# TencentARC/ViT-Lens

Hardware: AMD Instinct MI355X
Metric: modality-pairs/sec (ViT-L, 224^2 patches) (higher is better)
Workload: dtype bf16; 1 GPU; C3: ViT-L Lens(depth)->ViT + image + text tri-modal InfoNCE TRAINING step (fwd+bwd+AdamW), batch 1024/GPU in micro-batches of 256, first 4 blocks + adapter trainable; global_batch=1024, residual_dtype=bf16, accumulate=fp32, parallelism=dp1, gemm_cfg=-1, via=step, text_tower_operands=fp16, layernorm=folded into the GEMMs (frozen blocks), frozen_towers=second HIP stream beside the trainable tower's forward, backward=two halves of the micro-batches on two HIP streams

## Files before the change

include/vitlens_hip.h:

```cpp
#ifndef VITLENS_HIP_H
#define VITLENS_HIP_H

#include <stdint.h>

#ifdef __cplusplus
extern "C" {
#endif

#ifndef __HIP_PLATFORM_AMD__
typedef struct ihipStream_t* hipStream_t;
#endif

#define VL_EPI_BF16 0
#define VL_EPI_F32 1
#define VL_EPI_RES_F32 2
#define VL_EPI_RES_BF16 3
#define VL_EPI_GEGLU 5
#define VL_EPI_DGELU 6
#define VL_EPI_DGEGLU 7
#define VL_ACT_NONE 0
#define VL_ACT_GELU 1
#define VL_ACT_RELU 2
#define VL_ACT_GELU_DSAVE 4
#define VL_ACT_QGELU 5
#define VL_ACT_QGELU_DSAVE 6

#define VL_F32 0
#define VL_BF16 1
#define VL_F16 2

#define VL_GEMM_AUTO (-1)
#define VL_GEMM_PERSIST 8
#define VL_GEMM_PINGPONG 10

const char* vl_last_error(void);
#define VL_ABI_VERSION 606
int vl_version(void);

int vl_gemm_bf16(const void* A, const void* W, const float* bias, void* out, const void* res,
                 int M, int N, int K, int lda, int ldw, int ldo, float alpha, int epi, int act,
                 int cfg, hipStream_t stream);

int vl_gemm_splitk_accum_f32(const void* A, const void* W, float* out, int M, int N, int K, int lda, int ldw, long ldo,
                             float alpha, int splits, float* ws, hipStream_t stream);
int vl_gemm_tn_splitk_accum_f32(const void* At, const void* Bt, float* out, int M, int N, int K, int lda, int ldb, long ldo,
                                float alpha, int splits, float* ws, hipStream_t stream);
int vl_gemm_bf16_ex(const void* A, const void* W, const float* bias, void* out, const void* res, void* out2,
                    int M, int N, int K, int lda, int ldw, int ldo, float alpha, int epi, int act,
                    int res_div, int cfg, hipStream_t stream);

int vl_gemm_f16(const void* A, const void* W, const float* bias, void* out, const void* res, int M, int N, int K,
                int lda, int ldw, int ldo, float alpha, int epi, int act, hipStream_t stream);
int vl_attn_fwd_f16(const void* q, const void* k, const void* v, const long* strides, void* out, float* lse,
                    int B, int H, int Lq, int Lk, int dh, float qscale, int causal, hipStream_t stream);

int vl_gemm_f32(const float* A, const float* W, const float* bias, float* out, const float* res, int M, int N, int K,
                int lda, int ldw, int ldo, float alpha, int act, hipStream_t stream);
int vl_attn_fwd_f32(const float* q, const float* k, const float* v, const long* strides, float* out, float* lse,
                    int B, int H, int Lq, int Lk, int dh, float scale, int causal, hipStream_t stream);
int vl_im2col_f32(const float* x, float* patches, int N, int C, int H, int W, int kh, int kw, int sh, int sw,
                  int Kp, int transpose_hw, hipStream_t stream);
int vl_gemm_f32_ex(const float* A, const float* W, const float* bias, float* out, const float* res, int M, int N, int K,
                   int lda, int ldw, int ldo, float alpha, int act, int res_div, int res_pre, int geglu, hipStream_t stream);
int vl_knn_group_f32(const float* xyz, const int64_t* center_idx, int* nidx, float* patches, int B, int N, int G,
                     int k, int Kp, hipStream_t stream);
int vl_group_max_f32(const float* x, long ldx, float* out, long ldo, long groups, int M, int C, hipStream_t stream);
int vl_pad3_f32(const float* c, float* out, long R, int Kp, hipStream_t stream);

int vl_device_info(int device, char* arch, int arch_len, int* cus, int* clock_khz, long* hbm_bytes);

int vl_attn_fwd_bf16(const void* q, const void* k, const void* v, const long* strides, void* out, float* lse,
                     int B, int H, int Lq, int Lk, int dh, float qscale, int causal, hipStream_t stream);

int vl_gemm_main_rows(int M, int N);
int vl_gemm_lnfold_bf16(const void* A, const void* Wg, const float* bias_f, const float* ln_c, const float* ln_mean,
                        const float* ln_rstd, void* out, void* out2, int M, int N, int K, int lda, int ldw, int ldo, int act,
                        hipStream_t stream);
int vl_gemm_res_rowstats_bf16(const void* A, const void* W, const float* bias, void* out, const void* res, float* row_part,
                              int M, int N, int K, int lda, int ldw, int ldo, hipStream_t stream);
int vl_ln_row_stats(const float* row_part, int P, const void* x_bf16, long x_row_stride, int D, int m_main, int rows, float eps,
                    float* mean, float* rstd, const float* ln_w, const float* ln_b, void* y_left, long y_row_stride, int y_row0,
                    hipStream_t stream);

int vl_layernorm_fwd(const void* x, int x_dtype, long x_row_stride, const int64_t* row_index, long row_mul,
                     const float* w, const float* b, void* y, int y_dtype, long y_row_stride,
                     float* mean, float* rstd, int rows, int D, float eps, hipStream_t stream);

int vl_assemble_ln_pre(const void* tokens, int tok_dtype, const float* cls, const float* pos, const float* pos2,
                       const float* w, const float* b, void* y, int y_dtype, float* xpre, float* mean, float* rstd,
                       int B, int T, int D, float eps, hipStream_t stream);

int vl_l2_normalize(const float* x, float* y, void* y_bf16, float* norms, int rows, int D, float eps,
                    hipStream_t stream);
int vl_l2_normalize_bwd(const float* f, const float* df, const float* norms, float* dx, int rows, int D, float eps,
                        hipStream_t stream);

int vl_im2col_bf16(const float* x, void* patches, int N, int C, int H, int W, int kh, int kw, int sh, int sw,
                   int Kp, int transpose_hw, hipStream_t stream);

int vl_text_embed(const int64_t* ids, const float* tok_emb, const float* pos, void* out, int out_dtype,
                  int B, int L, int D, int vocab, hipStream_t stream);

int vl_cast_f32_bf16(const float* x, void* y, long n, hipStream_t stream);
int vl_add_rows(const void* x, int x_dtype, const float* table, void* y, int y_dtype, long rows, int T, int D,
                hipStream_t stream);
int vl_transpose_to_bf16(const void* in, int in_dtype, long ldi, int R, int C, void* out, long ldo, hipStream_t stream);
int vl_transpose_colsum_bf16(const void* in, int in_dtype, long ldi, int R, int C, void* out, long ldo,
                             float* colsum_out, float colsum_scale, float* ws, hipStream_t stream);

int vl_split_bf16x3(const float* x, void* out, long rows, int D, int pattern, hipStream_t stream);
int vl_ce_stats(const float* logits, long ld, int R, int C, int label_off, float* row_lse, float* col_lse,
                float* diag, float* col_ws, hipStream_t stream);
int vl_ce_loss_accum(const float* row_lse, const float* col_lse, const float* diag, int R, int C, int label_off,
                     float w_row, float w_col, float* loss_inout, hipStream_t stream);
int vl_ce_grad(const float* logits, long ld, int R, int C, int label_off, const float* row_lse, const float* col_lse,
               float w_row, float w_col, void* G, long ldg, void* GT, long ldgt, float logit_scale,
               float* dscale_inout, float* ws, hipStream_t stream);
long vl_ce_grad_ws_floats(int R, int C, long ldg, long ldgt);
int vl_ce_stats_masked(const float* logits, long ld, int R, int C, int label_off, float* row_lse, float* col_lse,
                       float* diag, float* col_ws, const float* sim, long ld_sim, float thres, hipStream_t stream);
int vl_ce_grad_masked(const float* logits, long ld, int R, int C, int label_off, const float* row_lse, const float* col_lse,
                      float w_row, float w_col, void* G, long ldg, void* GT, long ldgt, float logit_scale,
                      float* dscale_inout, float* ws, const float* sim, long ld_sim, float thres, hipStream_t stream);

int vl_layernorm_bwd(const void* dy, int dy_dtype, long dy_stride, const void* x, int x_dtype, long x_stride,
                     const float* mean, const float* rstd, const float* w, const float* dres, float* dx,
                     void* dx_bf16, long dx_stride, int rows, int D, hipStream_t stream);
int vl_layernorm_bwd_g(const void* dy, int dy_dtype, long dy_stride, const void* x, int x_dtype, long x_stride,
                       const float* mean, const float* rstd, const float* w, const void* dres, void* dx, int g_dtype,
                       void* dx_bf16, long dx_stride, int rows, int D, hipStream_t stream);
long vl_colreduce_ws_floats(int rows, int cols, int planes);
int vl_layernorm_bwd_params(const void* dy, int dy_dtype, long dy_stride, const void* x, int x_dtype, long x_stride,
                            const float* mean, const float* rstd, float* dw, float* db, int rows, int D,
                            float* ws, hipStream_t stream);
int vl_colsum(const void* a, int a_dtype, long lda, float* out, int rows, int cols, float scale, float* ws, hipStream_t stream);
int vl_gelu_bf16(const void* u, void* y, long n, hipStream_t stream);
int vl_geglu_bf16(const void* h, void* y, long rows, int n_out, hipStream_t stream);
int vl_attn_bwd_bf16(const void* q, const void* k, const void* v, const void* dO, const void* o, const long* strides,
                     const float* lse, float* delta, void* dq, void* dk, void* dv, long ld_dq, long ld_dkv,
                     int B, int H, int Lq, int Lk, int dh, float qscale, int causal, float scale, hipStream_t stream);
int vl_attn_bwd_fused_supported(int Lq, int Lk, int dh, int causal);
int vl_attn_bwd_fused_bf16(const void* q, const void* k, const void* v, const void* dO, const void* o, const long* strides,
                           const float* lse, void* dq, void* dk, void* dv, long ld_dq, long ld_dkv, int B, int H, int L, int dh,
                           float qscale, float scale, hipStream_t stream);
int vl_kaldi_fbank(const float* wave, long wave_stride, int batch, long n_samples, const float* window, const float* banks,
                   float* out, int target_len, int win, int shift, int nfft, int nmel, float preemph, float mean, float std,
                   hipStream_t stream);
int vl_resample_sinc(const float* in, long in_stride, int batch, long n_in, const int* offsets, const float* taps, int o, int n,
                     int K, float* out, long out_stride, long out_first, long n_out, hipStream_t stream);
int vl_fbank_augment(const float* in, float* out, int batch, int T, int F, const void* params, float mean, float std,
                     hipStream_t stream);
int vl_fps(const float* xyz, const int64_t* start, int64_t* idx, float* centers, int B, int N, int G, hipStream_t stream);
int vl_pc_gather_normalize(const float* pts, const int64_t* idx, float* out, int B, int N, int G, int C, hipStream_t stream);
int vl_resample_h_u8(const uint8_t* src, long row_stride, int W, int C, int row0, int nrows, const int* bounds,
                     const int* kk, int ksize, int xout0, int nxout, uint8_t* dst, hipStream_t stream);
int vl_resample_v_u8_norm(const uint8_t* src, int W, int C, int row0, int nrows, const int* bounds, const int* kk,
                          int ksize, int yout0, int nyout, const float* mean, const float* stdv, float* out,
                          uint8_t* out_u8, hipStream_t stream);
int vl_resample_batch_u8_norm(const int64_t* desc, int n, int C, int crop_h, int crop_w, int max_nrows, const int* tables,
                              uint8_t* tmp, const float* mean, const float* stdv, float* out, hipStream_t stream);
int vl_resample_h_f32(const float* src, long row_stride, int W, int row0, int nrows, const int* bounds,
                      const float* weights, int ksize, int xout0, int nxout, int clamp_on, float clamp_lo,
                      float clamp_hi, float divide_by, float* dst, hipStream_t stream);
int vl_resample_v_f32_norm(const float* src, int W, int H, int row0, const int* bounds, const float* weights, int ksize,
                           int yout0, int nyout, float mean, float stdv, float* out, hipStream_t stream);
int vl_knn_group(const float* xyz, const int64_t* center_idx, int* nidx, void* patches, int B, int N, int G,
                 int k, int Kp, hipStream_t stream);
int vl_ball_group(const float* xyz, const float* feats, const int64_t* center_idx, int* idx, void* patches, int B, int N,
                  int S, int D, float radius2, int nsample, int Kp, hipStream_t stream);
int vl_group_max(const void* x, long ldx, void* out, int out_dtype, long ldo, long groups, int M, int C, hipStream_t stream);
int vl_pad3_bf16(const float* c, void* out, long R, int Kp, hipStream_t stream);
int vl_bn_stats(const void* x, long ldx, int R, int C, float* ws, int nchunk, float* mean, float* var,
                float* running_mean, float* running_var, float momentum, hipStream_t stream);
int vl_bn_stats_local(const void* x, long ldx, int R, int C, float* ws, int nchunk, float* local, hipStream_t stream);
int vl_bn_stats_merge(const float* gathered, int W, int C, float* mean, float* var, float* running_mean,
                      float* running_var, float momentum, int* total, hipStream_t stream);
int vl_bn_bwd_reduce(const void* dy, long lddy, const void* x, long ldx, const float* mean, const float* var,
                     const float* gamma, const float* beta, float eps, int relu, float* ws, int nchunk, float* dgamma,
                     float* dbeta, float* sums, int R, int C, hipStream_t stream);
int vl_bn_bwd_apply(const void* dy, long lddy, const void* x, long ldx, const float* mean, const float* var,
                    const float* gamma, const float* beta, float eps, int relu, const float* sums, const int* total,
                    void* dx, long lddx, int R, int C, hipStream_t stream);
int vl_bn_apply(const void* x, long ldx, const float* mean, const float* var, const float* gamma, const float* beta,
                float eps, int relu, void* out, long ldo, long R, int C, hipStream_t stream);
int vl_bn_bwd(const void* dy, long lddy, const void* x, long ldx, const float* mean, const float* var,
              const float* gamma, const float* beta, float eps, int relu, int train, float* ws, int nchunk,
              float* dgamma, float* dbeta, void* dx, long lddx, int R, int C, hipStream_t stream);
int vl_group_max_bwd(const void* f, long ldf, const void* dg, long lddg, const void* base, long ldb, void* out,
                     long ldo, long groups, int M, int C, hipStream_t stream);
int vl_group_sum(const void* x, long ldx, void* out, long ldo, long groups, int M, int C, hipStream_t stream);
int vl_adamw_step(float* p, const float* g, float* m, float* v, long n, float lr, float beta1, float beta2,
                  float eps, float weight_decay, int step, float grad_scale, hipStream_t stream);
long vl_sumsq_ws_floats(void);
int vl_sumsq_f32(const float* x, long n, float* out, float* ws, hipStream_t stream);
typedef struct vl_adamw_slot {
  float* p; const float* g; float* m; float* v;
  long n;
  float weight_decay;
  int reserved;
} vl_adamw_slot;
#define VL_ADAMW_MAX_SLOTS 1024
int vl_adamw_multi_step(const vl_adamw_slot* slots, int nslots, float lr, float beta1, float beta2, float eps, int step,
                        float grad_scale, float max_norm, const float* sumsq, float* norm_out, hipStream_t stream);
int vl_clamp_scalar(float* p, float lo, float hi, hipStream_t stream);
int vl_axpy_f32(float* y, const float* x, float alpha, long n, hipStream_t stream);
int vl_scale_exp_f32(const float* x, float* out, long n, const float* log_scale, float mul, hipStream_t stream);
int vl_batch_rowsum(const float* x, float* out, int B, int T, int D, long batch_stride_rows, long row_offset,
                    hipStream_t stream);

typedef struct vl_comm* vl_comm_t;
int vl_comm_unique_id(void* id128);
int vl_comm_create(vl_comm_t* comm, const void* id128, int rank, int world);
int vl_comm_destroy(vl_comm_t comm);
int vl_allgather_embed(vl_comm_t comm, const float* local, float* gathered, long count, hipStream_t stream);
int vl_reducescatter_grad(vl_comm_t comm, const float* full, float* mine, long count_per_rank, hipStream_t stream);
int vl_allreduce_grad(vl_comm_t comm, float* buf, long count, hipStream_t stream);

#ifdef __cplusplus
}
#endif
#endif
```

vit-lens_amd/csrc/vl_bwd.hip:

```cpp
#include "vl_common.h"
#include "vitlens_hip.h"

namespace {

__device__ __forceinline__ float ld1(const float* p) { return *p; }
__device__ __forceinline__ float ld1(const bf16_t* p) { return bf2f(*p); }

__device__ __forceinline__ void ld4(const float* p, float (&v)[4]) {
  const f32x4 t = *(const f32x4*)p; v[0] = t[0]; v[1] = t[1]; v[2] = t[2]; v[3] = t[3];
}
__device__ __forceinline__ void ld4(const bf16_t* p, float (&v)[4]) {
  const u32x2 t = *(const u32x2*)p;
  v[0] = bf2f((bf16_t)(t[0] & 0xffff)); v[1] = bf2f((bf16_t)(t[0] >> 16));
  v[2] = bf2f((bf16_t)(t[1] & 0xffff)); v[3] = bf2f((bf16_t)(t[1] >> 16));
}
__device__ __forceinline__ void st4(float* p, const float (&v)[4]) { f32x4 t = {v[0], v[1], v[2], v[3]}; *(f32x4*)p = t; }
__device__ __forceinline__ void st4(bf16_t* p, const float (&v)[4]) {
  u32x2 t; t[0] = pack2bf(v[0], v[1]); t[1] = pack2bf(v[2], v[3]); *(u32x2*)p = t;
}

struct LnBwdP {
  const void* dy; const void* x; const float* mean; const float* rstd; const float* w;
  const void* dres;
  void* dx; bf16_t* dxb;
  long dys, xs, dxs;
  int rows, D;
};

template <int NCH, typename TDY, typename TX, typename TG>
__global__ void __launch_bounds__(256) ln_bwd_kernel(const LnBwdP p) {
  const int lane = threadIdx.x & 63;
  const int row = blockIdx.x * 4 + (threadIdx.x >> 6);
  if (row >= p.rows) return;
  const TDY* dy = (const TDY*)p.dy + (long)row * p.dys;
  const TX* x = (const TX*)p.x + (long)row * p.xs;
  const TG* dres = p.dres ? (const TG*)p.dres + (long)row * p.dxs : nullptr;
  TG* dx = p.dx ? (TG*)p.dx + (long)row * p.dxs : nullptr;
  bf16_t* dxb = p.dxb ? p.dxb + (long)row * p.dxs : nullptr;
  const float mu = p.mean[row], rs = p.rstd[row];
  const int D = p.D;
  if constexpr (NCH > 0) {
    float g[NCH][4], xh[NCH][4];
    float s1 = 0.f, s2 = 0.f;
#pragma unroll
    for (int c = 0; c < NCH; ++c) {
      const int e = c * 256 + lane * 4;
      float ww[4];
      ld4(dy + e, g[c]); ld4(x + e, xh[c]); ld4(p.w + e, ww);
#pragma unroll
      for (int k = 0; k < 4; ++k) {
        g[c][k] *= ww[k]; xh[c][k] = (xh[c][k] - mu) * rs;
        s1 += g[c][k]; s2 = fmaf(g[c][k], xh[c][k], s2);
      }
    }
    s1 = wave_sum(s1) / (float)D; s2 = wave_sum(s2) / (float)D;
#pragma unroll
    for (int c = 0; c < NCH; ++c) {
      const int e = c * 256 + lane * 4;
      float v[4];
#pragma unroll
      for (int k = 0; k < 4; ++k) v[k] = rs * (g[c][k] - s1 - xh[c][k] * s2);
      if (dres) {
        float r[4]; ld4(dres + e, r);
#pragma unroll
        for (int k = 0; k < 4; ++k) v[k] += r[k];
      }
      if (dx) st4(dx + e, v);
      if (dxb) st4(dxb + e, v);
    }
  } else {
    float s1 = 0.f, s2 = 0.f;
    for (int e = lane; e < D; e += 64) {
      const float g = ld1(dy + e) * p.w[e];
      const float xh = (ld1(x + e) - mu) * rs;
      s1 += g; s2 = fmaf(g, xh, s2);
    }
    s1 = wave_sum(s1) / (float)D; s2 = wave_sum(s2) / (float)D;
    for (int e = lane; e < D; e += 64) {
      const float g = ld1(dy + e) * p.w[e];
      const float xh = (ld1(x + e) - mu) * rs;
      float v = rs * (g - s1 - xh * s2);
      if (dres) v += ld1(dres + e);
      if (dx) { if constexpr (sizeof(TG) == 4) dx[e] = v; else dx[e] = f2bf(v); }
      if (dxb) dxb[e] = f2bf(v);
    }
  }
}

template <typename TDY, typename TX>
__global__ void __launch_bounds__(256) ln_bwd_params_kernel(const TDY* dy, long dys, const TX* x, long xs, const float* mean,
                                                            const float* rstd, float* ws, int rows, int D, int slab) {
  const int j = blockIdx.x * 256 + threadIdx.x;
  if (j >= D) return;
  const int r0 = blockIdx.y * slab, r1 = min(rows, r0 + slab);
  float a = 0.f, b = 0.f;
  for (int r = r0; r < r1; ++r) {
    const float g = ld1(dy + (long)r * dys + j);
    a = fmaf(g, (ld1(x + (long)r * xs + j) - mean[r]) * rstd[r], a);
    b += g;
  }
  ws[((long)blockIdx.y * 2) * D + j] = a; ws[((long)blockIdx.y * 2 + 1) * D + j] = b;
}

__global__ void __launch_bounds__(256) ln_bwd_params8_bf16_kernel(const bf16_t* dy, long dys, const bf16_t* x, long xs, const float* mean,
                                                                  const float* rstd, float* ws, int rows, int D, int slab) {
  __shared__ float sh[3][64][16];
  const int cx = threadIdx.x & 63, ry = threadIdx.x >> 6;
  const int j = (blockIdx.x * 64 + cx) * 8;
  const int r0 = blockIdx.y * slab, r1 = min(rows, r0 + slab);
  float a[8], b[8];
#pragma unroll
  for (int e = 0; e < 8; ++e) { a[e] = 0.f; b[e] = 0.f; }
  if (j < D) {
    for (int r = r0 + ry; r < r1; r += 8) {
      const bool two = r + 4 < r1;
      const int r2 = two ? r + 4 : r;
      const u32x4 g0 = *(const u32x4*)(dy + (long)r * dys + j), x0 = *(const u32x4*)(x + (long)r * xs + j);
      const u32x4 g1 = *(const u32x4*)(dy + (long)r2 * dys + j), x1 = *(const u32x4*)(x + (long)r2 * xs + j);
      const float m0 = mean[r], s0 = rstd[r], m1 = mean[r2], s1 = two ? rstd[r2] : 0.f;
      const float k1 = two ? 1.f : 0.f;
#pragma unroll
      for (int e = 0; e < 4; ++e) {
        const float gl = bf2f((bf16_t)(g0[e] & 0xffff)), gh = bf2f((bf16_t)(g0[e] >> 16));
        a[2 * e] = fmaf(gl, (bf2f((bf16_t)(x0[e] & 0xffff)) - m0) * s0, a[2 * e]);
        a[2 * e + 1] = fmaf(gh, (bf2f((bf16_t)(x0[e] >> 16)) - m0) * s0, a[2 * e + 1]);
        b[2 * e] += gl; b[2 * e + 1] += gh;
        const float hl = bf2f((bf16_t)(g1[e] & 0xffff)), hh = bf2f((bf16_t)(g1[e] >> 16));
        a[2 * e] = fmaf(hl, (bf2f((bf16_t)(x1[e] & 0xffff)) - m1) * s1, a[2 * e]);
        a[2 * e + 1] = fmaf(hh, (bf2f((bf16_t)(x1[e] >> 16)) - m1) * s1, a[2 * e + 1]);
        b[2 * e] = fmaf(hl, k1, b[2 * e]); b[2 * e + 1] = fmaf(hh, k1, b[2 * e + 1]);
      }
    }
  }
  if (ry) {
#pragma unroll
    for (int e = 0; e < 8; ++e) { sh[ry - 1][cx][e] = a[e]; sh[ry - 1][cx][8 + e] = b[e]; }
  }
  __syncthreads();
  if (ry == 0 && j < D) {
#pragma unroll
    for (int e = 0; e < 8; ++e) {
      ws[((long)blockIdx.y * 2) * D + j + e] = (a[e] + sh[0][cx][e]) + (sh[1][cx][e] + sh[2][cx][e]);
      ws[((long)blockIdx.y * 2 + 1) * D + j + e] = (b[e] + sh[0][cx][8 + e]) + (sh[1][cx][8 + e] + sh[2][cx][8 + e]);
    }
  }
}

__global__ void __launch_bounds__(256) colsum4_f32_kernel(const float* a, long lda, float* ws, int rows, int cols, int slab) {
  __shared__ float sh[3][64][4];
  const int cx = threadIdx.x & 63, ry = threadIdx.x >> 6;
  const int j = (blockIdx.x * 64 + cx) * 4;
  const int r0 = blockIdx.y * slab, r1 = min(rows, r0 + slab);
  f32x4 s = {0.f, 0.f, 0.f, 0.f};
  if (j < cols) {
    const float* ptr = a + j;
    int r = r0 + ry;
    for (; r + 12 < r1; r += 16) {
      const f32x4 v0 = *(const f32x4*)(ptr + (long)r * lda), v1 = *(const f32x4*)(ptr + (long)(r + 4) * lda);
      const f32x4 v2 = *(const f32x4*)(ptr + (long)(r + 8) * lda), v3 = *(const f32x4*)(ptr + (long)(r + 12) * lda);
      s += v0; s += v1; s += v2; s += v3;
    }
    for (; r < r1; r += 4) s += *(const f32x4*)(ptr + (long)r * lda);
  }
  if (ry) {
#pragma unroll
    for (int e = 0; e < 4; ++e) sh[ry - 1][cx][e] = s[e];
  }
  __syncthreads();
  if (ry == 0 && j < cols) {
#pragma unroll
    for (int e = 0; e < 4; ++e) ws[(long)blockIdx.y * cols + j + e] = (s[e] + sh[0][cx][e]) + (sh[1][cx][e] + sh[2][cx][e]);
  }
}

__global__ void __launch_bounds__(256) ln_bwd_params4_bf16_f32_kernel(const bf16_t* dy, long dys, const float* x, long xs, const float* mean,
                                                                      const float* rstd, float* ws, int rows, int D, int slab) {
  __shared__ float sh[3][64][8];
  const int cx = threadIdx.x & 63, ry = threadIdx.x >> 6;
  const int j = (blockIdx.x * 64 + cx) * 4;
  const int r0 = blockIdx.y * slab, r1 = min(rows, r0 + slab);
  float a[4], b[4];
#pragma unroll
  for (int e = 0; e < 4; ++e) { a[e] = 0.f; b[e] = 0.f; }
  if (j < D) {
    for (int r = r0 + ry; r < r1; r += 8) {
      const bool two = r + 4 < r1;
      const int r2 = two ? r + 4 : r;
      const u32x2 g0 = *(const u32x2*)(dy + (long)r * dys + j), g1 = *(const u32x2*)(dy + (long)r2 * dys + j);
      const f32x4 x0 = *(const f32x4*)(x + (long)r * xs + j), x1 = *(const f32x4*)(x + (long)r2 * xs + j);
      const float m0 = mean[r], s0 = rstd[r], m1 = mean[r2], s1 = two ? rstd[r2] : 0.f;
      const float k1 = two ? 1.f : 0.f;
#pragma unroll
      for (int e = 0; e < 4; ++e) {
        const float gl = bf2f((bf16_t)((e & 1) ? (g0[e >> 1] >> 16) : (g0[e >> 1] & 0xffff)));
        const float hl = bf2f((bf16_t)((e & 1) ? (g1[e >> 1] >> 16) : (g1[e >> 1] & 0xffff)));
        a[e] = fmaf(gl, (x0[e] - m0) * s0, a[e]);
        b[e] += gl;
        a[e] = fmaf(hl, (x1[e] - m1) * s1, a[e]);
        b[e] = fmaf(hl, k1, b[e]);
      }
    }
  }
  if (ry) {
#pragma unroll
    for (int e = 0; e < 4; ++e) { sh[ry - 1][cx][e] = a[e]; sh[ry - 1][cx][4 + e] = b[e]; }
  }
  __syncthreads();
  if (ry == 0 && j < D) {
#pragma unroll
    for (int e = 0; e < 4; ++e) {
      ws[((long)blockIdx.y * 2) * D + j + e] = (a[e] + sh[0][cx][e]) + (sh[1][cx][e] + sh[2][cx][e]);
      ws[((long)blockIdx.y * 2 + 1) * D + j + e] = (b[e] + sh[0][cx][4 + e]) + (sh[1][cx][4 + e] + sh[2][cx][4 + e]);
    }
  }
}

__global__ void __launch_bounds__(1024) slab_finalize_kernel(const float* ws, int nslab, int K, int D, float scale, float* out0, float* out1) {
  __shared__ float sh[16][64];
  const int jl = threadIdx.x & 63, g = threadIdx.x >> 6;
  const int j = blockIdx.x * 64 + jl, k = blockIdx.y;
  float s = 0.f;
  if (j < D)
    for (int t = g; t < nslab; t += 16) s += ws[((long)t * K + k) * D + j];
  sh[g][jl] = s;
  __syncthreads();
  if (g == 0 && j < D) {
    float a[16];
#pragma unroll
    for (int i = 0; i < 16; ++i) a[i] = sh[i][jl];
#pragma unroll
    for (int w = 8; w > 0; w >>= 1)
#pragma unroll
      for (int i = 0; i < w; ++i) a[i] += a[i + w];
    float* o = k == 0 ? out0 : out1;
    o[j] += a[0] * scale;
  }
}

template <typename T>
__global__ void __launch_bounds__(256) colsum_kernel(const T* a, long lda, float* ws, int rows, int cols, int slab) {
  const int j = blockIdx.x * 256 + threadIdx.x;
  if (j >= cols) return;
  const int r0 = blockIdx.y * slab, r1 = min(rows, r0 + slab);
  float s = 0.f;
  for (int r = r0; r < r1; ++r) s += ld1(a + (long)r * lda + j);
  ws[(long)blockIdx.y * cols + j] = s;
}

__global__ void __launch_bounds__(256) colsum8_bf16_kernel(const bf16_t* a, long lda, float* ws, int rows, int cols, int slab) {
  __shared__ float sh[3][64][8];
  const int cx = threadIdx.x & 63, ry = threadIdx.x >> 6;
  const int j = (blockIdx.x * 64 + cx) * 8;
  const int r0 = blockIdx.y * slab, r1 = min(rows, r0 + slab);
  float s[8];
#pragma unroll
  for (int e = 0; e < 8; ++e) s[e] = 0.f;
  auto add = [&](const u32x4 v) {
#pragma unroll
    for (int e = 0; e < 4; ++e) { s[2 * e] += bf2f((bf16_t)(v[e] & 0xffff)); s[2 * e + 1] += bf2f((bf16_t)(v[e] >> 16)); }
  };
  if (j < cols) {
    const bf16_t* ptr = a + j;
    int r = r0 + ry;
    for (; r + 12 < r1; r += 16) {
      const u32x4 v0 = *(const u32x4*)(ptr + (long)r * lda), v1 = *(const u32x4*)(ptr + (long)(r + 4) * lda);
      const u32x4 v2 = *(const u32x4*)(ptr + (long)(r + 8) * lda), v3 = *(const u32x4*)(ptr + (long)(r + 12) * lda);
      add(v0); add(v1); add(v2); add(v3);
    }
    for (; r < r1; r += 4) add(*(const u32x4*)(ptr + (long)r * lda));
  }
  if (ry) {
#pragma unroll
    for (int e = 0; e < 8; ++e) sh[ry - 1][cx][e] = s[e];
  }
  __syncthreads();
  if (ry == 0 && j < cols) {
#pragma unroll
    for (int e = 0; e < 8; ++e) ws[(long)blockIdx.y * cols + j + e] = (s[e] + sh[0][cx][e]) + (sh[1][cx][e] + sh[2][cx][e]);
  }
}

__global__ void __launch_bounds__(256) gelu_kernel(const bf16_t* u, bf16_t* y, long n) {
  for (long i = ((long)blockIdx.x * 256 + threadIdx.x) * 8; i < n; i += (long)gridDim.x * 256 * 8) {
    const u32x4 v = *(const u32x4*)(u + i);
    u32x4 o;
#pragma unroll
    for (int e = 0; e < 4; ++e)
      o[e] = pack2bf(gelu_erf(bf2f((bf16_t)(v[e] & 0xffff))), gelu_erf(bf2f((bf16_t)(v[e] >> 16))));
    *(u32x4*)(y + i) = o;
  }
}

__global__ void __launch_bounds__(256) geglu_kernel(const bf16_t* h, bf16_t* y, long n) {
  for (long i = ((long)blockIdx.x * 256 + threadIdx.x) * 4; i < n; i += (long)gridDim.x * 256 * 4) {
    const u32x4 v = *(const u32x4*)(h + 2 * i);
    u32x2 o;
    o[0] = pack2bf(bf2f((bf16_t)(v[0] & 0xffff)) * gelu_erf(bf2f((bf16_t)(v[0] >> 16))),
                   bf2f((bf16_t)(v[1] & 0xffff)) * gelu_erf(bf2f((bf16_t)(v[1] >> 16))));
    o[1] = pack2bf(bf2f((bf16_t)(v[2] & 0xffff)) * gelu_erf(bf2f((bf16_t)(v[2] >> 16))),
                   bf2f((bf16_t)(v[3] & 0xffff)) * gelu_erf(bf2f((bf16_t)(v[3] >> 16))));
    *(u32x2*)(y + i) = o;
  }
}

struct AdamwC { float lr, b1, b2, eps, bc1, bc2_sqrt; };
__device__ __forceinline__ void adamw_update(float& pi, const float gi, float& mi, float& vi, const AdamwC c, const float wd) {
#pragma clang fp contract(off)
  const float decay = fmaf(-c.lr, wd, 1.0f);
  mi = fmaf(1.0f - c.b1, gi, c.b1 * mi);
  vi = c.b2 * vi + ((1.0f - c.b2) * gi) * gi;
  pi = pi * decay - ((c.lr / c.bc1) * mi) / (sqrtf(vi) / c.bc2_sqrt + c.eps);
}

__global__ void __launch_bounds__(256) adamw_kernel(float* p, const float* g, float* m, float* v, long n, float lr, float b1,
                                                    float b2, float eps, float wd, float bc1, float bc2_sqrt, float gscale) {
  const AdamwC c{lr, b1, b2, eps, bc1, bc2_sqrt};
  for (long i = (long)blockIdx.x * 256 + threadIdx.x; i < n; i += (long)gridDim.x * 256) {
    float pi = p[i], mi = m[i], vi = v[i];
    adamw_update(pi, g[i] * gscale, mi, vi, c, wd);
    m[i] = mi; v[i] = vi;
    p[i] = pi;
  }
}

constexpr int kSumsqMaxBlocks = 2048;
constexpr int kSumsqPerBlock = 256 * 16;

__device__ __forceinline__ double wave_sum_f64(double v) {
#pragma unroll
  for (int o = 32; o > 0; o >>= 1) v += __shfl_xor(v, o, 64);
  return v;
}
__device__ __forceinline__ double block_sum_f64(double v) {
  __shared__ double sh[4];
  v = wave_sum_f64(v);
  if ((threadIdx.x & 63) == 0) sh[threadIdx.x >> 6] = v;
  __syncthreads();
  return (sh[0] + sh[1]) + (sh[2] + sh[3]);
}

__global__ void __launch_bounds__(256) sumsq_partial_kernel(const float* x, long n, double* part) {
  const long head = min(n, (long)((4 - (((uintptr_t)x >> 2) & 3)) & 3));
  const f32x4* x4 = (const f32x4*)(x + head);
  const long n4 = (n - head) >> 2;
  double a0 = 0.0, a1 = 0.0, a2 = 0.0, a3 = 0.0;
  const long stride = (long)gridDim.x * 1024;
  for (long base = (long)blockIdx.x * 1024; base < n4; base += stride) {
    const long i = base + threadIdx.x;
    const f32x4 z = {0.f, 0.f, 0.f, 0.f};
    f32x4 t0, t1, t2, t3;
    if (base + 1024 <= n4) {
      t0 = x4[i]; t1 = x4[i + 256]; t2 = x4[i + 512]; t3 = x4[i + 768];
    } else {
      t0 = i < n4 ? x4[i] : z; t1 = i + 256 < n4 ? x4[i + 256] : z;
      t2 = i + 512 < n4 ? x4[i + 512] : z; t3 = i + 768 < n4 ? x4[i + 768] : z;
    }
#pragma unroll
    for (int e = 0; e < 4; ++e) {
      a0 = fma((double)t0[e], (double)t0[e], a0); a1 = fma((double)t1[e], (double)t1[e], a1);
      a2 = fma((double)t2[e], (double)t2[e], a2); a3 = fma((double)t3[e], (double)t3[e], a3);
    }
  }
  if (blockIdx.x == 0 && threadIdx.x < 8) {
    const long t = threadIdx.x < 4 ? threadIdx.x : head + n4 * 4 + (threadIdx.x - 4);
    const bool live = threadIdx.x < 4 ? t < head : t < n;
    if (live) a1 = fma((double)x[t], (double)x[t], a1);
  }
  const double s = block_sum_f64((a0 + a1) + (a2 + a3));
  if (threadIdx.x == 0) part[blockIdx.x] = s;
}

__global__ void __launch_bounds__(256) sumsq_final_kernel(const double* part, int nparts, float* out) {
  double a = 0.0;
  for (int i = threadIdx.x; i < nparts; i += 256) a += part[i];
  const double s = block_sum_f64(a);
  if (threadIdx.x == 0) out[0] = (float)s;
}

constexpr int kAdamTile = 2048;

__device__ __forceinline__ float clip_coef(const float norm, const float max_norm) {
  const float c = max_norm / (norm + 1e-6f);
  return c > 1.0f ? 1.0f : c;
}

__global__ void __launch_bounds__(256) adamw_multi_kernel(const vl_adamw_slot* slots, int nslots, AdamwC c, float gscale,
                                                          float max_norm, const float* sumsq, float* norm_out) {
  __shared__ int first[VL_ADAMW_MAX_SLOTS + 1];
  if (threadIdx.x < 64) {
    const int lane = threadIdx.x;
    int cnt[16], sum = 0;
#pragma unroll
    for (int k = 0; k < 16; ++k) {
      const int s = lane * 16 + k;
      cnt[k] = s < nslots ? (int)((slots[s].n + kAdamTile - 1) / kAdamTile) : 0;
      sum += cnt[k];
    }
    int incl = sum;
#pragma unroll
    for (int o = 1; o < 64; o <<= 1) {
      const int t = __shfl_up(incl, o, 64);
      if (lane >= o) incl += t;
    }
    int run = incl - sum;
#pragma unroll
    for (int k = 0; k < 16; ++k) {
      const int s = lane * 16 + k;
      if (s < nslots) first[s] = run;
      run += cnt[k];
    }
    if (lane == 63) first[nslots] = incl;
  }
  __syncthreads();
  const int ntiles = first[nslots];
  const float norm = gscale * sqrtf(sumsq[0]);
  const float gmul = clip_coef(norm, max_norm);
  if (norm_out && blockIdx.x == 0 && threadIdx.x == 0) norm_out[0] = norm;
  for (int tile = blockIdx.x; tile < ntiles; tile += gridDim.x) {
    int lo = 0, hi = nslots - 1;
    while (lo < hi) {
      const int mid = (lo + hi + 1) >> 1;
      if (first[mid] <= tile) lo = mid; else hi = mid - 1;
    }
    const vl_adamw_slot S = slots[lo];
    const long base = (long)(tile - first[lo]) * kAdamTile;
    const int cntE = (int)min((long)kAdamTile, S.n - base);
    float* p = S.p + base; const float* g = S.g + base; float* m = S.m + base; float* v = S.v + base;
    const float wd = S.weight_decay;
    const bool vec = ((((uintptr_t)p | (uintptr_t)g | (uintptr_t)m | (uintptr_t)v) & 15) == 0);
    const int nvec = vec ? (cntE >> 2) : 0;
    for (int i = threadIdx.x; i < nvec; i += 256) {
      f32x4 pp = ((f32x4*)p)[i], mm = ((f32x4*)m)[i], vv = ((f32x4*)v)[i];
      const f32x4 gg = ((const f32x4*)g)[i];
#pragma unroll
      for (int e = 0; e < 4; ++e) {
        float pe = pp[e], me = mm[e], ve = vv[e];
        adamw_update(pe, gg[e] * gscale * gmul, me, ve, c, wd);
        pp[e] = pe; mm[e] = me; vv[e] = ve;
      }
      ((f32x4*)m)[i] = mm; ((f32x4*)v)[i] = vv; ((f32x4*)p)[i] = pp;
    }
    for (int i = nvec * 4 + threadIdx.x; i < cntE; i += 256) {
      float pe = p[i], me = m[i], ve = v[i];
      adamw_update(pe, g[i] * gscale * gmul, me, ve, c, wd);
      m[i] = me; v[i] = ve; p[i] = pe;
    }
  }
}

__global__ void clamp_scalar_kernel(float* p, float lo, float hi) { *p = fminf(fmaxf(*p, lo), hi); }

__global__ void __launch_bounds__(256) axpy_kernel(float* y, const float* x, float alpha, long n) {
  for (long i = (long)blockIdx.x * 256 + threadIdx.x; i < n; i += (long)gridDim.x * 256) y[i] = fmaf(alpha, x[i], y[i]);
}

__global__ void __launch_bounds__(256) scale_exp_kernel(const float* x, float* out, long n, const float* log_scale, float mul) {
  const float s = __expf(log_scale[0]) * mul;
  for (long i = (long)blockIdx.x * 256 + threadIdx.x; i < n; i += (long)gridDim.x * 256) out[i] = x[i] * s;
}

__global__ void __launch_bounds__(256) batch_rowsum_kernel(const float* x, float* out, int B, int T, int D, long bstride, long toff) {
  const long n = (long)T * D;
  for (long i = (long)blockIdx.x * 256 + threadIdx.x; i < n; i += (long)gridDim.x * 256) {
    const long t = i / D; const int d = (int)(i - t * D);
    float s = 0.f;
    for (int b = 0; b < B; ++b) s += x[((long)b * bstride + toff + t) * D + d];
    out[i] += s;
  }
}

}

extern "C" int vl_set_error(const char* msg);
#define VL_HIP_OK(e) do { hipError_t _e = (e); if (_e != hipSuccess) return vl_set_error(hipGetErrorString(_e)); } while (0)
static int grid_for(long n) { long g = (n + 255) / 256; return (int)(g > 4096 ? 4096 : (g < 1 ? 1 : g)); }

template <typename TDY, typename TX, typename TG>
static void ln_bwd_launch(const LnBwdP& p, hipStream_t stream) {
  const dim3 g((p.rows + 3) / 4), b(256);
  const bool vec = (p.D % 256 == 0) && (p.dys % 4 == 0) && (p.xs % 4 == 0) && (p.dxs % 4 == 0);
  if (vec && p.D == 1024) hipLaunchKernelGGL((ln_bwd_kernel<4, TDY, TX, TG>), g, b, 0, stream, p);
  else if (vec && p.D == 768) hipLaunchKernelGGL((ln_bwd_kernel<3, TDY, TX, TG>), g, b, 0, stream, p);
  else if (vec && p.D == 512) hipLaunchKernelGGL((ln_bwd_kernel<2, TDY, TX, TG>), g, b, 0, stream, p);
  else if (vec && p.D == 256) hipLaunchKernelGGL((ln_bwd_kernel<1, TDY, TX, TG>), g, b, 0, stream, p);
  else hipLaunchKernelGGL((ln_bwd_kernel<0, TDY, TX, TG>), g, b, 0, stream, p);
}

extern "C" int vl_layernorm_bwd_g(const void* dy, int dy_dtype, long dy_stride, const void* x, int x_dtype, long x_stride,
                                  const float* mean, const float* rstd, const float* w, const void* dres, void* dx, int g_dtype,
                                  void* dx_bf16, long dx_stride, int rows, int D, hipStream_t stream) {
  if (rows <= 0 || D <= 0) return vl_set_error("vl_layernorm_bwd: empty problem");
  LnBwdP p{dy, x, mean, rstd, w, dres, dx, (bf16_t*)dx_bf16, dy_stride, x_stride, dx_stride, rows, D};
  const int key = (dy_dtype == VL_BF16 ? 4 : 0) | (x_dtype == VL_BF16 ? 2 : 0) | (g_dtype == VL_BF16 ? 1 : 0);
  switch (key) {
    case 0: ln_bwd_launch<float, float, float>(p, stream); break;
    case 1: ln_bwd_launch<float, float, bf16_t>(p, stream); break;
    case 2: ln_bwd_launch<float, bf16_t, float>(p, stream); break;
    case 3: ln_bwd_launch<float, bf16_t, bf16_t>(p, stream); break;
    case 4: ln_bwd_launch<bf16_t, float, float>(p, stream); break;
    case 5: ln_bwd_launch<bf16_t, float, bf16_t>(p, stream); break;
    case 6: ln_bwd_launch<bf16_t, bf16_t, float>(p, stream); break;
    default: ln_bwd_launch<bf16_t, bf16_t, bf16_t>(p, stream); break;
  }
  VL_HIP_OK(hipGetLastError());
  return 0;
}

extern "C" int vl_layernorm_bwd(const void* dy, int dy_dtype, long dy_stride, const void* x, int x_dtype, long x_stride,
                                const float* mean, const float* rstd, const float* w, const float* dres, float* dx,
                                void* dx_bf16, long dx_stride, int rows, int D, hipStream_t stream) {
  return vl_layernorm_bwd_g(dy, dy_dtype, dy_stride, x, x_dtype, x_stride, mean, rstd, w, dres, dx, VL_F32, dx_bf16, dx_stride, rows, D, stream);
}

static const int kSlabRows = 256;
extern "C" long vl_colreduce_ws_floats(int rows, int cols, int planes) {
  return (long)((rows + kSlabRows - 1) / kSlabRows) * planes * cols;
}

extern "C" int vl_layernorm_bwd_params(const void* dy, int dy_dtype, long dy_stride, const void* x, int x_dtype, long x_stride,
                                       const float* mean, const float* rstd, float* dw, float* db, int rows, int D,
                                       float* ws, hipStream_t stream) {
  if (rows <= 0 || D <= 0) return vl_set_error("vl_layernorm_bwd_params: empty problem");
  if (!ws) return vl_set_error("vl_layernorm_bwd_params: workspace of vl_colreduce_ws_floats(rows, D, 2) floats required");
  const int slab = kSlabRows, nslab = (rows + slab - 1) / slab;
  const dim3 g((D + 255) / 256, nslab), b(256);
  if (dy_dtype == VL_BF16 && x_dtype == VL_F32 && (D & 3) == 0 && (dy_stride & 3) == 0 && (x_stride & 3) == 0 &&
      ((uintptr_t)dy & 7) == 0 && ((uintptr_t)x & 15) == 0)
    hipLaunchKernelGGL(ln_bwd_params4_bf16_f32_kernel, dim3((D + 255) / 256, nslab), b, 0, stream, (const bf16_t*)dy, dy_stride, (const float*)x, x_stride, mean, rstd, ws, rows, D, slab);
  else if (dy_dtype == VL_BF16 && x_dtype == VL_F32)
    hipLaunchKernelGGL((ln_bwd_params_kernel<bf16_t, float>), g, b, 0, stream, (const bf16_t*)dy, dy_stride, (const float*)x, x_stride, mean, rstd, ws, rows, D, slab);
  else if (dy_dtype == VL_BF16 && (D & 7) == 0 && (dy_stride & 7) == 0 && (x_stride & 7) == 0 && (((uintptr_t)dy | (uintptr_t)x) & 15) == 0)
    hipLaunchKernelGGL(ln_bwd_params8_bf16_kernel, dim3((D + 511) / 512, nslab), b, 0, stream, (const bf16_t*)dy, dy_stride, (const bf16_t*)x, x_stride, mean, rstd, ws, rows, D, slab);
  else if (dy_dtype == VL_BF16)
    hipLaunchKernelGGL((ln_bwd_params_kernel<bf16_t, bf16_t>), g, b, 0, stream, (const bf16_t*)dy, dy_stride, (const bf16_t*)x, x_stride, mean, rstd, ws, rows, D, slab);
  else if (x_dtype == VL_F32)
    hipLaunchKernelGGL((ln_bwd_params_kernel<float, float>), g, b, 0, stream, (const float*)dy, dy_stride, (const float*)x, x_stride, mean, rstd, ws, rows, D, slab);
  else
    hipLaunchKernelGGL((ln_bwd_params_kernel<float, bf16_t>), g, b, 0, stream, (const float*)dy, dy_stride, (const bf16_t*)x, x_stride, mean, rstd, ws, rows, D, slab);
  hipLaunchKernelGGL(slab_finalize_kernel, dim3((D + 63) / 64, 2), dim3(1024), 0, stream, ws, nslab, 2, D, 1.0f, dw, db);
  VL_HIP_OK(hipGetLastError());
  return 0;
}

extern "C" int vl_colsum(const void* a, int a_dtype, long lda, float* out, int rows, int cols, float scale, float* ws, hipStream_t stream) {
  if (rows <= 0 || cols <= 0) return vl_set_error("vl_colsum: empty problem");
  if (!ws) return vl_set_error("vl_colsum: workspace of vl_colreduce_ws_floats(rows, cols, 1) floats required");
  const int slab = kSlabRows, nslab = (rows + slab - 1) / slab;
  const dim3 g((cols + 255) / 256, nslab), b(256);
  if (a_dtype == VL_BF16 && (cols & 7) == 0 && (lda & 7) == 0 && ((uintptr_t)a & 15) == 0)
    hipLaunchKernelGGL(colsum8_bf16_kernel, dim3((cols + 511) / 512, nslab), b, 0, stream, (const bf16_t*)a, lda, ws, rows, cols, slab);
  else if (a_dtype == VL_BF16) hipLaunchKernelGGL(colsum_kernel<bf16_t>, g, b, 0, stream, (const bf16_t*)a, lda, ws, rows, cols, slab);
  else if (a_dtype == VL_F32 && (cols & 3) == 0 && (lda & 3) == 0 && ((uintptr_t)a & 15) == 0)
    hipLaunchKernelGGL(colsum4_f32_kernel, g, b, 0, stream, (const float*)a, lda, ws, rows, cols, slab);
  else hipLaunchKernelGGL(colsum_kernel<float>, g, b, 0, stream, (const float*)a, lda, ws, rows, cols, slab);
  hipLaunchKernelGGL(slab_finalize_kernel, dim3((cols + 63) / 64, 1), dim3(1024), 0, stream, ws, nslab, 1, cols, scale, out, out);
  VL_HIP_OK(hipGetLastError());
  return 0;
}

extern "C" int vl_gelu_bf16(const void* u, void* y, long n, hipStream_t stream) {
  if (n <= 0) return 0;
  if (n & 7) return vl_set_error("vl_gelu_bf16: n must be a multiple of 8");
  hipLaunchKernelGGL(gelu_kernel, dim3(grid_for(n / 8)), dim3(256), 0, stream, (const bf16_t*)u, (bf16_t*)y, n);
  VL_HIP_OK(hipGetLastError());
  return 0;
}

extern "C" int vl_geglu_bf16(const void* h, void* y, long rows, int n_out, hipStream_t stream) {
  const long n = rows * n_out;
  if (n <= 0) return 0;
  if (n_out & 3) return vl_set_error("vl_geglu_bf16: n_out must be a multiple of 4");
  hipLaunchKernelGGL(geglu_kernel, dim3(grid_for(n / 4)), dim3(256), 0, stream, (const bf16_t*)h, (bf16_t*)y, n);
  VL_HIP_OK(hipGetLastError());
  return 0;
}

extern "C" int vl_adamw_step(float* p, const float* g, float* m, float* v, long n, float lr, float beta1, float beta2,
                             float eps, float weight_decay, int step, float grad_scale, hipStream_t stream) {
  if (n <= 0) return 0;
  if (step < 1) return vl_set_error("vl_adamw_step: step counts from 1");
  const float bc1 = 1.0f - powf(beta1, (float)step);
  const float bc2s = sqrtf(1.0f - powf(beta2, (float)step));
  hipLaunchKernelGGL(adamw_kernel, dim3(grid_for(n)), dim3(256), 0, stream, p, g, m, v, n, lr, beta1, beta2, eps, weight_decay,
                     bc1, bc2s, grad_scale);
  VL_HIP_OK(hipGetLastError());
  return 0;
}

extern "C" long vl_sumsq_ws_floats(void) { return 2L * kSumsqMaxBlocks; }

extern "C" int vl_sumsq_f32(const float* x, long n, float* out, float* ws, hipStream_t stream) {
  if (n < 0) return vl_set_error("vl_sumsq_f32: negative n");
  if (!out || !ws || (n > 0 && !x)) return vl_set_error("vl_sumsq_f32: null argument");
  if (((uintptr_t)x & 3) || ((uintptr_t)out & 3)) return vl_set_error("vl_sumsq_f32: x and out must be 4-byte aligned");
  if ((uintptr_t)ws & 7) return vl_set_error("vl_sumsq_f32: workspace of vl_sumsq_ws_floats() floats, 8-byte aligned, required");
  const long want = (n / 4 + 1023) / 1024;
  const int nb = (int)(want > kSumsqMaxBlocks ? kSumsqMaxBlocks : (want < 1 ? 1 : want));
  hipLaunchKernelGGL(sumsq_partial_kernel, dim3(nb), dim3(256), 0, stream, x, n, (double*)ws);
  hipLaunchKernelGGL(sumsq_final_kernel, dim3(1), dim3(256), 0, stream, (const double*)ws, nb, out);
  VL_HIP_OK(hipGetLastError());
  return 0;
}

extern "C" int vl_adamw_multi_step(const vl_adamw_slot* slots, int nslots, float lr, float beta1, float beta2, float eps, int step,
                                   float grad_scale, float max_norm, const float* sumsq, float* norm_out, hipStream_t stream) {
  if (nslots < 0 || nslots > VL_ADAMW_MAX_SLOTS) return vl_set_error("vl_adamw_multi_step: 0 <= nslots <= VL_ADAMW_MAX_SLOTS");
  if (step < 1) return vl_set_error("vl_adamw_multi_step: step counts from 1");
  if (!(max_norm > 0.0f)) return vl_set_error("vl_adamw_multi_step: max_norm must be positive");
  if (!sumsq || (nslots > 0 && !slots)) return vl_set_error("vl_adamw_multi_step: null argument");
  if (nslots == 0) return 0;
  const AdamwC c{lr, beta1, beta2, eps, 1.0f - powf(beta1, (float)step), sqrtf(1.0f - powf(beta2, (float)step))};
  hipLaunchKernelGGL(adamw_multi_kernel, dim3(2048), dim3(256), 0, stream, slots, nslots, c, grad_scale, max_norm, sumsq, norm_out);
  VL_HIP_OK(hipGetLastError());
  return 0;
}

extern "C" int vl_clamp_scalar(float* p, float lo, float hi, hipStream_t stream) {
  hipLaunchKernelGGL(clamp_scalar_kernel, dim3(1), dim3(1), 0, stream, p, lo, hi);
  VL_HIP_OK(hipGetLastError());
  return 0;
}

extern "C" int vl_axpy_f32(float* y, const float* x, float alpha, long n, hipStream_t stream) {
  if (n <= 0) return 0;
  hipLaunchKernelGGL(axpy_kernel, dim3(grid_for(n)), dim3(256), 0, stream, y, x, alpha, n);
  VL_HIP_OK(hipGetLastError());
  return 0;
}

extern "C" int vl_scale_exp_f32(const float* x, float* out, long n, const float* log_scale, float mul, hipStream_t stream) {
  if (n <= 0) return 0;
  if (!x || !out || !log_scale) return vl_set_error("vl_scale_exp_f32: null argument");
  hipLaunchKernelGGL(scale_exp_kernel, dim3(grid_for(n)), dim3(256), 0, stream, x, out, n, log_scale, mul);
  VL_HIP_OK(hipGetLastError());
  return 0;
}

extern "C" int vl_batch_rowsum(const float* x, float* out, int B, int T, int D, long batch_stride_rows, long row_offset,
                               hipStream_t stream) {
  if (B <= 0 || T <= 0 || D <= 0) return vl_set_error("vl_batch_rowsum: empty problem");
  hipLaunchKernelGGL(batch_rowsum_kernel, dim3(grid_for((long)T * D)), dim3(256), 0, stream, x, out, B, T, D, batch_stride_rows, row_offset);
  VL_HIP_OK(hipGetLastError());
  return 0;
}
```

vit-lens_amd/vitlens_hip/_lib.py:

```python
import ctypes as C
import os

_HERE = os.path.dirname(os.path.abspath(__file__))
_LIB = None


class LibraryNotBuilt(ImportError):
    pass


def lib_path() -> str:
    return os.path.join(_HERE, "libvitlens_hip.so")


P, I, L, F = C.c_void_p, C.c_int, C.c_long, C.c_float

ABI_VERSION = 606

SIGNATURES = {
    "vl_version": [],
    "vl_device_info": [I, C.c_char_p, I, C.POINTER(I), C.POINTER(I), C.POINTER(L)],
    "vl_gemm_bf16": [P, P, P, P, P, I, I, I, I, I, I, F, I, I, I, P],
    "vl_gemm_splitk_accum_f32": [P, P, P, I, I, I, I, I, L, F, I, P, P],
    "vl_gemm_tn_splitk_accum_f32": [P, P, P, I, I, I, I, I, L, F, I, P, P],
    "vl_attn_fwd_bf16": [P, P, P, P, P, P, I, I, I, I, I, F, I, P],
    "vl_gemm_f16": [P, P, P, P, P, I, I, I, I, I, I, F, I, I, P],
    "vl_gemm_f32": [P, P, P, P, P, I, I, I, I, I, I, F, I, P],
    "vl_attn_fwd_f32": [P, P, P, P, P, P, I, I, I, I, I, F, I, P],
    "vl_im2col_f32": [P, P, I, I, I, I, I, I, I, I, I, I, P],
    "vl_gemm_f32_ex": [P, P, P, P, P, I, I, I, I, I, I, F, I, I, I, I, P],
    "vl_knn_group_f32": [P, P, P, P, I, I, I, I, I, P],
    "vl_group_max_f32": [P, L, P, L, L, I, I, P],
    "vl_pad3_f32": [P, P, L, I, P],
    "vl_attn_fwd_f16": [P, P, P, P, P, P, I, I, I, I, I, F, I, P],
    "vl_layernorm_fwd": [P, I, L, P, L, P, P, P, I, L, P, P, I, I, F, P],
    "vl_gemm_main_rows": [I, I],
    "vl_gemm_lnfold_bf16": [P, P, P, P, P, P, P, P, I, I, I, I, I, I, I, P],
    "vl_gemm_res_rowstats_bf16": [P, P, P, P, P, P, I, I, I, I, I, I, P],
    "vl_ln_row_stats": [P, I, P, L, I, I, I, F, P, P, P, P, P, L, I, P],
    "vl_assemble_ln_pre": [P, I, P, P, P, P, P, P, I, P, P, P, I, I, I, F, P],
    "vl_l2_normalize": [P, P, P, P, I, I, F, P],
    "vl_l2_normalize_bwd": [P, P, P, P, I, I, F, P],
    "vl_im2col_bf16": [P, P, I, I, I, I, I, I, I, I, I, I, P],
    "vl_text_embed": [P, P, P, P, I, I, I, I, I, P],
    "vl_cast_f32_bf16": [P, P, L, P],
    "vl_add_rows": [P, I, P, P, I, L, I, I, P],
    "vl_transpose_to_bf16": [P, I, L, I, I, P, L, P],
    "vl_transpose_colsum_bf16": [P, I, L, I, I, P, L, P, F, P, P],
    "vl_split_bf16x3": [P, P, L, I, I, P],
    "vl_ce_stats": [P, L, I, I, I, P, P, P, P, P],
    "vl_ce_loss_accum": [P, P, P, I, I, I, F, F, P, P],
    "vl_ce_grad": [P, L, I, I, I, P, P, F, F, P, L, P, L, F, P, P, P],
    "vl_ce_grad_ws_floats": [I, I, L, L],
    "vl_ce_stats_masked": [P, L, I, I, I, P, P, P, P, P, L, F, P],
    "vl_ce_grad_masked": [P, L, I, I, I, P, P, F, F, P, L, P, L, F, P, P, P, L, F, P],
    "vl_gemm_bf16_ex": [P, P, P, P, P, P, I, I, I, I, I, I, F, I, I, I, I, P],
    "vl_kaldi_fbank": [P, L, I, L, P, P, P, I, I, I, I, I, F, F, F, P],
    "vl_resample_sinc": [P, L, I, L, P, P, I, I, I, P, L, L, L, P],
    "vl_fbank_augment": [P, P, I, I, I, P, F, F, P],
    "vl_fps": [P, P, P, P, I, I, I, P],
    "vl_pc_gather_normalize": [P, P, P, I, I, I, I, P],
    "vl_resample_h_u8": [P, L, I, I, I, I, P, P, I, I, I, P, P],
    "vl_resample_v_u8_norm": [P, I, I, I, I, P, P, I, I, I, P, P, P, P, P],
    "vl_resample_batch_u8_norm": [P, I, I, I, I, I, P, P, P, P, P, P],
    "vl_resample_h_f32": [P, L, I, I, I, P, P, I, I, I, I, F, F, F, P, P],
    "vl_resample_v_f32_norm": [P, I, I, I, P, P, I, I, I, F, F, P, P],
    "vl_knn_group": [P, P, P, P, I, I, I, I, I, P],
    "vl_ball_group": [P, P, P, P, P, I, I, I, I, F, I, I, P],
    "vl_group_max": [P, L, P, I, L, L, I, I, P],
    "vl_pad3_bf16": [P, P, L, I, P],
    "vl_bn_stats": [P, L, I, I, P, I, P, P, P, P, F, P],
    "vl_bn_stats_local": [P, L, I, I, P, I, P, P],
    "vl_bn_stats_merge": [P, I, I, P, P, P, P, F, P, P],
    "vl_bn_bwd_reduce": [P, L, P, L, P, P, P, P, F, I, P, I, P, P, P, I, I, P],
    "vl_bn_bwd_apply": [P, L, P, L, P, P, P, P, F, I, P, P, P, L, I, I, P],
    "vl_bn_apply": [P, L, P, P, P, P, F, I, P, L, L, I, P],
    "vl_bn_bwd": [P, L, P, L, P, P, P, P, F, I, I, P, I, P, P, P, L, I, I, P],
    "vl_group_max_bwd": [P, L, P, L, P, L, P, L, L, I, I, P],
    "vl_group_sum": [P, L, P, L, L, I, I, P],
    "vl_layernorm_bwd": [P, I, L, P, I, L, P, P, P, P, P, P, L, I, I, P],
    "vl_layernorm_bwd_g": [P, I, L, P, I, L, P, P, P, P, P, I, P, L, I, I, P],
    "vl_colreduce_ws_floats": [I, I, I],
    "vl_layernorm_bwd_params": [P, I, L, P, I, L, P, P, P, P, I, I, P, P],
    "vl_colsum": [P, I, L, P, I, I, F, P, P],
    "vl_gelu_bf16": [P, P, L, P],
    "vl_geglu_bf16": [P, P, L, I, P],
    "vl_attn_bwd_bf16": [P, P, P, P, P, P, P, P, P, P, P, L, L, I, I, I, I, I, F, I, F, P],
    "vl_attn_bwd_fused_supported": [I, I, I, I],
    "vl_attn_bwd_fused_bf16": [P, P, P, P, P, P, P, P, P, P, L, L, I, I, I, I, F, F, P],
    "vl_adamw_step": [P, P, P, P, L, F, F, F, F, F, I, F, P],
    "vl_sumsq_ws_floats": [],
    "vl_sumsq_f32": [P, L, P, P, P],
    "vl_adamw_multi_step": [P, I, F, F, F, F, I, F, F, P, P, P],
    "vl_clamp_scalar": [P, F, F, P],
    "vl_axpy_f32": [P, P, F, L, P],
    "vl_scale_exp_f32": [P, P, L, P, F, P],
    "vl_batch_rowsum": [P, P, I, I, I, L, L, P],
    "vl_comm_unique_id": [P],
    "vl_comm_create": [C.POINTER(P), P, I, I],
    "vl_comm_destroy": [P],
    "vl_allgather_embed": [P, P, P, L, P],
    "vl_reducescatter_grad": [P, P, P, L, P],
    "vl_allreduce_grad": [P, P, L, P],
}


_RET = {"vl_colreduce_ws_floats": L, "vl_ce_grad_ws_floats": L, "vl_sumsq_ws_floats": L}


def load_library():
    global _LIB
    if _LIB is not None:
        return _LIB
    path = lib_path()
    if not os.path.exists(path):
        raise LibraryNotBuilt(
            f"{path} is missing: build it with `python -c 'import __graft_entry__ as g; g.build()'` "
            "or `make -C vit-lens_amd/csrc` (hipcc --offload-arch=gfx950). No CPU/eager fallback exists.")
    lib = C.CDLL(path)
    lib.vl_last_error.restype = C.c_char_p
    lib.vl_last_error.argtypes = []
    for name, args in SIGNATURES.items():
        fn = getattr(lib, name)
        fn.argtypes = args
        fn.restype = _RET.get(name, I)
    got = int(lib.vl_version())
    if got != ABI_VERSION:
        raise RuntimeError(f"{path} reports ABI version {got}, this binding was written for {ABI_VERSION} "
                           "(include/vitlens_hip.h: VL_ABI_VERSION): rebuild the library (`make -C vit-lens_amd/csrc`)")
    _LIB = lib
    return lib


def check(status: int):
    if status != 0:
        raise RuntimeError("libvitlens_hip: " + load_library().vl_last_error().decode())
```

vit-lens_amd/vitlens_hip/engine.py:

```python
from dataclasses import dataclass
from typing import Dict, Optional

import os

import torch

from . import ops


@dataclass
class TowerCfg:
    width: int = 1024
    layers: int = 24
    heads: int = 16
    mlp_ratio: float = 4.0
    patch: int = 14
    image_size: int = 224
    embed_dim: int = 768
    in_chans: int = 3
    quick_gelu: bool = False


@dataclass
class TextCfg:
    context_length: int = 77
    vocab_size: int = 49408
    width: int = 768
    heads: int = 12
    layers: int = 12
    embed_dim: int = 768
    quick_gelu: bool = False


def _pad64(n):
    return (n + 63) // 64 * 64


def _dev(t, device, dtype=torch.float32):
    out = t.detach().to(device=device, dtype=dtype).contiguous()
    return out.clone() if out.data_ptr() == t.data_ptr() else out


def prep_block(sd: Dict[str, torch.Tensor], p: str, device) -> Dict[str, torch.Tensor]:
    bf = torch.bfloat16
    dv = lambda k: sd[p + k].detach().to(device)
    blk = _prep_block_plain(sd, p, device)
    if LN_FOLD:
        blk["in_f"] = ops.fold_ln_linear(dv("attn.in_proj_weight"), dv("attn.in_proj_bias"), dv("ln_1.weight"), dv("ln_1.bias"))
        blk["fc_f"] = ops.fold_ln_linear(dv("mlp.c_fc.weight"), dv("mlp.c_fc.bias"), dv("ln_2.weight"), dv("ln_2.bias"))
    return blk


def _prep_block_plain(sd: Dict[str, torch.Tensor], p: str, device) -> Dict[str, torch.Tensor]:
    bf = torch.bfloat16
    return {
        "ln1_w": _dev(sd[p + "ln_1.weight"], device), "ln1_b": _dev(sd[p + "ln_1.bias"], device),
        "in_w": _dev(sd[p + "attn.in_proj_weight"], device, bf), "in_b": _dev(sd[p + "attn.in_proj_bias"], device),
        "out_w": _dev(sd[p + "attn.out_proj.weight"], device, bf), "out_b": _dev(sd[p + "attn.out_proj.bias"], device),
        "ln2_w": _dev(sd[p + "ln_2.weight"], device), "ln2_b": _dev(sd[p + "ln_2.bias"], device),
        "fc_w": _dev(sd[p + "mlp.c_fc.weight"], device, bf), "fc_b": _dev(sd[p + "mlp.c_fc.bias"], device),
        "proj_w": _dev(sd[p + "mlp.c_proj.weight"], device, bf), "proj_b": _dev(sd[p + "mlp.c_proj.bias"], device),
    }


def conv_weight_as_gemm(w: torch.Tensor, device, dtype=torch.bfloat16) -> torch.Tensor:
    O = w.shape[0]
    K = w[0].numel()
    out = torch.zeros(O, _pad64(K), dtype=torch.float32, device=w.device)
    out[:, :K] = w.detach().reshape(O, K).float()
    return out.to(device=device, dtype=dtype).contiguous()


def copy_tree(dst, src):
    if torch.is_tensor(dst):
        dst.copy_(src)
    elif isinstance(dst, dict):
        for k in dst:
            copy_tree(dst[k], src[k])
    else:
        for d, s_ in zip(dst, src):
            copy_tree(d, s_)


class _Workspace:
    def __init__(self, B, L, D, H, hidden, device, res_dtype):
        dh = D // H
        bf = torch.bfloat16
        self.Lp = (L + 7) // 8 * 8
        self.x = torch.empty(B * L, D, device=device, dtype=res_dtype)
        self.h = torch.empty(B * L, D, device=device, dtype=bf)
        self.qkv = torch.empty(B * L, 3 * D, device=device, dtype=bf)
        hv = lambda i: ops.heads_view(self.qkv, B, L, H, dh, i * D)
        self.q, self.k, self.v = hv(0), hv(1), hv(2)
        self.a = torch.empty(B * L, D, device=device, dtype=bf)
        self.hid = torch.empty(B * L, hidden, device=device, dtype=bf)
        self.mean = torch.empty(B * L, device=device, dtype=torch.float32)
        self.rstd = torch.empty(B * L, device=device, dtype=torch.float32)
        self.part = torch.empty(B * L * (D // 64) * 2, device=device, dtype=torch.float32) if D % 64 == 0 else None


LN_FOLD = True


def run_blocks(blocks, ws: _Workspace, B, L, D, H, causal=False, cfg=-1, fold=None, quick_gelu=False):
    dh = D // H
    act = ops.mlp_act(quick_gelu)
    res_epi = ops.EPI_RES_F32 if ws.x.dtype == torch.float32 else ops.EPI_RES_BF16
    if fold is None:
        fold = LN_FOLD
    can_fold = bool(fold) and ws.x.dtype == torch.bfloat16 and ws.part is not None
    folded = [can_fold and "in_f" in w for w in blocks]
    mm = 0
    r_in = r_fc = 0
    if any(folded):
        r_in, r_fc = ops.fold_rows(ws.x, ws.qkv, 3 * D), ops.fold_rows(ws.x, ws.hid, ws.hid.shape[1])
    for i, w in enumerate(blocks):
        nxt = i + 1 < len(blocks) and folded[i + 1]
        if folded[i]:
            k_in = dict(ln_w=w["ln1_w"], ln_b=w["ln1_b"], h_left=ws.h, h_row0=r_in) if mm <= r_in else {}
            ops.ln_row_stats(ws.part, ws.x, mm, ws.mean, ws.rstd, **k_in)
            ops.gemm_lnfold(ws.x, w["in_f"], ws.mean, ws.rstd, ws.qkv, w["in_w"], w["in_b"], w["ln1_w"], w["ln1_b"], ws.h, cfg=cfg,
                            h_ready=bool(k_in))
            ops.attn_fwd(ws.q, ws.k, ws.v, ws.a, causal=causal, qscale=dh ** -0.5 * ops.LOG2E)
            mm = ops.gemm_res_rowstats(ws.a, w["out_w"], w["out_b"], ws.x, ws.x, ws.part, cfg=cfg)
            k_fc = dict(ln_w=w["ln2_w"], ln_b=w["ln2_b"], h_left=ws.h, h_row0=r_fc) if mm <= r_fc else {}
            ops.ln_row_stats(ws.part, ws.x, mm, ws.mean, ws.rstd, **k_fc)
            ops.gemm_lnfold(ws.x, w["fc_f"], ws.mean, ws.rstd, ws.hid, w["fc_w"], w["fc_b"], w["ln2_w"], w["ln2_b"], ws.h,
                            act=act, cfg=cfg, h_ready=bool(k_fc))
        else:
            ops.layernorm(ws.x, w["ln1_w"], w["ln1_b"], ws.h, B * L, D)
            ops.gemm(ws.h, w["in_w"], w["in_b"], out=ws.qkv, epi=ops.EPI_BF16, cfg=cfg)
            ops.attn_fwd(ws.q, ws.k, ws.v, ws.a, causal=causal, qscale=dh ** -0.5 * ops.LOG2E)
            ops.gemm(ws.a, w["out_w"], w["out_b"], out=ws.x, res=ws.x, epi=res_epi, cfg=cfg)
            ops.layernorm(ws.x, w["ln2_w"], w["ln2_b"], ws.h, B * L, D)
            ops.gemm(ws.h, w["fc_w"], w["fc_b"], out=ws.hid, epi=ops.EPI_BF16, act=act, cfg=cfg)
        if nxt:
            mm = ops.gemm_res_rowstats(ws.hid, w["proj_w"], w["proj_b"], ws.x, ws.x, ws.part, cfg=cfg)
        else:
            ops.gemm(ws.hid, w["proj_w"], w["proj_b"], out=ws.x, res=ws.x, epi=res_epi, cfg=cfg)
            mm = 0


def _hi_lo(w: torch.Tensor, device):
    w = w.detach().float().to(device)
    hi = w.bfloat16()
    lo = (w - hi.float()).bfloat16()
    return hi.contiguous(), lo.contiguous()


def prep_block_wsplit(sd: Dict[str, torch.Tensor], p: str, device) -> Dict[str, torch.Tensor]:
    blk = prep_block(sd, p, device)
    for key, name in (("in_w", "attn.in_proj_weight"), ("fc_w", "mlp.c_fc.weight")):
        hi, lo = _hi_lo(sd[p + name], device)
        blk[key + "2"] = torch.cat([hi, lo], dim=1).contiguous()
    for key, name in (("out_w", "attn.out_proj.weight"), ("proj_w", "mlp.c_proj.weight")):
        blk[key], blk[key + "_lo"] = _hi_lo(sd[p + name], device)
    return blk


def run_blocks_wsplit(blocks, ws: "_Workspace", B, L, D, H, causal=False, cfg=-1, quick_gelu=False):
    dh = D // H
    act = ops.mlp_act(quick_gelu)
    h2 = ws.h2
    for w in blocks:
        ops.layernorm(ws.x, w["ln1_w"], w["ln1_b"], h2[:, :D], B * L, D)
        ops.layernorm(ws.x, w["ln1_w"], w["ln1_b"], h2[:, D:], B * L, D)
        ops.gemm(h2, w["in_w2"], w["in_b"], out=ws.qkv, epi=ops.EPI_BF16, cfg=cfg)
        ops.attn_fwd(ws.q, ws.k, ws.v, ws.a, causal=causal, qscale=dh ** -0.5 * ops.LOG2E)
        ops.gemm(ws.a, w["out_w"], w["out_b"], out=ws.x, res=ws.x, epi=ops.EPI_RES_F32, cfg=cfg)
        ops.gemm(ws.a, w["out_w_lo"], None, out=ws.x, res=ws.x, epi=ops.EPI_RES_F32, cfg=cfg)
        ops.layernorm(ws.x, w["ln2_w"], w["ln2_b"], h2[:, :D], B * L, D)
        ops.layernorm(ws.x, w["ln2_w"], w["ln2_b"], h2[:, D:], B * L, D)
        ops.gemm(h2, w["fc_w2"], w["fc_b"], out=ws.hid, epi=ops.EPI_BF16, act=act, cfg=cfg)
        ops.gemm(ws.hid, w["proj_w"], w["proj_b"], out=ws.x, res=ws.x, epi=ops.EPI_RES_F32, cfg=cfg)
        ops.gemm(ws.hid, w["proj_w_lo"], None, out=ws.x, res=ws.x, epi=ops.EPI_RES_F32, cfg=cfg)


class VitEngine:

    def __init__(self, sd, prefix: str, cfg: TowerCfg, device, res_dtype=torch.float32, gemm_cfg: int = -1,
                 n_tokens: Optional[int] = None):
        self.cfg, self.device, self.res_dtype, self.gemm_cfg = cfg, torch.device(device), res_dtype, gemm_cfg
        self.prefix = prefix
        D = cfg.width
        self.cls = _dev(sd[prefix + "class_embedding"], device)
        self.pos = _dev(sd[prefix + "positional_embedding"], device)
        self.T = self.pos.shape[0] - 1
        self.ln_pre = (_dev(sd[prefix + "ln_pre.weight"], device), _dev(sd[prefix + "ln_pre.bias"], device))
        self.ln_post = (_dev(sd[prefix + "ln_post.weight"], device), _dev(sd[prefix + "ln_post.bias"], device))
        self.projT = _dev(sd[prefix + "proj"].t(), device, torch.bfloat16) if prefix + "proj" in sd else None
        self.blocks = [prep_block(sd, f"{prefix}transformer.resblocks.{i}.", device) for i in range(cfg.layers)]
        self.conv_w = None
        if prefix + "conv1.weight" in sd:
            self.conv_w = conv_weight_as_gemm(sd[prefix + "conv1.weight"], device)
        self._ws = {}

    def update_params(self, sd, names):
        p, dev = self.prefix, self.device
        top = {n for n in names if not n.startswith("transformer.resblocks.")}
        if "class_embedding" in top:
            self.cls.copy_(sd[p + "class_embedding"])
        if "positional_embedding" in top:
            self.pos.copy_(sd[p + "positional_embedding"])
        for nm, pair in (("ln_pre", self.ln_pre), ("ln_post", self.ln_post)):
            if nm + ".weight" in top or nm + ".bias" in top:
                pair[0].copy_(sd[p + nm + ".weight"]); pair[1].copy_(sd[p + nm + ".bias"])
        if "proj" in top and self.projT is not None:
            self.projT.copy_(sd[p + "proj"].t())
        if "conv1.weight" in top and self.conv_w is not None:
            self.conv_w.copy_(conv_weight_as_gemm(sd[p + "conv1.weight"], dev))
        for l in sorted({int(n.split(".")[2]) for n in names if n.startswith("transformer.resblocks.")}):
            copy_tree(self.blocks[l], prep_block(sd, f"{p}transformer.resblocks.{l}.", dev))

    def workspace(self, B, L):
        key = (B, L)
        if key not in self._ws:
            self._ws[key] = _Workspace(B, L, self.cfg.width, self.cfg.heads, int(self.cfg.width * self.cfg.mlp_ratio),
                                       self.device, self.res_dtype)
        return self._ws[key]

    def patch_tokens(self, image: torch.Tensor) -> torch.Tensor:
        p = self.cfg.patch
        cols, gh, gw = ops.im2col(image.contiguous().float(), p, p, p, p, self.conv_w.shape[1])
        return ops.gemm(cols, self.conv_w, None, epi=ops.EPI_BF16, cfg=self.gemm_cfg)

    def trunk(self, tokens: torch.Tensor, B: int, pos2: Optional[torch.Tensor] = None, use_orig_pos=True):
        cfg = self.cfg
        D, T = cfg.width, tokens.shape[0] // B
        L = T + 1
        ws = self.workspace(B, L)
        pos = self.pos if use_orig_pos else torch.zeros_like(self.pos)
        ops.assemble_ln_pre(tokens, self.cls, pos, pos2, self.ln_pre[0], self.ln_pre[1], ws.x, B, T, D)
        run_blocks(self.blocks, ws, B, L, D, cfg.heads, causal=False, cfg=self.gemm_cfg, quick_gelu=cfg.quick_gelu)
        pooled = torch.empty(B, D, device=self.device, dtype=torch.bfloat16)
        if self.projT is None:
            pooled = torch.empty(B, D, device=self.device, dtype=torch.float32)
        ops.layernorm(ws.x, self.ln_post[0], self.ln_post[1], pooled, B, D, x_row_stride=L * D)
        if self.projT is None:
            return pooled
        return ops.gemm(pooled, self.projT, None, epi=ops.EPI_F32, cfg=self.gemm_cfg)

    def encode_image(self, image: torch.Tensor, normalize: bool = False) -> torch.Tensor:
        B = image.shape[0]
        f = self.trunk(self.patch_tokens(image), B)
        return ops.l2_normalize(f) if normalize else f


def prep_block_f16(sd: Dict[str, torch.Tensor], p: str, device) -> Dict[str, torch.Tensor]:
    hf = torch.float16
    return {
        "ln1_w": _dev(sd[p + "ln_1.weight"], device), "ln1_b": _dev(sd[p + "ln_1.bias"], device),
        "in_w": _dev(sd[p + "attn.in_proj_weight"], device, hf), "in_b": _dev(sd[p + "attn.in_proj_bias"], device),
        "out_w": _dev(sd[p + "attn.out_proj.weight"], device, hf), "out_b": _dev(sd[p + "attn.out_proj.bias"], device),
        "ln2_w": _dev(sd[p + "ln_2.weight"], device), "ln2_b": _dev(sd[p + "ln_2.bias"], device),
        "fc_w": _dev(sd[p + "mlp.c_fc.weight"], device, hf), "fc_b": _dev(sd[p + "mlp.c_fc.bias"], device),
        "proj_w": _dev(sd[p + "mlp.c_proj.weight"], device, hf), "proj_b": _dev(sd[p + "mlp.c_proj.bias"], device),
    }


class _WorkspaceF16:

    def __init__(self, B, L, D, H, device):
        hf = torch.float16
        self.rows = B * L
        self.Mp = (self.rows + 255) // 256 * 256
        self.Bp = (B + 255) // 256 * 256
        z = lambda *shape, dt=hf: torch.zeros(*shape, device=device, dtype=dt)
        self.x = z(self.Mp, D, dt=torch.float32)
        self.h, self.qkv, self.a, self.hid = z(self.Mp, D), z(self.Mp, 3 * D), z(self.Mp, D), z(self.Mp, 4 * D)
        dh = D // H
        hv = lambda i: ops.heads_view(self.qkv, B, L, H, dh, i * D)
        self.q, self.k, self.v = hv(0), hv(1), hv(2)
        self.pooled = z(self.Bp, D)


class TextEngine:

    def __init__(self, sd, cfg: TextCfg, device, res_dtype=torch.float32, gemm_cfg: int = -1, wsplit: Optional[bool] = None,
                 arith: str = "f16"):
        self.cfg, self.device, self.gemm_cfg = cfg, torch.device(device), gemm_cfg
        if wsplit is not None:
            arith = "bf16x2" if wsplit else "bf16"
        if arith not in ("f16", "bf16x2", "bf16"):
            raise ValueError(f"TextEngine: arith must be 'f16', 'bf16x2' or 'bf16', got {arith!r}")
        if arith == "f16" and (cfg.width % 256 or cfg.width < 512 or cfg.width // cfg.heads != 64 or cfg.embed_dim % 256
                               or cfg.context_length > 288):
            arith = "bf16x2"
        self.arith = arith
        self.wsplit = arith == "bf16x2"
        self.res_dtype = res_dtype if arith == "bf16" else torch.float32
        self.tok = _dev(sd["token_embedding.weight"], device)
        self.pos = _dev(sd["positional_embedding"], device)
        self.ln_final = (_dev(sd["ln_final.weight"], device), _dev(sd["ln_final.bias"], device))
        if arith == "f16":
            self.projT = _dev(sd["text_projection"].t(), device, torch.float16)
            self.blocks = [prep_block_f16(sd, f"transformer.resblocks.{i}.", device) for i in range(cfg.layers)]
        elif self.wsplit:
            hi, lo = _hi_lo(sd["text_projection"].t(), device)
            self.projT = torch.cat([hi, lo], dim=1).contiguous()
            self.blocks = [prep_block_wsplit(sd, f"transformer.resblocks.{i}.", device) for i in range(cfg.layers)]
        else:
            self.projT = _dev(sd["text_projection"].t(), device, torch.bfloat16)
            self.blocks = [_prep_block_plain(sd, f"transformer.resblocks.{i}.", device) for i in range(cfg.layers)]
        self._ws = {}

    def _encode_f16(self, text: torch.Tensor) -> torch.Tensor:
        cfg = self.cfg
        B, L = text.shape
        D, H = cfg.width, cfg.heads
        key = ("f16", B, L)
        if key not in self._ws:
            self._ws[key] = _WorkspaceF16(B, L, D, H, self.device)
        ws = self._ws[key]
        rows = ws.rows
        ops.text_embed(text, self.tok, self.pos, ws.x[:rows])
        eot = text.argmax(dim=-1).contiguous()
        qs = (D // H) ** -0.5 * ops.LOG2E
        act = ops.mlp_act(cfg.quick_gelu)
        for w in self.blocks:
            ops.layernorm(ws.x, w["ln1_w"], w["ln1_b"], ws.h, rows, D)
            ops.gemm_f16(ws.h, w["in_w"], w["in_b"], out=ws.qkv)
            ops.attn_fwd(ws.q, ws.k, ws.v, ws.a, causal=True, qscale=qs)
            ops.gemm_f16(ws.a, w["out_w"], w["out_b"], out=ws.x, res=ws.x, epi=ops.EPI_RES_F32)
            ops.layernorm(ws.x, w["ln2_w"], w["ln2_b"], ws.h, rows, D)
            ops.gemm_f16(ws.h, w["fc_w"], w["fc_b"], out=ws.hid, act=act)
            ops.gemm_f16(ws.hid, w["proj_w"], w["proj_b"], out=ws.x, res=ws.x, epi=ops.EPI_RES_F32)
        ops.layernorm(ws.x, self.ln_final[0], self.ln_final[1], ws.pooled, B, D, x_row_stride=D, row_index=eot, row_mul=L)
        f = torch.zeros(ws.Bp, self.projT.shape[0], device=self.device, dtype=torch.float32)
        ops.gemm_f16(ws.pooled, self.projT, None, out=f, res=f, epi=ops.EPI_RES_F32)
        return f[:B]

    def encode_text(self, text: torch.Tensor, normalize: bool = False) -> torch.Tensor:
        cfg = self.cfg
        B, L = text.shape
        D = cfg.width
        text = text.to(self.device).contiguous()
        if self.arith == "f16":
            f = self._encode_f16(text)
            return ops.l2_normalize(f) if normalize else f.contiguous()
        key = (B, L)
        if key not in self._ws:
            self._ws[key] = _Workspace(B, L, D, cfg.heads, 4 * D, self.device, self.res_dtype)
        ws = self._ws[key]
        ops.text_embed(text, self.tok, self.pos, ws.x)
        eot = text.argmax(dim=-1).contiguous()
        if self.wsplit:
            if not hasattr(ws, "h2"):
                ws.h2 = torch.empty(B * L, 2 * D, device=self.device, dtype=torch.bfloat16)
            run_blocks_wsplit(self.blocks, ws, B, L, D, cfg.heads, causal=True, cfg=self.gemm_cfg, quick_gelu=cfg.quick_gelu)
            pooled = torch.empty(B, 2 * D, device=self.device, dtype=torch.bfloat16)
            for half in (pooled[:, :D], pooled[:, D:]):
                ops.layernorm(ws.x, self.ln_final[0], self.ln_final[1], half, B, D, x_row_stride=D, row_index=eot, row_mul=L)
        else:
            run_blocks(self.blocks, ws, B, L, D, cfg.heads, causal=True, cfg=self.gemm_cfg, fold=False, quick_gelu=cfg.quick_gelu)
            pooled = torch.empty(B, D, device=self.device, dtype=torch.bfloat16)
            ops.layernorm(ws.x, self.ln_final[0], self.ln_final[1], pooled, B, D, x_row_stride=D, row_index=eot, row_mul=L)
        f = ops.gemm(pooled, self.projT, None, epi=ops.EPI_F32, cfg=self.gemm_cfg)
        return ops.l2_normalize(f) if normalize else f


@dataclass
class LensCfg:
    modality: str = "depth"
    perceiver_identity: bool = True
    depth: int = 2
    self_per_cross: int = 3
    num_latents: int = 256
    latent_dim: int = 1024
    input_chan: int = 1024
    cross_heads: int = 1
    cross_dim_head: int = 64
    latent_heads: int = 16
    latent_dim_head: int = 64
    audio_fstride: int = 10
    audio_tstride: int = 10
    audio_mel_bins: int = 128
    audio_target_length: int = 512
    pc_num_group: int = 512
    pc_group_size: int = 32
    pc_encoder_dims: int = 256
    pc_trans_dim: int = 384
    pc_tokenizer: str = "pointbert"
    pc_radius: float = 0.2
    pc_in_dim: int = 3
    use_orig_pos: bool = True
    disable_adapter_pos: bool = False
    eeg_chans: int = 128
    eeg_time_len: int = 512
    eeg_window_size: int = 1
    eeg_stride: int = 1
    weight_tie_layers: bool = False


def _interleave_geglu(w: torch.Tensor, b: torch.Tensor):
    half = w.shape[0] // 2
    wi = torch.stack([w[:half], w[half:]], dim=1).reshape(w.shape[0], w.shape[1])
    bi = torch.stack([b[:half], b[half:]], dim=1).reshape(-1)
    return wi, bi


def prep_lens_attn(sd, p, device, packed_self: bool):
    bf = torch.bfloat16
    d = {"to_out_w": _dev(sd[p + "to_out.weight"], device, bf), "to_out_b": _dev(sd[p + "to_out.bias"], device)}
    if packed_self:
        d["qkv_w"] = _dev(torch.cat([sd[p + "to_q.weight"], sd[p + "to_kv.weight"]], 0), device, bf)
    else:
        d["q_w"] = _dev(sd[p + "to_q.weight"], device, bf)
        d["kv_w"] = _dev(sd[p + "to_kv.weight"], device, bf)
    return d


def prep_lens_ff(sd, p, device):
    w0, b0 = _interleave_geglu(sd[p + "net.0.weight"].detach().float(), sd[p + "net.0.bias"].detach().float())
    return {"w0": _dev(w0, device, torch.bfloat16), "b0": _dev(b0, device),
            "w2": _dev(sd[p + "net.2.weight"], device, torch.bfloat16), "b2": _dev(sd[p + "net.2.bias"], device)}


class PerceiverEngine:

    def __init__(self, sd, prefix: str, cfg: LensCfg, device, gemm_cfg=-1):
        self.cfg, self.device, self.gemm_cfg = cfg, torch.device(device), gemm_cfg
        self.latents = _dev(sd[prefix + "latents"], device)
        ln = lambda q: (_dev(sd[q + ".weight"], device), _dev(sd[q + ".bias"], device))
        self.layers = []
        for i in range(cfg.depth):
            if cfg.weight_tie_layers and i >= 2:
                self.layers.append(self.layers[1])
                continue
            q = f"{prefix}layers.{i}."
            lay = {"x_norm": ln(q + "0.norm"), "x_norm_ctx": ln(q + "0.norm_context"),
                   "x_attn": prep_lens_attn(sd, q + "0.fn.", device, False),
                   "x_ff_norm": ln(q + "1.norm"), "x_ff": prep_lens_ff(sd, q + "1.fn.", device), "selfs": []}
            for j in range(cfg.self_per_cross):
                r = f"{q}2.{j}."
                lay["selfs"].append({"norm": ln(r + "0.norm"), "attn": prep_lens_attn(sd, r + "0.fn.", device, True),
                                     "ff_norm": ln(r + "1.norm"), "ff": prep_lens_ff(sd, r + "1.fn.", device)})
            self.layers.append(lay)
        self._ws = {}

    def update_params(self, sd, prefix: str):
        fresh = PerceiverEngine(sd, prefix, self.cfg, self.device, self.gemm_cfg)
        self.latents.copy_(fresh.latents)
        copy_tree(self.layers, fresh.layers)

    def _workspace(self, B, Tc):
        key = (B, Tc)
        if key in self._ws:
            return self._ws[key]
        c, dev, bf = self.cfg, self.device, torch.bfloat16
        n, D = c.num_latents, c.latent_dim
        f = lambda *s, dt=bf: torch.empty(*s, device=dev, dtype=dt)
        ws = {
            "x": f(B * n, D, dt=torch.float32), "h": f(B * n, D), "ctx": f(B * Tc, c.input_chan),
            "xq2": f(B * n, c.cross_heads * c.cross_dim_head), "xkv2": f(B * Tc, 2 * c.cross_heads * c.cross_dim_head),
            "xa": f(B * n, c.cross_heads * c.cross_dim_head),
            "sqkv2": f(B * n, 3 * c.latent_heads * c.latent_dim_head),
            "sa": f(B * n, c.latent_heads * c.latent_dim_head), "hid": f(B * n, 4 * D),
        }
        xi, si = c.cross_heads * c.cross_dim_head, c.latent_heads * c.latent_dim_head
        ws["xq"] = ops.heads_view(ws["xq2"], B, n, c.cross_heads, c.cross_dim_head)
        ws["xk"] = ops.heads_view(ws["xkv2"], B, Tc, c.cross_heads, c.cross_dim_head)
        ws["xv"] = ops.heads_view(ws["xkv2"], B, Tc, c.cross_heads, c.cross_dim_head, xi)
        for i, nm in enumerate(("sq", "sk", "sv")):
            ws[nm] = ops.heads_view(ws["sqkv2"], B, n, c.latent_heads, c.latent_dim_head, i * si)
        self._ws[key] = ws
        return ws

    def _ff(self, ws, norm, ff, rows, D):
        ops.layernorm(ws["x"], norm[0], norm[1], ws["h"], rows, D)
        ops.gemm(ws["h"], ff["w0"], ff["b0"], out=ws["hid"], epi=ops.EPI_GEGLU, cfg=self.gemm_cfg)
        ops.gemm(ws["hid"], ff["w2"], ff["b2"], out=ws["x"], res=ws["x"], epi=ops.EPI_RES_F32, cfg=self.gemm_cfg)

    def forward(self, data: torch.Tensor, B: int) -> torch.Tensor:
        c = self.cfg
        Tc, n, D = data.shape[0] // B, c.num_latents, c.latent_dim
        ws = self._workspace(B, Tc)
        ws["x"].view(B, n, D).copy_(self.latents)
        rows = B * n
        for lay in self.layers:
            a = lay["x_attn"]
            ops.layernorm(ws["x"], lay["x_norm"][0], lay["x_norm"][1], ws["h"], rows, D)
            ops.layernorm(data, lay["x_norm_ctx"][0], lay["x_norm_ctx"][1], ws["ctx"], B * Tc, c.input_chan)
            ops.gemm(ws["h"], a["q_w"], None, out=ws["xq2"], epi=ops.EPI_BF16, cfg=self.gemm_cfg)
            ops.gemm(ws["ctx"], a["kv_w"], None, out=ws["xkv2"], epi=ops.EPI_BF16, cfg=self.gemm_cfg)
            ops.attn_fwd(ws["xq"], ws["xk"], ws["xv"], ws["xa"], qscale=c.cross_dim_head ** -0.5 * ops.LOG2E)
            ops.gemm(ws["xa"], a["to_out_w"], a["to_out_b"], out=ws["x"], res=ws["x"], epi=ops.EPI_RES_F32, cfg=self.gemm_cfg)
            self._ff(ws, lay["x_ff_norm"], lay["x_ff"], rows, D)
            for sl in lay["selfs"]:
                a = sl["attn"]
                ops.layernorm(ws["x"], sl["norm"][0], sl["norm"][1], ws["h"], rows, D)
                ops.gemm(ws["h"], a["qkv_w"], None, out=ws["sqkv2"], epi=ops.EPI_BF16, cfg=self.gemm_cfg)
                ops.attn_fwd(ws["sq"], ws["sk"], ws["sv"], ws["sa"], qscale=c.latent_dim_head ** -0.5 * ops.LOG2E)
                ops.gemm(ws["sa"], a["to_out_w"], a["to_out_b"], out=ws["x"], res=ws["x"], epi=ops.EPI_RES_F32, cfg=self.gemm_cfg)
                self._ff(ws, sl["ff_norm"], sl["ff"], rows, D)
        return ws["x"]


class LensEngine:

    def __init__(self, sd, prefix: str, tower: TowerCfg, lens: LensCfg, device, res_dtype=torch.float32, gemm_cfg=-1):
        self.tower, self.lens, self.device, self.gemm_cfg = tower, lens, torch.device(device), gemm_cfg
        self.vit = VitEngine(sd, prefix, tower, device, res_dtype=res_dtype, gemm_cfg=gemm_cfg)
        a = prefix + "visual_adapter."
        self.prefix_adapter = a
        self.adapter_pos = None
        if lens.modality in ("depth", "audio"):
            self.conv_w = conv_weight_as_gemm(sd[a + "conv1.weight"], device)
            pos = sd[a + "pos_emb"].detach().float()
            self.adapter_pos = _dev(pos * (0.0 if lens.disable_adapter_pos else 1.0), device)
        elif lens.modality == "eeg":
            self.conv_w = conv_weight_as_gemm(sd[a + "proj.weight"].unsqueeze(2), device)
            self.conv_b = _dev(sd[a + "proj.bias"], device)
            self.adapter_pos = _dev(sd[a + "pos_emb"].detach().float() * (0.0 if lens.disable_adapter_pos else 1.0), device)
        elif lens.modality == "pc":
            if lens.pc_tokenizer == "pnsa":
                from .points import PNSATokenizerTrainer
                self.points = PNSATokenizerTrainer(sd, a, lens, device, gemm_cfg=gemm_cfg, bn_training=False)
            else:
                from .points import PointTokenizerEngine
                self.points = PointTokenizerEngine(sd, a, lens, device, gemm_cfg=gemm_cfg)
        else:
            raise NotImplementedError(lens.modality)
        self.perceiver = None if lens.perceiver_identity else PerceiverEngine(sd, prefix + "perceiver.", lens, device, gemm_cfg)

    def update_params(self, sd, prefix: str, names):
        L, a = self.lens, prefix + "visual_adapter."
        self.vit.update_params(sd, [n for n in names if not n.startswith(("visual_adapter.", "perceiver."))])
        if any(n.startswith("visual_adapter.") for n in names):
            scale = 0.0 if L.disable_adapter_pos else 1.0
            if L.modality in ("depth", "audio"):
                self.conv_w.copy_(conv_weight_as_gemm(sd[a + "conv1.weight"], self.device))
                self.adapter_pos.copy_(sd[a + "pos_emb"].detach().float() * scale)
            elif L.modality == "eeg":
                self.conv_w.copy_(conv_weight_as_gemm(sd[a + "proj.weight"].unsqueeze(2), self.device))
                self.conv_b.copy_(sd[a + "proj.bias"])
                self.adapter_pos.copy_(sd[a + "pos_emb"].detach().float() * scale)
# ... 51 lines not shown
```

vit-lens_amd/vitlens_hip/ops.py:

```python
import ctypes as C
import threading

import torch

from ._lib import load_library, check

F32, BF16, F16 = 0, 1, 2
EPI_BF16, EPI_F32, EPI_RES_F32, EPI_RES_BF16, EPI_GEGLU, EPI_DGELU, EPI_DGEGLU = 0, 1, 2, 3, 5, 6, 7
ACT_NONE, ACT_GELU, ACT_RELU = 0, 1, 2
ACT_GELU_DSAVE = 4
ACT_QGELU = 5
ACT_QGELU_DSAVE = 6


def mlp_act(quick_gelu: bool, dsave: bool = False) -> int:
    if quick_gelu:
        return ACT_QGELU_DSAVE if dsave else ACT_QGELU
    return ACT_GELU_DSAVE if dsave else ACT_GELU
LOG2E = 1.4426950408889634

_lib = load_library()


def _stream():
# ... 48 lines not shown
            raise ValueError("gemm: residual must share out's row stride and dtype")
        if res_div > 1 and res.shape[0] * res_div < M:
            raise ValueError("gemm: broadcast residual has too few rows")
    if bias is not None and (bias.dtype != torch.float32 or bias.numel() != N):
        raise ValueError("gemm: bias must be f32 [N]")
    if out2 is not None and (out2.stride(0) != out.stride(0) * (2 if epi == EPI_GEGLU else 1) or out2.dtype != torch.bfloat16):
        raise ValueError("gemm: out2 must be bf16 with out's row stride (twice that for GEGLU)")
    check(_lib.vl_gemm_bf16_ex(_p(a), _p(w), _p(bias), _p(out), _p(res), _p(out2), M, N, K, a.stride(0), w.stride(0),
                               out.stride(0), float(alpha), epi, act, res_div, cfg, _stream()))
    return out


def gemm_f16(a, w, bias=None, out=None, res=None, epi=EPI_BF16, act=ACT_NONE, alpha=1.0):
    _chk2d(a, "a", torch.float16); _chk2d(w, "w", torch.float16)
    M, K = a.shape
    N = w.shape[0]
    if w.shape[1] != K:
        raise ValueError(f"gemm_f16: K mismatch {a.shape} vs {w.shape}")
    if out is None:
        out = torch.empty(M, N, device=a.device, dtype=torch.float32 if epi == EPI_RES_F32 else torch.float16)
    _chk2d(out, "out", torch.float32 if epi == EPI_RES_F32 else torch.float16)
    if res is not None:
        _chk2d(res, "res", torch.float32)
        if res.stride(0) != out.stride(0):
            raise ValueError("gemm_f16: residual must share out's row stride")
    if bias is not None and (bias.dtype != torch.float32 or bias.numel() != N):
        raise ValueError("gemm_f16: bias must be f32 [N]")
    check(_lib.vl_gemm_f16(_p(a), _p(w), _p(bias), _p(out), _p(res), M, N, K, a.stride(0), w.stride(0), out.stride(0),
                           float(alpha), epi, act, _stream()))
    return out


def gemm_f32(a, w, bias=None, out=None, res=None, act=ACT_NONE, alpha=1.0):
    _chk2d(a, "a", torch.float32); _chk2d(w, "w", torch.float32)
    M, K = a.shape
    N = w.shape[0]
    if w.shape[1] != K:
        raise ValueError(f"gemm_f32: K mismatch {a.shape} vs {w.shape}")
    if out is None:
        out = torch.empty(M, N, device=a.device, dtype=torch.float32)
    _chk2d(out, "out", torch.float32)
    if res is not None:
        _chk2d(res, "res", torch.float32)
        if res.stride(0) != out.stride(0):
            raise ValueError("gemm_f32: residual must share out's row stride")
    if bias is not None and (bias.dtype != torch.float32 or bias.numel() != N):
        raise ValueError("gemm_f32: bias must be f32 [N]")
    check(_lib.vl_gemm_f32(_p(a), _p(w), _p(bias), _p(out), _p(res), M, N, K, a.stride(0), w.stride(0), out.stride(0),
                           float(alpha), act, _stream()))
    return out


def attn_fwd_f32(q, k, v, out, lse=None, causal=False, scale=1.0):
    import ctypes
    B, H, Lq, dh = q.shape
    Lk = k.shape[2]
    vals = []
    for t in (q, k, v):
        if t.dim() != 4 or t.stride(3) != 1 or t.dtype != torch.float32:
            raise ValueError("attn_fwd_f32: operands must be f32 [B,H,L,dh] views with unit last stride")
        vals += [t.stride(0), t.stride(1), t.stride(2)]
    if out.dtype != torch.float32:
        raise TypeError("attn_fwd_f32: out must be f32")
    check(_lib.vl_attn_fwd_f32(_p(q), _p(k), _p(v), (ctypes.c_long * 9)(*vals), _p(out), _p(lse), B, H, Lq, Lk, dh, float(scale),
                               1 if causal else 0, _stream()))
    return out


def gemm_f32_ex(a, w, bias=None, out=None, res=None, act=ACT_NONE, alpha=1.0, res_div=1, res_pre=False, geglu=False):
    _chk2d(a, "a", torch.float32); _chk2d(w, "w", torch.float32)
    M, K = a.shape
    N = w.shape[0]
    if w.shape[1] != K:
        raise ValueError(f"gemm_f32_ex: K mismatch {a.shape} vs {w.shape}")
    if out is None:
        out = torch.empty(M, N // 2 if geglu else N, device=a.device, dtype=torch.float32)
    _chk2d(out, "out", torch.float32)
    if res is not None:
        _chk2d(res, "res", torch.float32)
        if res.stride(0) != out.stride(0):
            raise ValueError("gemm_f32_ex: residual must share out's row stride")
        if res.shape[0] * res_div < M:
            raise ValueError("gemm_f32_ex: residual has too few rows")
    if bias is not None and (bias.dtype != torch.float32 or bias.numel() != N):
        raise ValueError("gemm_f32_ex: bias must be f32 [N]")
    check(_lib.vl_gemm_f32_ex(_p(a), _p(w), _p(bias), _p(out), _p(res), M, N, K, a.stride(0), w.stride(0), out.stride(0),
                              float(alpha), act, int(res_div), 1 if res_pre else 0, 1 if geglu else 0, _stream()))
    return out


def im2col_f32(x, kh, kw, sh, sw, Kp, transpose_hw=False):
    if x.dtype != torch.float32 or not x.is_contiguous():
        raise ValueError("im2col_f32: need contiguous f32 input")
    N, Cc = x.shape[0], x.shape[1]
    H, W = (x.shape[3], x.shape[2]) if transpose_hw else (x.shape[2], x.shape[3])
    gh, gw = (H - kh) // sh + 1, (W - kw) // sw + 1
    out = torch.empty(N * gh * gw, Kp, device=x.device, dtype=torch.float32)
    check(_lib.vl_im2col_f32(_p(x), _p(out), N, Cc, H, W, kh, kw, sh, sw, Kp, 1 if transpose_hw else 0, _stream()))
    return out, gh, gw


def fold_ln_linear(w, b, gamma, beta):
    w = w.detach().float()
    wg = (w * gamma.detach().float()[None, :]).to(torch.bfloat16).contiguous()
    c = wg.float().sum(1).contiguous()
    d = (b.detach().float() + (w * beta.detach().float()[None, :]).sum(1)).contiguous()
    return wg, d, c


def _fold_rows(x, out, N, K):
    M = x.shape[0]
    if x.dtype != torch.bfloat16 or out.dtype != torch.bfloat16 or K < 512 or K % 64 or N % 256 or x.stride(0) % 8 or out.stride(0) % 8:
        return 0
    if x.data_ptr() % 16 or out.data_ptr() % 16:
        return 0
    return int(_lib.vl_gemm_main_rows(M, N))


def _leftover_cfg(rows, N, cfg):
    if cfg >= 0 or rows > 512:
        return cfg
    return 11 if ((rows + 63) // 64) * ((N + 63) // 64) >= 192 else 9


def gemm_lnfold(x, fold, mean, rstd, out, w, b, ln_w, ln_b, h_ws, act=ACT_NONE, out2=None, eps=1e-5, cfg=-1, h_ready=False):
    wg, d, c = fold
    M, K = x.shape
    N = wg.shape[0]
    mm = _fold_rows(x, out, N, K)
    if mm:
        check(_lib.vl_gemm_lnfold_bf16(_p(x), _p(wg), _p(d), _p(c), _p(mean), _p(rstd), _p(out), _p(out2), mm, N, K,
                                       x.stride(0), wg.stride(0), out.stride(0), act, _stream()))
    if mm < M:
        r = M - mm
        h = h_ws[:r]
        if not h_ready:
            layernorm(x[mm:], ln_w, ln_b, h, r, K, x_row_stride=x.stride(0), mean=mean[mm:], rstd=rstd[mm:], eps=eps)
        gemm(h, w, b, out=out[mm:], epi=EPI_BF16, act=act, cfg=_leftover_cfg(r, N, cfg) if mm else cfg,
             out2=None if out2 is None else out2[mm:])
    return out


def gemm_res_rowstats(a, w, b, out, res, part, cfg=-1):
    M, K = a.shape
    N = w.shape[0]
    mm = _fold_rows(a, out, N, K) if (res.dtype == torch.bfloat16 and res.stride(0) == out.stride(0) and res.data_ptr() % 16 == 0
                                      and part.numel() >= M * (N // 64) * 2) else 0
    if mm:
        check(_lib.vl_gemm_res_rowstats_bf16(_p(a), _p(w), _p(b), _p(out), _p(res), _p(part), mm, N, K, a.stride(0), w.stride(0),
                                             out.stride(0), _stream()))
    if mm < M:
        gemm(a[mm:], w, b, out=out[mm:], res=res[mm:], epi=EPI_RES_BF16, cfg=_leftover_cfg(M - mm, N, cfg) if mm else cfg)
    return mm


def fold_rows(x, out, N):
    return _fold_rows(x, out, N, x.shape[1])


def ln_row_stats(part, x, m_main, mean, rstd, eps=1e-5, ln_w=None, ln_b=None, h_left=None, h_row0=None):
    rows, D = x.shape
    if h_left is not None:
        if h_row0 is None or h_row0 < m_main or h_left.dtype != torch.bfloat16 or h_left.shape[0] < rows - h_row0:
            raise ValueError("ln_row_stats: h_left needs h_row0 >= m_main and a bf16 buffer of at least rows - h_row0 rows")
    check(_lib.vl_ln_row_stats(_p(part) if m_main else None, D // 64, _p(x), x.stride(0), D, m_main, rows, float(eps), _p(mean),
                               _p(rstd), _p(ln_w), _p(ln_b), _p(h_left), h_left.stride(0) if h_left is not None else 0,
                               int(h_row0 or 0), _stream()))


def logits_gemm(xb, yb, scale):
    Cn = yb.shape[0]
    Cp = (Cn + 3) // 4 * 4
    if Cp != Cn:
        yb = torch.cat([yb, torch.zeros(Cp - Cn, yb.shape[1], device=yb.device, dtype=yb.dtype)], 0)
    out = gemm(xb, yb, None, epi=EPI_F32, alpha=scale)
    return out if Cp == Cn else out[:, :Cn]


def gemm_dw(dyt, xt, g, cfg=-1, alpha=1.0):
    _chk2d(dyt, "dyt", torch.bfloat16); _chk2d(xt, "xt", torch.bfloat16); _chk2d(g, "g", torch.float32)
    M, K = dyt.shape
    N = xt.shape[0]
    nk = K // 64
    if K % 64 == 0 and M % 256 == 0 and N % 256 == 0 and nk >= 64:
        t256 = (M // 256) * (N // 256)
        for splits in (1, 2, 4, 8, 16):
            if nk % splits == 0 and t256 * splits >= 192 and nk // splits >= 16:
                ws = torch.empty(splits * M * N, device=g.device, dtype=torch.float32)
                check(_lib.vl_gemm_splitk_accum_f32(_p(dyt), _p(xt), _p(g), M, N, K, dyt.stride(0), xt.stride(0), g.stride(0),
                                                    float(alpha), splits, _p(ws), _stream()))
                return g
    tiles = ((M + 127) // 128) * ((N + 127) // 128)
    if K % 64 == 0 and tiles * 2 <= 256 and nk >= 32:
        splits = max(1, min(512 // tiles, nk // 16))
        if splits > 1:
            ws = torch.empty(splits * M * N, device=g.device, dtype=torch.float32)
            check(_lib.vl_gemm_splitk_accum_f32(_p(dyt), _p(xt), _p(g), M, N, K, dyt.stride(0), xt.stride(0), g.stride(0),
                                                float(alpha), splits, _p(ws), _stream()))
            return g
    return gemm(dyt, xt, None, out=g, res=g, epi=EPI_RES_F32, cfg=cfg, alpha=alpha)


def gemm_dw_tn(dy, x, g, alpha=1.0):
    if dy.dtype != torch.bfloat16 or x.dtype != torch.bfloat16 or g.dtype != torch.float32 or dy.dim() != 2 or x.dim() != 2:
        return False
    R, M = dy.shape
    N = x.shape[1]
    if x.shape[0] != R or R % 64 or M % 256 or N % 256 or dy.stride(1) != 1 or x.stride(1) != 1 or g.stride(1) != 1:
        return False
    if dy.stride(0) % 8 or x.stride(0) % 8 or g.stride(0) % 4 or dy.data_ptr() % 16 or x.data_ptr() % 16 or tuple(g.shape) != (M, N):
        return False
    splits = tn_splits(R // 64, (M // 256) * (N // 256))
    if not splits:
        return False
    ws = torch.empty(splits * M * N, device=g.device, dtype=torch.float32)
    check(_lib.vl_gemm_tn_splitk_accum_f32(_p(dy), _p(x), _p(g), M, N, R, dy.stride(0), x.stride(0), g.stride(0),
                                           float(alpha), splits, _p(ws), _stream()))
    return True


def tn_splits(nk: int, tiles: int, few_tiles_ok: bool = False) -> int:
    valid = lambda splits: (nk // splits >= 16 and nk - (-(-nk // (-(-nk // splits))) - 1) * (-(-nk // splits)) >= 4)
    cands = (1, 2, 4, 8, 16, 32, 64) if few_tiles_ok else (1, 2, 4, 8, 16)
    best = 0
    for splits in cands:
        if not valid(splits):
            continue
        if tiles * splits >= 192:
            return splits
        best = splits
    return best if few_tiles_ok else 0


_pad_cache = {}


def _zero_padded(t, cols, tag):
    key = (tag, t.device, torch.cuda.current_stream(t.device).cuda_stream, threading.get_ident(), t.shape[0], t.shape[1], cols)
    buf = _pad_cache.get(key)
    if buf is None:
        buf = torch.zeros(t.shape[0], cols, device=t.device, dtype=torch.bfloat16)
        _pad_cache[key] = buf
    buf[:, :t.shape[1]].copy_(t)
    return buf


def gemm_dw_tn_any(dy, x, g, alpha=1.0):
    if dy.dtype != torch.bfloat16 or x.dtype != torch.bfloat16 or g.dtype != torch.float32 or dy.dim() != 2 or x.dim() != 2:
        return False
    R, M = dy.shape
    N = x.shape[1]
    if x.shape[0] != R or R % 64 or tuple(g.shape) != (M, N) or dy.stride(1) != 1 or x.stride(1) != 1:
        return False
    Mp, Np = (M + 255) // 256 * 256, (N + 255) // 256 * 256
    if Mp == M and Np == N and gemm_dw_tn(dy, x, g, alpha):
        return True
    if dy.stride(0) % 8 or x.stride(0) % 8 or dy.data_ptr() % 16 or x.data_ptr() % 16:
        return False
    splits = tn_splits(R // 64, (Mp // 256) * (Np // 256), few_tiles_ok=True)
    if not splits:
        return False
    dyp = dy if Mp == M else _zero_padded(dy, Mp, "dy")
    xp = x if Np == N else _zero_padded(x, Np, "x")
    direct = Mp == M and Np == N and g.stride(1) == 1 and g.stride(0) % 4 == 0
    gp = g if direct else torch.zeros(Mp, Np, device=g.device, dtype=torch.float32)
    ws = torch.empty(splits * Mp * Np, device=g.device, dtype=torch.float32)
    check(_lib.vl_gemm_tn_splitk_accum_f32(_p(dyp), _p(xp), _p(gp), Mp, Np, R, dyp.stride(0), xp.stride(0), gp.stride(0),
                                           float(alpha), splits, _p(ws), _stream()))
    if not direct:
        g += gp[:M, :N]
    return True


def _bhld_strides(*views):
    import ctypes
    vals = []
    for t in views:
        if t.dim() != 4 or t.stride(3) != 1 or t.dtype != views[0].dtype or t.dtype not in (torch.bfloat16, torch.float16):
            raise ValueError("attention operands must be bf16 (or, forward only, fp16) [B,H,L,dh] views of one dtype with unit last stride")
        vals += [t.stride(0), t.stride(1), t.stride(2)]
    return (ctypes.c_long * len(vals))(*vals)


def heads_view(x2d, B, L, H, dh, col0=0):
    W = x2d.stride(0)
    return x2d.as_strided((B, H, L, dh), (L * W, dh, W, 1), x2d.storage_offset() + col0)


def attn_fwd(q, k, v, out, lse=None, causal=False, qscale=1.0):
    B, H, Lq, dh = q.shape
    Lk = k.shape[2]
    st = _bhld_strides(q, k, v)
    if q.dtype == torch.float16:
        if k.dtype != q.dtype or v.dtype != q.dtype or out.dtype != q.dtype:
            raise TypeError("attn_fwd: fp16 q needs fp16 k, v and out")
        check(_lib.vl_attn_fwd_f16(_p(q), _p(k), _p(v), st, _p(out), _p(lse), B, H, Lq, Lk, dh, float(qscale),
                                   1 if causal else 0, _stream()))
        return out
    check(_lib.vl_attn_fwd_bf16(_p(q), _p(k), _p(v), st, _p(out), _p(lse), B, H, Lq, Lk, dh, float(qscale),
                                1 if causal else 0, _stream()))
    return out


def layernorm(x, w, b, out, rows, D, x_row_stride=None, row_index=None, row_mul=0, mean=None, rstd=None,
              eps=1e-5):
    xs = D if x_row_stride is None else x_row_stride
    check(_lib.vl_layernorm_fwd(_p(x), _dt(x), xs, _p(row_index), row_mul, _p(w), _p(b), _p(out), _dt(out),
                                out.stride(-2) if out.dim() >= 2 else D, _p(mean), _p(rstd), rows, D,
                                float(eps), _stream()))
    return out


def assemble_ln_pre(tokens, cls, pos, pos2, w, b, out, B, T, D, eps=1e-5, xpre=None, mean=None, rstd=None):
    check(_lib.vl_assemble_ln_pre(_p(tokens), _dt(tokens), _p(cls), _p(pos), _p(pos2), _p(w), _p(b), _p(out),
                                  _dt(out), _p(xpre), _p(mean), _p(rstd), B, T, D, float(eps), _stream()))
    return out


def l2_normalize(x, out=None, out_bf16=None, norms=None, eps=1e-12):
    _chk2d(x, "x", torch.float32)
    if out is None:
        out = torch.empty_like(x)
    check(_lib.vl_l2_normalize(_p(x), _p(out), _p(out_bf16), _p(norms), x.shape[0], x.shape[1], float(eps),
                               _stream()))
    return out


def l2_normalize_bwd(f, df, norms, eps=1e-12):
    dx = torch.empty_like(f)
    check(_lib.vl_l2_normalize_bwd(_p(f), _p(df), _p(norms), _p(dx), f.shape[0], f.shape[1], float(eps),
                                   _stream()))
    return dx


def im2col(x, kh, kw, sh, sw, Kp, transpose_hw=False, out=None):
    if x.dtype != torch.float32 or not x.is_contiguous():
        raise ValueError("im2col: need contiguous f32 input")
    N, Cc = x.shape[0], x.shape[1]
    H, W = (x.shape[3], x.shape[2]) if transpose_hw else (x.shape[2], x.shape[3])
    gh, gw = (H - kh) // sh + 1, (W - kw) // sw + 1
    if out is None:
        out = torch.empty(N * gh * gw, Kp, device=x.device, dtype=torch.bfloat16)
    check(_lib.vl_im2col_bf16(_p(x), _p(out), N, Cc, H, W, kh, kw, sh, sw, Kp, 1 if transpose_hw else 0,
                              _stream()))
    return out, gh, gw


def text_embed(ids, tok_emb, pos, out):
    B, L = ids.shape
    check(_lib.vl_text_embed(_p(ids), _p(tok_emb), _p(pos), _p(out), _dt(out), B, L, tok_emb.shape[1],
                             tok_emb.shape[0], _stream()))
    return out


def cast_bf16(x, out=None):
    if out is None:
        out = torch.empty(x.shape, device=x.device, dtype=torch.bfloat16)
    check(_lib.vl_cast_f32_bf16(_p(x), _p(out), x.numel(), _stream()))
    return out


def add_rows(x, table, out, rows, T, D):
    check(_lib.vl_add_rows(_p(x), _dt(x), _p(table), _p(out), _dt(out), rows, T, D, _stream()))
    return out


def transpose_to_bf16(x, ldo=None, out=None):
    _chk2d(x, "x")
    R, Cc = x.shape
    ldo = R if ldo is None else ldo
    if out is None:
        out = torch.empty(Cc, ldo, device=x.device, dtype=torch.bfloat16)
    check(_lib.vl_transpose_to_bf16(_p(x), _dt(x), x.stride(0), R, Cc, _p(out), ldo, _stream()))
    return out


def transpose_colsum(x, ldo, colsum_out=None, scale=1.0, out=None):
    _chk2d(x, "x")
    R, Cc = x.shape
    ok = Cc % 64 == 0 and ldo % 8 == 0 and x.stride(0) % 8 == 0 and R >= 256 and x.data_ptr() % 16 == 0
    if not ok:
        out = transpose_to_bf16(x, ldo=ldo, out=out)
        if colsum_out is not None:
            colsum(x, colsum_out, scale)
        return out
    if out is None:
        out = torch.empty(Cc, ldo, device=x.device, dtype=torch.bfloat16)
    ws = _ws_for(x.device, ldo, Cc, 1) if colsum_out is not None else None
    check(_lib.vl_transpose_colsum_bf16(_p(x), _dt(x), x.stride(0), R, Cc, _p(out), ldo, _p(colsum_out), float(scale), _p(ws),
                                        _stream()))
    return out


def split_bf16x3(x, pattern):
    _chk2d(x, "x", torch.float32)
    out = torch.empty(x.shape[0], 3 * x.shape[1], device=x.device, dtype=torch.bfloat16)
    check(_lib.vl_split_bf16x3(_p(x.contiguous()), _p(out), x.shape[0], x.shape[1], pattern, _stream()))
    return out


def _chk_sim(logits, sim, thres, who):
    if thres is None:
        raise ValueError(f"{who}: sim needs thres")
    if not torch.is_tensor(sim) or sim.dtype != torch.float32 or sim.dim() != 2 or tuple(sim.shape) != tuple(logits.shape):
        raise ValueError(f"{who}: sim must be an f32 tensor of the logits' shape {tuple(logits.shape)}")
    if sim.device != logits.device or sim.stride(1) != 1:
        raise ValueError(f"{who}: sim must live on the logits' device with contiguous rows")


def ce_stats(logits, label_off=0, want_cols=True, sim=None, thres=None):
    _chk2d(logits, "logits", torch.float32)
    if sim is None and thres is not None:
        raise ValueError("ce_stats: thres needs sim")
    if sim is not None:
        _chk_sim(logits, sim, thres, "ce_stats")
    R, Cc = logits.shape
    dev = logits.device
    row_lse = torch.empty(R, device=dev, dtype=torch.float32)
    diag = torch.empty(R, device=dev, dtype=torch.float32)
    col_lse = torch.empty(Cc, device=dev, dtype=torch.float32) if want_cols else None
    ws = torch.empty(2 * ((R + 63) // 64) * Cc, device=dev, dtype=torch.float32) if want_cols else None
    if sim is None:
        check(_lib.vl_ce_stats(_p(logits), logits.stride(0), R, Cc, label_off, _p(row_lse), _p(col_lse), _p(diag),
                               _p(ws), _stream()))
    else:
        check(_lib.vl_ce_stats_masked(_p(logits), logits.stride(0), R, Cc, label_off, _p(row_lse), _p(col_lse), _p(diag),
                                      _p(ws), _p(sim), sim.stride(0), float(thres), _stream()))
    return row_lse, col_lse, diag


def ce_loss_accum(loss, row_lse, col_lse, diag, R, Cc, label_off, w_row, w_col):
    check(_lib.vl_ce_loss_accum(_p(row_lse), _p(col_lse), _p(diag), R, Cc, label_off, float(w_row), float(w_col),
                                _p(loss), _stream()))


def ce_grad(logits, row_lse, col_lse, label_off, w_row, w_col, logit_scale, dscale, need_g=True, need_gt=True, sim=None,
            thres=None):
    if sim is None and thres is not None:
        raise ValueError("ce_grad: thres needs sim")
    if sim is not None:
        _chk2d(logits, "logits", torch.float32)
        _chk_sim(logits, sim, thres, "ce_grad")
    R, Cc = logits.shape
    dev = logits.device
    ldg = (Cc + 63) // 64 * 64
    ldgt = (R + 63) // 64 * 64
    G = torch.empty(R, ldg, device=dev, dtype=torch.bfloat16) if need_g else None
    GT = torch.empty(Cc, ldgt, device=dev, dtype=torch.bfloat16) if need_gt else None
    ws = None
    if dscale is not None:
        ws = torch.empty(int(_lib.vl_ce_grad_ws_floats(R, Cc, ldg if need_g else 0, ldgt if need_gt else 0)), device=dev,
                         dtype=torch.float32)
    if sim is None:
        check(_lib.vl_ce_grad(_p(logits), logits.stride(0), R, Cc, label_off, _p(row_lse), _p(col_lse), float(w_row),
                              float(w_col), _p(G), ldg, _p(GT), ldgt, float(logit_scale), _p(dscale), _p(ws), _stream()))
    else:
        check(_lib.vl_ce_grad_masked(_p(logits), logits.stride(0), R, Cc, label_off, _p(row_lse), _p(col_lse), float(w_row),
                                     float(w_col), _p(G), ldg, _p(GT), ldgt, float(logit_scale), _p(dscale), _p(ws), _p(sim),
                                     sim.stride(0), float(thres), _stream()))
    return G, GT


def device_info(device=0):
    arch = C.create_string_buffer(64)
    cus, clk, mem = C.c_int(), C.c_int(), C.c_long()
    check(_lib.vl_device_info(device, arch, 64, C.byref(cus), C.byref(clk), C.byref(mem)))
    return {"arch": arch.value.decode(), "cus": cus.value, "clock_khz": clk.value, "hbm_bytes": mem.value}


def layernorm_bwd(dy, x, mean, rstd, w, rows, D, dres=None, dx=None, dx_bf16=None, x_row_stride=None,
                  dy_row_stride=None, dx_row_stride=None):
    g = dx if dx is not None else dres
    gdt = F32 if g is None else _dt(g)
    if dres is not None and dx is not None and dres.dtype != dx.dtype:
        raise TypeError("layernorm_bwd: dres and dx must share a dtype")
    check(_lib.vl_layernorm_bwd_g(_p(dy), _dt(dy), D if dy_row_stride is None else dy_row_stride, _p(x), _dt(x),
                                  D if x_row_stride is None else x_row_stride, _p(mean), _p(rstd), _p(w), _p(dres),
                                  _p(dx), gdt, _p(dx_bf16), D if dx_row_stride is None else dx_row_stride, rows, D, _stream()))


_colreduce_ws = {}


def _ws_for(device, rows, cols, planes):
    need = int(_lib.vl_colreduce_ws_floats(rows, cols, planes))
    key = (device, torch.cuda.current_stream(device).cuda_stream, threading.get_ident())
    t = _colreduce_ws.get(key)
    if t is None or t.numel() < need:
        t = torch.empty(need, device=device, dtype=torch.float32)
        _colreduce_ws[key] = t
    return t


def layernorm_bwd_params(dy, x, mean, rstd, dw, db, rows, D, x_row_stride=None, dy_row_stride=None):
    ws = _ws_for(dy.device, rows, D, 2)
    check(_lib.vl_layernorm_bwd_params(_p(dy), _dt(dy), D if dy_row_stride is None else dy_row_stride, _p(x), _dt(x),
                                       D if x_row_stride is None else x_row_stride, _p(mean), _p(rstd), _p(dw), _p(db),
                                       rows, D, _p(ws), _stream()))


def colsum(a, out, scale=1.0):
    _chk2d(a, "a")
    ws = _ws_for(a.device, a.shape[0], a.shape[1], 1)
    check(_lib.vl_colsum(_p(a), _dt(a), a.stride(0), _p(out), a.shape[0], a.shape[1], float(scale), _p(ws), _stream()))


def geglu_bf16(h, out):
    check(_lib.vl_geglu_bf16(_p(h), _p(out), h.shape[0], h.shape[1] // 2, _stream()))
    return out


def gelu_bf16(u, out):
    check(_lib.vl_gelu_bf16(_p(u), _p(out), u.numel(), _stream()))
    return out


def attn_bwd(q, k, v, dO, o, lse, delta, dq, dk, dv, ld_dq, ld_dkv, causal=False, softmax_scale=None, qscale=None, fused=None):
    B, H, Lq, dh = q.shape
    Lk = k.shape[2]
    scale = dh ** -0.5 if softmax_scale is None else softmax_scale
    qs = scale * LOG2E if qscale is None else qscale
    st = _bhld_strides(q, k, v, dO, o)
    if fused is None:
        fused = bool(_lib.vl_attn_bwd_fused_supported(Lq, Lk, dh, 1 if causal else 0))
    if fused:
        if Lq != Lk or causal:
            raise ValueError("attn_bwd(fused=True): self-attention without a causal mask only")
        check(_lib.vl_attn_bwd_fused_bf16(_p(q), _p(k), _p(v), _p(dO), _p(o), st, _p(lse), _p(dq), _p(dk), _p(dv),
                                          ld_dq, ld_dkv, B, H, Lq, dh, float(qs), float(scale), _stream()))
        return
    check(_lib.vl_attn_bwd_bf16(_p(q), _p(k), _p(v), _p(dO), _p(o), st, _p(lse), _p(delta), _p(dq), _p(dk), _p(dv),
                                ld_dq, ld_dkv, B, H, Lq, Lk, dh, float(qs), 1 if causal else 0, float(scale), _stream()))


def adamw_step(p, g, m, v, lr, beta1, beta2, eps, weight_decay, step, grad_scale=1.0):
    for t in (p, g, m, v):
        if t.dtype != torch.float32 or not t.is_contiguous():
            raise ValueError("adamw_step: contiguous f32 tensors required")
    check(_lib.vl_adamw_step(_p(p), _p(g), _p(m), _p(v), p.numel(), float(lr), float(beta1), float(beta2), float(eps),
                             float(weight_decay), int(step), float(grad_scale), _stream()))


ADAMW_MAX_SLOTS = 1024
_sumsq_ws = {}


def grad_sumsq(flat, out=None):
    if flat.dtype != torch.float32 or not flat.is_contiguous():
        raise ValueError("grad_sumsq: contiguous f32 tensor required")
    if not flat.is_cuda:
        raise RuntimeError("vitlens_hip ops need GPU tensors (no CPU fallback)")
    if out is None:
        out = torch.empty(1, device=flat.device, dtype=torch.float32)
    elif out.dtype != torch.float32 or out.numel() != 1 or out.device != flat.device:
        raise ValueError("grad_sumsq: out must be one f32 element on the input's device")
    key = (flat.device, torch.cuda.current_stream(flat.device).cuda_stream)
    ws = _sumsq_ws.get(key)
    if ws is None:
        ws = _sumsq_ws[key] = torch.empty(int(_lib.vl_sumsq_ws_floats()) // 2, device=flat.device, dtype=torch.float64)
    check(_lib.vl_sumsq_f32(_p(flat) if flat.numel() else None, flat.numel(), _p(out), _p(ws), _stream()))
    return out


def adamw_multi(slots, nslots, lr, beta1, beta2, eps, step, grad_scale, max_norm, sumsq, norm_out=None):
    if slots.dtype != torch.int64 or slots.dim() != 2 or slots.shape[1] != 6 or not slots.is_contiguous():
        raise ValueError("adamw_multi: slots must be a contiguous int64 [nslots, 6] table")
    if not 0 <= int(nslots) <= min(slots.shape[0], ADAMW_MAX_SLOTS):
        raise ValueError(f"adamw_multi: nslots {nslots} outside the table of {slots.shape[0]} rows (at most {ADAMW_MAX_SLOTS} per launch)")
    if sumsq.dtype != torch.float32 or sumsq.numel() != 1:
        raise ValueError("adamw_multi: sumsq must be one f32 element")
    if norm_out is not None and (norm_out.dtype != torch.float32 or norm_out.numel() != 1):
        raise ValueError("adamw_multi: norm_out must be one f32 element")
    if not float(max_norm) > 0.0:
        raise ValueError(f"adamw_multi: max_norm must be positive, got {max_norm}")
    if int(step) < 1:
        raise ValueError("adamw_multi: step counts from 1")
    check(_lib.vl_adamw_multi_step(_p(slots), int(nslots), float(lr), float(beta1), float(beta2), float(eps), int(step),
                                   float(grad_scale), float(max_norm), _p(sumsq), _p(norm_out), _stream()))


def clamp_scalar(p, lo, hi):
    check(_lib.vl_clamp_scalar(_p(p), float(lo), float(hi), _stream()))


def axpy(y, x, alpha=1.0):
    check(_lib.vl_axpy_f32(_p(y), _p(x), float(alpha), y.numel(), _stream()))


def scale_exp(x, log_scale, out=None, mul=1.0):
    if x.dtype != torch.float32 or not x.is_contiguous() or log_scale.dtype != torch.float32:
        raise ValueError("scale_exp: contiguous f32 tensors required")
    out = torch.empty_like(x) if out is None else out
    check(_lib.vl_scale_exp_f32(_p(x), _p(out), x.numel(), _p(log_scale), float(mul), _stream()))
    return out


def batch_rowsum(x, out, B, T, D, batch_stride_rows, row_offset):
    check(_lib.vl_batch_rowsum(_p(x), _p(out), B, T, D, batch_stride_rows, row_offset, _stream()))


def fps(xyz, start, G, want_centers=True):
    B, N, _ = xyz.shape
    idx = torch.empty(B, G, device=xyz.device, dtype=torch.int64)
    centers = torch.empty(B, G, 3, device=xyz.device, dtype=torch.float32) if want_centers else None
    check(_lib.vl_fps(_p(xyz.contiguous()), _p(start.contiguous()), _p(idx), _p(centers), B, N, G, _stream()))
    return idx, centers


def pc_gather_normalize(pts, idx=None):
    B, N, Cc = pts.shape
    G = N if idx is None else idx.shape[1]
    out = torch.empty(B, G, Cc, device=pts.device, dtype=torch.float32)
    check(_lib.vl_pc_gather_normalize(_p(pts.contiguous()), _p(idx.contiguous() if idx is not None else None), _p(out), B, N, G, Cc,
                                      _stream()))
    return out


def knn_group(xyz, center_idx, k, Kp=64, want_idx=False):
    B, N, _ = xyz.shape
    G = center_idx.shape[1]
    nidx = torch.empty(B, G, k, device=xyz.device, dtype=torch.int32) if want_idx else None
    patches = torch.empty(B * G * k, Kp, device=xyz.device, dtype=torch.bfloat16)
    check(_lib.vl_knn_group(_p(xyz.contiguous()), _p(center_idx.contiguous()), _p(nidx), _p(patches), B, N, G, k, Kp, _stream()))
    return patches, nidx


def ball_group(xyz, feats, center_idx, radius, nsample, Kp=64, want_idx=False):
    import numpy as np
    B, N, _ = xyz.shape
    S = center_idx.shape[1]
    D = 0 if feats is None else feats.shape[2]
    idx = torch.empty(B, S, nsample, device=xyz.device, dtype=torch.int32) if want_idx else None
    patches = torch.empty(B * S * nsample, Kp, device=xyz.device, dtype=torch.bfloat16)
    check(_lib.vl_ball_group(_p(xyz.contiguous()), _p(feats.contiguous() if feats is not None else None), _p(center_idx.contiguous()),
                             _p(idx), _p(patches), B, N, S, D, float(np.float32(float(radius) ** 2)), nsample, Kp, _stream()))
    return patches, idx


def group_max(x, M, out_dtype=torch.bfloat16):
    _chk2d(x, "x", torch.bfloat16)
    groups = x.shape[0] // M
    out = torch.empty(groups, x.shape[1], device=x.device, dtype=out_dtype)
    check(_lib.vl_group_max(_p(x), x.stride(0), _p(out), _dt(out), out.stride(0), groups, M, x.shape[1], _stream()))
    return out


def pad3(c, Kp=64):
    c = c.reshape(-1, 3).contiguous()
    out = torch.empty(c.shape[0], Kp, device=c.device, dtype=torch.bfloat16)
    check(_lib.vl_pad3_bf16(_p(c), _p(out), c.shape[0], Kp, _stream()))
    return out


def knn_group_f32(xyz, center_idx, k, Kp=4, want_idx=False, out=None):
    B, N, _ = xyz.shape
    G = center_idx.shape[1]
    nidx = torch.empty(B, G, k, device=xyz.device, dtype=torch.int32) if want_idx else None
    patches = torch.empty(B * G * k, Kp, device=xyz.device, dtype=torch.float32) if out is None else out
    if patches.dtype != torch.float32 or not patches.is_contiguous() or tuple(patches.shape) != (B * G * k, Kp):
        raise ValueError(f"knn_group_f32: out must be contiguous f32 [{B * G * k}, {Kp}]")
    check(_lib.vl_knn_group_f32(_p(xyz.contiguous()), _p(center_idx.contiguous()), _p(nidx), _p(patches), B, N, G, k, Kp,
                                _stream()))
    return patches, nidx


def group_max_f32(x, M, out=None):
    _chk2d(x, "x", torch.float32)
    groups = x.shape[0] // M
    if out is None:
        out = torch.empty(groups, x.shape[1], device=x.device, dtype=torch.float32)
    _chk2d(out, "out", torch.float32)
    check(_lib.vl_group_max_f32(_p(x), x.stride(0), _p(out), out.stride(0), groups, M, x.shape[1], _stream()))
    return out


def pad3_f32(c, Kp=4):
    c = c.reshape(-1, 3).contiguous()
    out = torch.empty(c.shape[0], Kp, device=c.device, dtype=torch.float32)
    check(_lib.vl_pad3_f32(_p(c), _p(out), c.shape[0], Kp, _stream()))
    return out


def _bn_chunks(R):
    return max(1, min(1024, R // 64))


def bn_stats(x, running_mean=None, running_var=None, momentum=0.1):
    _chk2d(x, "x", torch.bfloat16)
    R, C = x.shape
    n = _bn_chunks(R)
    ws = torch.empty((n + 1) * 2 * C, device=x.device, dtype=torch.float32)
    mean = torch.empty(C, device=x.device, dtype=torch.float32); var = torch.empty_like(mean)
    check(_lib.vl_bn_stats(_p(x), x.stride(0), R, C, _p(ws), n, _p(mean), _p(var), _p(running_mean), _p(running_var),
                           momentum, _stream()))
    return mean, var


def bn_apply(x, mean, var, gamma, beta, eps=1e-5, relu=False, out=None):
    _chk2d(x, "x", torch.bfloat16)
    out = torch.empty_like(x) if out is None else out
    check(_lib.vl_bn_apply(_p(x), x.stride(0), _p(mean), _p(var), _p(gamma), _p(beta), eps, int(relu), _p(out), out.stride(0),
                           x.shape[0], x.shape[1], _stream()))
    return out


def bn_bwd(dy, x, mean, var, gamma, beta, dgamma, dbeta, eps=1e-5, relu=False, train=True, need_dx=True):
    _chk2d(dy, "dy", torch.bfloat16); _chk2d(x, "x", torch.bfloat16)
    R, C = x.shape
    n = _bn_chunks(R)
    ws = torch.empty((n + 1) * 2 * C, device=x.device, dtype=torch.float32)
    dx = torch.empty_like(x) if need_dx else None
    check(_lib.vl_bn_bwd(_p(dy), dy.stride(0), _p(x), x.stride(0), _p(mean), _p(var), _p(gamma), _p(beta), eps, int(relu),
                         int(train), _p(ws), n, _p(dgamma), _p(dbeta), _p(dx), dx.stride(0) if need_dx else 0, R, C, _stream()))
    return dx


def bn_stats_local(x):
    _chk2d(x, "x", torch.bfloat16)
    R, C = x.shape
    n = _bn_chunks(R)
    ws = torch.empty((n + 1) * 2 * C, device=x.device, dtype=torch.float32)
    local = torch.empty(2 * C + 1, device=x.device, dtype=torch.float32)
    check(_lib.vl_bn_stats_local(_p(x), x.stride(0), R, C, _p(ws), n, _p(local), _stream()))
    return local


def bn_stats_merge(gathered, running_mean=None, running_var=None, momentum=0.1):
    W, n = gathered.shape
    Cc = (n - 1) // 2
    mean = torch.empty(Cc, device=gathered.device, dtype=torch.float32); var = torch.empty_like(mean)
    total = torch.empty(1, device=gathered.device, dtype=torch.int32)
    check(_lib.vl_bn_stats_merge(_p(gathered.contiguous()), W, Cc, _p(mean), _p(var), _p(running_mean), _p(running_var), momentum,
                                 _p(total), _stream()))
    return mean, var, total


def bn_bwd_reduce(dy, x, mean, var, gamma, beta, dgamma, dbeta, eps=1e-5, relu=False):
    _chk2d(dy, "dy", torch.bfloat16); _chk2d(x, "x", torch.bfloat16)
    R, C = x.shape
    n = _bn_chunks(R)
    ws = torch.empty((n + 1) * 2 * C, device=x.device, dtype=torch.float32)
    sums = torch.empty(2 * C, device=x.device, dtype=torch.float32)
    check(_lib.vl_bn_bwd_reduce(_p(dy), dy.stride(0), _p(x), x.stride(0), _p(mean), _p(var), _p(gamma), _p(beta), eps, int(relu),
                                _p(ws), n, _p(dgamma), _p(dbeta), _p(sums), R, C, _stream()))
    return sums


def bn_bwd_apply(dy, x, mean, var, gamma, beta, sums, total, eps=1e-5, relu=False):
    _chk2d(dy, "dy", torch.bfloat16); _chk2d(x, "x", torch.bfloat16)
    R, C = x.shape
    dx = torch.empty_like(x)
    check(_lib.vl_bn_bwd_apply(_p(dy), dy.stride(0), _p(x), x.stride(0), _p(mean), _p(var), _p(gamma), _p(beta), eps, int(relu),
                               _p(sums), _p(total), _p(dx), dx.stride(0), R, C, _stream()))
    return dx


def group_max_bwd(f, dg, M, base=None):
    _chk2d(f, "f", torch.bfloat16); _chk2d(dg, "dg", torch.bfloat16)
    out = torch.empty_like(f)
    check(_lib.vl_group_max_bwd(_p(f), f.stride(0), _p(dg), dg.stride(0), _p(base), base.stride(0) if base is not None else 0,
                                _p(out), out.stride(0), f.shape[0] // M, M, f.shape[1], _stream()))
    return out


def group_sum(x, M):
    _chk2d(x, "x", torch.bfloat16)
    out = torch.empty(x.shape[0] // M, x.shape[1], device=x.device, dtype=torch.bfloat16)
    check(_lib.vl_group_sum(_p(x), x.stride(0), _p(out), out.stride(0), x.shape[0] // M, M, x.shape[1], _stream()))
    return out
```

vit-lens_amd/vitlens_hip/train.py:

```python
from typing import Dict, Iterable, Optional

import torch

from . import ops
from . import engine as _engine
from .engine import VitEngine

BF = torch.bfloat16


class _Saved:

    def __init__(self, B, L, D, H, hidden, layers, device, res_dtype=torch.float32, keep_blocks=(), checkpoint=False):
        dh = D // H
        T = B * L
        Lp = (L + 7) // 8 * 8
        f32 = lambda *s: torch.empty(*s, device=device, dtype=torch.float32)
        bf = lambda *s: torch.empty(*s, device=device, dtype=BF)
        self.Lp = Lp
        xres = f32 if res_dtype == torch.float32 else bf

        def per_layer(make):
            if not checkpoint:
                return [make() for _ in range(layers)]
            one = make()
            return [one] * layers
        mids = per_layer(lambda: xres(T, D))
        self.X = [None] * (2 * layers + 1)
        for l in range(layers):
            self.X[2 * l] = xres(T, D); self.X[2 * l + 1] = mids[l]
        self.X[2 * layers] = xres(T, D)
        self.stats = per_layer(lambda: [f32(T) for _ in range(4)])
        self.qkv = per_layer(lambda: bf(T, 3 * D))
        hv = lambda m, i=0: ops.heads_view(m, B, L, H, dh, i * D)
        self.q = [hv(m, 0) for m in self.qkv]; self.k = [hv(m, 1) for m in self.qkv]; self.v = [hv(m, 2) for m in self.qkv]
        self.a = per_layer(lambda: bf(T, D))
        self.av = [hv(m) for m in self.a]
        self.lse = per_layer(lambda: f32(B, H, L))
        self.u = per_layer(lambda: bf(T, hidden))
        self.h = bf(T, D); self.hid = bf(T, hidden)
        if checkpoint and keep_blocks:
            k1, k2, k3 = bf(T, D), bf(T, D), bf(T, hidden)
            self.h1 = {l: k1 for l in keep_blocks}; self.h2 = {l: k2 for l in keep_blocks}; self.hidk = {l: k3 for l in keep_blocks}
        else:
            self.h1 = {l: bf(T, D) for l in keep_blocks}; self.h2 = {l: bf(T, D) for l in keep_blocks}
            self.hidk = {l: bf(T, hidden) for l in keep_blocks}
        self.part = f32(T * (D // 64) * 2) if (D % 64 == 0 and res_dtype == BF) else None
        self.part_of, self.part_rows = None, 0
        self.xpre = f32(T, D); self.pre_stats = [f32(T), f32(T)]
        self.post_stats = [f32(B), f32(B)]
        self.pooled = bf(B, D)
        self.dx = xres(T, D); self.dxb = bf(T, D) if res_dtype == torch.float32 else self.dx
        self.du = bf(T, hidden); self.dh = bf(T, D)
        self.dOm = bf(T, D); self.dO = hv(self.dOm)
        self.delta = f32(B, H, L); self.dqkv = bf(T, 3 * D)


class TowerTrainer:
    def __init__(self, eng: VitEngine, train_blocks: Iterable[int] = (), train_cls=False, train_pos=False,
                 param_prefix: str = "visual.", train_ln_pre=False, train_ln_post=False, train_proj=False, checkpoint=False):
        self.eng, self.prefix = eng, param_prefix
        self.causal = False
        self.checkpoint = bool(checkpoint)
        self.train_blocks = sorted(set(train_blocks))
        self.train_cls, self.train_pos = train_cls, train_pos
        self.train_ln_pre, self.train_ln_post, self.train_proj = train_ln_pre, train_ln_post, train_proj
        c = eng.cfg
        self.D, self.H, self.hidden, self.layers = c.width, c.heads, int(c.width * c.mlp_ratio), c.layers
        self.act_dsave = ops.mlp_act(bool(getattr(c, "quick_gelu", False)), dsave=True)
        dev = eng.device
        self.wT = [{k: w[k].t().contiguous() for k in ("in_w", "out_w", "fc_w", "proj_w")} for w in eng.blocks]
        self.proj = eng.projT.t().contiguous() if eng.projT is not None else None
        self._saved = {}
        self.grads: Dict[str, torch.Tensor] = {}
        self.ctx = None

    def refresh_derived(self, blocks=(), proj=False):
        for l in blocks:
            for k in ("in_w", "out_w", "fc_w", "proj_w"):
                self.wT[l][k].copy_(self.eng.blocks[l][k].t())
        if proj and self.proj is not None:
            self.proj.copy_(self.eng.projT.t())

    def saved(self, B, L):
        key = (B, L)
        if key not in self._saved:
            self._saved[key] = _Saved(B, L, self.D, self.H, self.hidden, self.layers, self.eng.device, self.eng.res_dtype,
                                      keep_blocks=tuple(self.train_blocks), checkpoint=self.checkpoint)
        return self._saved[key]

    def grad_buffer(self, name, like):
        g = self.grads.get(name)
        if g is None:
            g = torch.zeros(like.shape, device=self.eng.device, dtype=torch.float32)
            self.grads[name] = g
        return g

    def zero_grads(self):
        for g in self.grads.values():
            g.zero_()

    def forward(self, tokens: torch.Tensor, B: int, pos2: Optional[torch.Tensor] = None) -> torch.Tensor:
        e, D, H = self.eng, self.D, self.H
        T = tokens.shape[0] // B
        L = T + 1
        dh = D // H
        S = self.saved(B, L)
        cfg = e.gemm_cfg
        res_epi = ops.EPI_RES_F32 if e.res_dtype == torch.float32 else ops.EPI_RES_BF16
        ops.assemble_ln_pre(tokens, e.cls, e.pos, pos2, e.ln_pre[0], e.ln_pre[1], S.X[0], B, T, D,
                            xpre=S.xpre, mean=S.pre_stats[0], rstd=S.pre_stats[1])
        for l in range(self.layers):
            self._block_forward(S, l, B, L)
        xl = S.X[2 * self.layers]
        ops.layernorm(xl, e.ln_post[0], e.ln_post[1], S.pooled, B, D, x_row_stride=L * D,
                      mean=S.post_stats[0], rstd=S.post_stats[1])
        if e.projT is None:
            feat = S.pooled.float()
        else:
            feat = ops.gemm(S.pooled, e.projT, None, epi=ops.EPI_F32, cfg=cfg)
        self.ctx = (B, L, tokens, pos2 is not None)
        return feat

    def _block_forward(self, S, l, B, L, write_out=True):
        e, D, H = self.eng, self.D, self.H
        dh = D // H
        cfg = e.gemm_cfg
        res_epi = ops.EPI_RES_F32 if e.res_dtype == torch.float32 else ops.EPI_RES_BF16
        w = e.blocks[l]
        m1, r1, m2, r2 = S.stats[l]
        h1, h2, hid = S.h1.get(l, S.h), S.h2.get(l, S.h), S.hidk.get(l, S.hid)
        fold_ok = _engine.LN_FOLD and S.part is not None
        folded = fold_ok and "in_f" in w and l not in self.train_blocks
        next_folded = (fold_ok and l + 1 < self.layers and "in_f" in e.blocks[l + 1] and (l + 1) not in self.train_blocks)
        if folded:
            x0, x1 = S.X[2 * l], S.X[2 * l + 1]
            mm0 = S.part_rows if S.part_of is x0 else 0
            S.part_of = None
            r_in, r_fc = ops.fold_rows(x0, S.qkv[l], 3 * D), ops.fold_rows(x1, hid, hid.shape[1])
            k_in = dict(ln_w=w["ln1_w"], ln_b=w["ln1_b"], h_left=S.h, h_row0=r_in) if mm0 <= r_in else {}
            ops.ln_row_stats(S.part, x0, mm0, m1, r1, **k_in)
            ops.gemm_lnfold(x0, w["in_f"], m1, r1, S.qkv[l], w["in_w"], w["in_b"], w["ln1_w"], w["ln1_b"], S.h, cfg=cfg,
                            h_ready=bool(k_in))
            ops.attn_fwd(S.q[l], S.k[l], S.v[l], S.a[l], lse=S.lse[l], causal=self.causal, qscale=dh ** -0.5 * ops.LOG2E)
            mm = ops.gemm_res_rowstats(S.a[l], w["out_w"], w["out_b"], x1, x0, S.part, cfg=cfg)
            k_fc = dict(ln_w=w["ln2_w"], ln_b=w["ln2_b"], h_left=S.h, h_row0=r_fc) if mm <= r_fc else {}
            ops.ln_row_stats(S.part, x1, mm, m2, r2, **k_fc)
            ops.gemm_lnfold(x1, w["fc_f"], m2, r2, hid, w["fc_w"], w["fc_b"], w["ln2_w"], w["ln2_b"], S.h,
                            act=self.act_dsave, out2=S.u[l], cfg=cfg, h_ready=bool(k_fc))
        else:
            ops.layernorm(S.X[2 * l], w["ln1_w"], w["ln1_b"], h1, B * L, D, mean=m1, rstd=r1)
            ops.gemm(h1, w["in_w"], w["in_b"], out=S.qkv[l], epi=ops.EPI_BF16, cfg=cfg)
            ops.attn_fwd(S.q[l], S.k[l], S.v[l], S.a[l], lse=S.lse[l], causal=self.causal, qscale=dh ** -0.5 * ops.LOG2E)
            ops.gemm(S.a[l], w["out_w"], w["out_b"], out=S.X[2 * l + 1], res=S.X[2 * l], epi=res_epi, cfg=cfg)
            ops.layernorm(S.X[2 * l + 1], w["ln2_w"], w["ln2_b"], h2, B * L, D, mean=m2, rstd=r2)
            ops.gemm(h2, w["fc_w"], w["fc_b"], out=hid, epi=ops.EPI_BF16, act=self.act_dsave, cfg=cfg, out2=S.u[l])
        if write_out:
            S.part_of, S.part_rows = None, 0
            if next_folded:
                S.part_rows = ops.gemm_res_rowstats(hid, w["proj_w"], w["proj_b"], S.X[2 * l + 2], S.X[2 * l + 1], S.part, cfg=cfg)
                S.part_of = S.X[2 * l + 2]
            else:
                ops.gemm(hid, w["proj_w"], w["proj_b"], out=S.X[2 * l + 2], res=S.X[2 * l + 1], epi=res_epi, cfg=cfg)

    def _dw(self, name, dy, x, rows, bias_name=None):
        g = self.grad_buffer(name, torch.empty(dy.shape[1], x.shape[1]))
        rp = (rows + 63) // 64 * 64
        gb = self.grad_buffer(bias_name, torch.empty(dy.shape[1])) if bias_name else None
        if rows == dy.shape[0] == x.shape[0] and ops.gemm_dw_tn(dy, x, g):
            if gb is not None:
                ops.colsum(dy, gb)
            return
        dyt = ops.transpose_colsum(dy, rp, colsum_out=gb)
        xt = ops.transpose_colsum(x, rp)
        ops.gemm_dw(dyt, xt, g, cfg=self.eng.gemm_cfg)

    def backward(self, dfeat: torch.Tensor, on_block_done=None) -> torch.Tensor:
        e, D, H = self.eng, self.D, self.H
        B, L, tokens, has_pos2 = self.ctx
        dh = D // H
        T = L - 1
        S = self.saved(B, L)
        rows = B * L
        cfg = e.gemm_cfg
        P = self.prefix
        dfb = ops.cast_bf16(dfeat.contiguous())
        dpooled = dfb if self.proj is None else ops.gemm(dfb, self.proj, None, epi=ops.EPI_BF16, cfg=cfg)
        if self.train_proj and self.proj is not None:
            bp = (B + 63) // 64 * 64
            ops.gemm_dw(ops.transpose_to_bf16(S.pooled, ldo=bp), ops.transpose_to_bf16(dfb, ldo=bp),
                        self.grad_buffer(P + "proj", torch.empty(D, dfeat.shape[1])), cfg=cfg)
        if self.train_ln_post:
            ops.layernorm_bwd_params(dpooled, S.X[2 * self.layers], S.post_stats[0], S.post_stats[1],
                                     self.grad_buffer(P + "ln_post.weight", e.ln_post[0]),
                                     self.grad_buffer(P + "ln_post.bias", e.ln_post[1]), B, D, x_row_stride=L * D)
        S.dx.zero_()
        ops.layernorm_bwd(dpooled, S.X[2 * self.layers], S.post_stats[0], S.post_stats[1], e.ln_post[0], B, D,
                          dx=S.dx, x_row_stride=L * D, dx_row_stride=L * D)
        self._blocks_backward(S, B, L, on_block_done)
        dxpre = torch.empty(S.dx.shape, device=S.dx.device, dtype=torch.float32)
        if self.train_ln_pre:
            ops.layernorm_bwd_params(S.dx, S.xpre, S.pre_stats[0], S.pre_stats[1], self.grad_buffer(P + "ln_pre.weight", e.ln_pre[0]),
                                     self.grad_buffer(P + "ln_pre.bias", e.ln_pre[1]), rows, D)
        ops.layernorm_bwd(S.dx, S.xpre, S.pre_stats[0], S.pre_stats[1], e.ln_pre[0], rows, D, dx=dxpre)
        if self.train_cls:
            ops.batch_rowsum(dxpre, self.grad_buffer(P + "class_embedding", e.cls).view(1, D), B, 1, D, L, 0)
        if self.train_pos:
            ops.batch_rowsum(dxpre, self.grad_buffer(P + "positional_embedding", e.pos), B, L, D, L, 0)
        self.dxpre = dxpre
        return dxpre.view(B, L, D)[:, 1:, :].reshape(B * T, D)

    def _blocks_backward(self, S, B, L, on_block_done=None):
        e, D, H = self.eng, self.D, self.H
        rows = B * L
        cfg = e.gemm_cfg
        P = self.prefix
        f32_stream = S.dx.dtype == torch.float32
        dxb_out = S.dxb if f32_stream else None
        if f32_stream:
            ops.cast_bf16(S.dx, out=S.dxb)
        for l in reversed(range(self.layers)):
            if self.checkpoint:
                self._block_forward(S, l, B, L, write_out=False)
            w, wT = e.blocks[l], self.wT[l]
            m1, r1, m2, r2 = S.stats[l]
            trainable = l in self.train_blocks
            bp = f"{P}transformer.resblocks.{l}."
            ops.gemm(S.dxb, wT["proj_w"], None, out=S.du, res=S.u[l], epi=ops.EPI_DGELU, act=self.act_dsave, cfg=cfg)
            if trainable:
                self._dw(bp + "mlp.c_proj.weight", S.dx, S.hidk[l], rows, bp + "mlp.c_proj.bias")
                self._dw(bp + "mlp.c_fc.weight", S.du, S.h2[l], rows, bp + "mlp.c_fc.bias")
            ops.gemm(S.du, wT["fc_w"], None, out=S.dh, epi=ops.EPI_BF16, cfg=cfg)
            if trainable:
                ops.layernorm_bwd_params(S.dh, S.X[2 * l + 1], m2, r2, self.grad_buffer(bp + "ln_2.weight", w["ln2_w"]),
                                         self.grad_buffer(bp + "ln_2.bias", w["ln2_b"]), rows, D)
            ops.layernorm_bwd(S.dh, S.X[2 * l + 1], m2, r2, w["ln2_w"], rows, D, dres=S.dx, dx=S.dx, dx_bf16=dxb_out)
            if trainable:
                self._dw(bp + "attn.out_proj.weight", S.dx, S.a[l], rows, bp + "attn.out_proj.bias")
            ops.gemm(S.dxb, wT["out_w"], None, out=S.dOm, epi=ops.EPI_BF16, cfg=cfg)
            ops.attn_bwd(S.q[l], S.k[l], S.v[l], S.dO, S.av[l], S.lse[l], S.delta,
                         S.dqkv, S.dqkv[:, D:], S.dqkv[:, 2 * D:], 3 * D, 3 * D, causal=self.causal)
            if trainable:
                self._dw(bp + "attn.in_proj_weight", S.dqkv, S.h1[l], rows, bp + "attn.in_proj_bias")
            ops.gemm(S.dqkv, wT["in_w"], None, out=S.dh, epi=ops.EPI_BF16, cfg=cfg)
            if trainable:
                ops.layernorm_bwd_params(S.dh, S.X[2 * l], m1, r1, self.grad_buffer(bp + "ln_1.weight", w["ln1_w"]),
                                         self.grad_buffer(bp + "ln_1.bias", w["ln1_b"]), rows, D)
            ops.layernorm_bwd(S.dh, S.X[2 * l], m1, r1, w["ln1_w"], rows, D, dres=S.dx, dx=S.dx, dx_bf16=dxb_out)
            if trainable and on_block_done is not None:
                on_block_done(l)


def conv_weight_grad(dtok: torch.Tensor, cols: torch.Tensor, g: torch.Tensor, gemm_cfg: int = -1):
    if ops.gemm_dw_tn_any(ops.cast_bf16(dtok.contiguous()), cols, g):
        return
    rp = (dtok.shape[0] + 63) // 64 * 64
    ops.gemm_dw(ops.transpose_to_bf16(dtok, ldo=rp), ops.transpose_to_bf16(cols, ldo=rp), g, cfg=gemm_cfg)


class DepthLensTrainer:

    def __init__(self, lens_engine, unlock_first_n: int = 4, tower_kw=None):
        self.le = lens_engine
        kw = dict(train_blocks=range(unlock_first_n)) if tower_kw is None else dict(tower_kw)
        self.tower = TowerTrainer(lens_engine.vit, param_prefix="visual.", **kw)
        self.ctx = None

    @property
    def grads(self):
        return self.tower.grads

    def forward(self, x: torch.Tensor) -> torch.Tensor:
        le = self.le
        p = le.tower.patch
        cols, gh, gw = ops.im2col(x.contiguous().float(), p, p, p, p, le.conv_w.shape[1])
        tok = ops.gemm(cols, le.conv_w, None, epi=ops.EPI_BF16, cfg=le.gemm_cfg)
        self.ctx = (cols, x.shape[0])
        return self.tower.forward(tok, x.shape[0], pos2=le.adapter_pos)

    def backward(self, dfeat: torch.Tensor, on_block_done=None):
        cols, B = self.ctx
        dtok = self.tower.backward(dfeat, on_block_done)
        T, D = dtok.shape[0] // B, dtok.shape[1]
        t = self.tower
        g = t.grad_buffer("visual.visual_adapter.conv1.weight_gemm", torch.empty(D, cols.shape[1]))
        conv_weight_grad(dtok, cols, g, self.le.gemm_cfg)
        ops.batch_rowsum(t.dxpre, t.grad_buffer("visual.visual_adapter.pos_emb", self.le.adapter_pos), B, T, D, T + 1, 1)


class ImageTowerTrainer:

    def __init__(self, vit_engine, tower_kw=None, train_conv: bool = False):
        self.eng = vit_engine
        self.tower = TowerTrainer(vit_engine, param_prefix="visual.", **(tower_kw or {}))
        self.train_conv = train_conv
        self.ctx = None

    @property
    def grads(self):
        return self.tower.grads

    def forward(self, x: torch.Tensor) -> torch.Tensor:
        e = self.eng
        p = e.cfg.patch
        cols, gh, gw = ops.im2col(x.contiguous().float(), p, p, p, p, e.conv_w.shape[1])
        tok = ops.gemm(cols, e.conv_w, None, epi=ops.EPI_BF16, cfg=e.gemm_cfg)
        self.ctx = cols
        return self.tower.forward(tok, x.shape[0])

    def backward(self, dfeat: torch.Tensor):
        dtok = self.tower.backward(dfeat)
        if self.train_conv:
            cols = self.ctx
            g = self.tower.grad_buffer("visual.conv1.weight_gemm", torch.empty(dtok.shape[1], cols.shape[1]))
            conv_weight_grad(dtok, cols, g, self.eng.gemm_cfg)


class _TextAsTower:

    def __init__(self, te):
        from types import SimpleNamespace
        c = te.cfg
        self.cfg = SimpleNamespace(width=c.width, heads=c.heads, mlp_ratio=4.0, layers=c.layers, quick_gelu=c.quick_gelu)
        self.device, self.res_dtype, self.gemm_cfg = te.device, torch.float32, te.gemm_cfg
        self.blocks, self.projT, self.ln_post = te.blocks, te.projT, te.ln_final
        self.tok, self.pos = te.tok, te.pos


class TextTowerTrainer(TowerTrainer):

    def __init__(self, text_engine):
        if getattr(text_engine, "arith", "bf16") != "bf16":
            raise ValueError("TextTowerTrainer needs a TextEngine(arith='bf16')")
        eng = _TextAsTower(text_engine)
        super().__init__(eng, train_blocks=range(eng.cfg.layers), param_prefix="", train_ln_post=True, train_proj=True)
        self.causal = True

    def forward(self, text: torch.Tensor) -> torch.Tensor:
        e, D = self.eng, self.D
        B, L = text.shape
        S = self.saved(B, L)
        text = text.to(e.device).contiguous()
        ops.text_embed(text, e.tok, e.pos, S.X[0])
        for l in range(self.layers):
            self._block_forward(S, l, B, L)
        eot = text.argmax(dim=-1).contiguous()
        ops.layernorm(S.X[2 * self.layers], e.ln_post[0], e.ln_post[1], S.pooled, B, D, x_row_stride=D, row_index=eot, row_mul=L,
                      mean=S.post_stats[0], rstd=S.post_stats[1])
        feat = ops.gemm(S.pooled, e.projT, None, epi=ops.EPI_F32, cfg=e.gemm_cfg)
        self.ctx = (B, L, text, eot)
        return feat

    def backward(self, dfeat: torch.Tensor):
        e, D = self.eng, self.D
        B, L, text, eot = self.ctx
        S = self.saved(B, L)
        cfg = e.gemm_cfg
        dfb = ops.cast_bf16(dfeat.contiguous())
        dpooled = ops.gemm(dfb, self.proj, None, epi=ops.EPI_BF16, cfg=cfg)
        bp = (B + 63) // 64 * 64
        ops.gemm_dw(ops.transpose_to_bf16(S.pooled, ldo=bp), ops.transpose_to_bf16(dfb, ldo=bp),
                    self.grad_buffer("text_projection", torch.empty(D, dfeat.shape[1])), cfg=cfg)
        rows = torch.arange(B, device=e.device) * L + eot
        x_eot = S.X[2 * self.layers].index_select(0, rows).contiguous()
        ops.layernorm_bwd_params(dpooled, x_eot, S.post_stats[0], S.post_stats[1], self.grad_buffer("ln_final.weight", e.ln_post[0]),
                                 self.grad_buffer("ln_final.bias", e.ln_post[1]), B, D)
        dx_eot = torch.empty(B, D, device=e.device, dtype=torch.float32)
        ops.layernorm_bwd(dpooled, x_eot, S.post_stats[0], S.post_stats[1], e.ln_post[0], B, D, dx=dx_eot)
        S.dx.zero_()
        S.dx.index_copy_(0, rows, dx_eot)
        self._blocks_backward(S, B, L)
        ops.batch_rowsum(S.dx, self.grad_buffer("positional_embedding", e.pos), B, L, D, L, 0)
        self.grad_buffer("token_embedding.weight", e.tok).index_add_(0, text.reshape(-1), S.dx)


def clip_coef(sumsq: torch.Tensor, max_norm: float, grad_scale: float = 1.0) -> torch.Tensor:
    norm = torch.sqrt(sumsq.float()) * float(grad_scale)
    return torch.clamp(max_norm / (norm + 1e-6), max=1.0)


def clip_grad_norm_(flat_or_tensors, max_norm: float) -> torch.Tensor:
    if not float(max_norm) > 0.0:
        raise ValueError(f"clip_grad_norm_: max_norm must be positive, got {max_norm}")
    if torch.is_tensor(flat_or_tensors):
        ts = [flat_or_tensors]
    else:
        ts = [t for t in (flat_or_tensors.values() if isinstance(flat_or_tensors, dict) else flat_or_tensors) if t is not None]
    if not ts:
        raise ValueError("clip_grad_norm_: no tensors")
    parts = [ops.grad_sumsq(t) for t in ts]
    sumsq = parts[0] if len(parts) == 1 else torch.cat(parts).sum(dtype=torch.float64).float().reshape(1)
    coef = clip_coef(sumsq, float(max_norm)).reshape(())
    for t in ts:
        t.mul_(coef)
    return torch.sqrt(sumsq).reshape(())


def pack_adamw_slots(rows) -> torch.Tensor:
    import struct
    t = torch.empty(len(rows), 6, dtype=torch.int64)
    for i, (p, g, m, v, n, wd) in enumerate(rows):
        t[i] = torch.tensor([p, g, m, v, n, struct.unpack("<I", struct.pack("<f", wd))[0]], dtype=torch.int64)
    return t


class AdamW:

    def __init__(self, params: Dict[str, torch.Tensor], lr=5e-4, betas=(0.9, 0.98), eps=1e-6, weight_decay=0.2):
        self._slots, self._slot_key = None, None
        self.last_grad_norm = None
        self.param_groups = [{"lr": lr}]
        self.params, self.betas, self.eps, self.wd = params, betas, eps, weight_decay
        self.m = {k: torch.zeros_like(v) for k, v in params.items()}
        self.v = {k: torch.zeros_like(v) for k, v in params.items()}
        self.t = 0

    @property
    def lr(self) -> float:
        return float(self.param_groups[0]["lr"])

    @lr.setter
    def lr(self, value):
        self.param_groups[0]["lr"] = float(value)

    @staticmethod
    def decays(name: str, p: torch.Tensor) -> bool:
        return not (p.ndim < 2 or "bn" in name or "ln" in name or "bias" in name or "logit_scale" in name)

    def slot_rows(self, grads: Dict[str, torch.Tensor]):
        rows = []
        for k, p in self.params.items():
            g = grads.get(k)
            if g is None:
                continue
            for t in (p, g, self.m[k], self.v[k]):
                if t.dtype != torch.float32 or not t.is_contiguous():
                    raise ValueError(f"AdamW: contiguous f32 tensors required ({k})")
            if g.numel() != p.numel():
                raise ValueError(f"AdamW: gradient of {k} has {g.numel()} elements, the parameter {p.numel()}")
            rows.append((p.data_ptr(), g.data_ptr(), self.m[k].data_ptr(), self.v[k].data_ptr(), p.numel(),
                         self.wd if self.decays(k, p) else 0.0))
        return rows

    def _clipped_step(self, grads, grad_scale, max_norm, sumsq):
        if not float(max_norm) > 0.0:
            raise ValueError(f"AdamW.step: max_norm must be positive, got {max_norm}")
        rows = self.slot_rows(grads)
        if not rows:
            return
        dev = next(iter(self.params.values())).device
        key = tuple(rows)
        if key != self._slot_key:
            self._slots, self._slot_key = pack_adamw_slots(rows).to(dev), key
        if sumsq is None:
            parts = [ops.grad_sumsq(g) for k, g in grads.items() if k in self.params and g is not None]
            sumsq = torch.cat(parts).sum(dtype=torch.float64).float().reshape(1)
        if self.last_grad_norm is None:
            self.last_grad_norm = torch.zeros((), device=dev, dtype=torch.float32)
        self.t += 1
        for a in range(0, len(rows), ops.ADAMW_MAX_SLOTS):
            n = min(ops.ADAMW_MAX_SLOTS, len(rows) - a)
            ops.adamw_multi(self._slots[a:a + n], n, self.lr, self.betas[0], self.betas[1], self.eps, self.t, grad_scale,
                            max_norm, sumsq, self.last_grad_norm)

    def step(self, grads: Dict[str, torch.Tensor], grad_scale: float = 1.0, max_norm: Optional[float] = None,
             sumsq: Optional[torch.Tensor] = None):
        if max_norm is not None:
            return self._clipped_step(grads, grad_scale, max_norm, sumsq)
        self.t += 1
        for k, p in self.params.items():
            g = grads.get(k)
            if g is None:
                continue
            wd = self.wd if self.decays(k, p) else 0.0
            ops.adamw_step(p.view(-1), g.view(-1), self.m[k].view(-1), self.v[k].view(-1), self.lr, self.betas[0],
                           self.betas[1], self.eps, wd, self.t, grad_scale)


class _AttnSaved:

    def __init__(self, B, H, Lq, Lk, dh, device, packed: bool):
        bf = lambda *s: torch.empty(*s, device=device, dtype=BF)
        inner = H * dh
        if packed:
            self.qkv2 = bf(B * Lq, 3 * inner)
            self.q2, self.kv2 = self.qkv2, None
            self.q, self.k, self.v = (ops.heads_view(self.qkv2, B, Lq, H, dh, i * inner) for i in range(3))
        else:
            self.q2, self.kv2 = bf(B * Lq, inner), bf(B * Lk, 2 * inner)
            self.q = ops.heads_view(self.q2, B, Lq, H, dh)
            self.k, self.v = ops.heads_view(self.kv2, B, Lk, H, dh), ops.heads_view(self.kv2, B, Lk, H, dh, inner)
        self.a = bf(B * Lq, inner)
        self.av = ops.heads_view(self.a, B, Lq, H, dh)
        self.lse = torch.empty(B, H, Lq, device=device, dtype=torch.float32)
        self.dOm = bf(B * Lq, inner)
        self.dO = ops.heads_view(self.dOm, B, Lq, H, dh)
        self.delta = torch.empty(B, H, Lq, device=device, dtype=torch.float32)


def deinterleave_geglu(g: torch.Tensor) -> torch.Tensor:
    return torch.cat([g[0::2], g[1::2]], dim=0)


class PerceiverTrainer:
    def __init__(self, pe, param_prefix: str = "visual.perceiver."):
        self.pe, self.P = pe, param_prefix
        c = pe.cfg
        self.grads: Dict[str, torch.Tensor] = {}
        t = lambda w: w.t().contiguous()
        self.wT = []
        for li, lay in enumerate(pe.layers):
            if li >= 2 and lay is pe.layers[1]:
                self.wT.append(self.wT[1])
                continue
            d = {"x": {"q": t(lay["x_attn"]["q_w"]), "kv": t(lay["x_attn"]["kv_w"]), "out": t(lay["x_attn"]["to_out_w"])},
                 "xff": {"w0": t(lay["x_ff"]["w0"]), "w2": t(lay["x_ff"]["w2"])}, "selfs": []}
            for sl in lay["selfs"]:
                d["selfs"].append({"qkv": t(sl["attn"]["qkv_w"]), "out": t(sl["attn"]["to_out_w"]),
                                   "w0": t(sl["ff"]["w0"]), "w2": t(sl["ff"]["w2"])})
            self.wT.append(d)
        self._st = {}

    def refresh_derived(self):
        for li, lay in enumerate(self.pe.layers):
# ... 281 lines not shown
```

Baseline: 1764 modality-pairs/sec.

## Prune last frozen transformer block to CLS-row-only forward and backward

When the last block is frozen and not checkpointed, the forward computes only the CLS query row's attention, out-proj, MLP and residual, since only the pooled CLS token feeds the output. The backward matching the pruned block uses new single-query attention forward and backward kernels, plus a layernorm backward that adds the residual gradient only on every L-th row. This removes most of the final block's attention, MLP GEMM and layernorm work over all tokens, in both forward and backward. Stats buffers are now initialised to identity values, and the dense dQ/dK/dV paths are still written for all rows by the q1 kernel.

New measurement: 1812 modality-pairs/sec (median of 6 runs). 1.03x the previous value.

```diff
diff --git a/include/vitlens_hip.h b/include/vitlens_hip.h
--- a/include/vitlens_hip.h
+++ b/include/vitlens_hip.h
@@ -34,7 +34,7 @@
 #define VL_GEMM_PINGPONG 10
 
 const char* vl_last_error(void);
-#define VL_ABI_VERSION 606
+#define VL_ABI_VERSION 607
 int vl_version(void);
 
 int vl_gemm_bf16(const void* A, const void* W, const float* bias, void* out, const void* res,
@@ -129,6 +129,10 @@
 int vl_layernorm_bwd_g(const void* dy, int dy_dtype, long dy_stride, const void* x, int x_dtype, long x_stride,
                        const float* mean, const float* rstd, const float* w, const void* dres, void* dx, int g_dtype,
                        void* dx_bf16, long dx_stride, int rows, int D, hipStream_t stream);
+int vl_layernorm_bwd_sres(const void* dy, int dy_dtype, long dy_stride, const void* x, int x_dtype, long x_stride,
+                          const float* mean, const float* rstd, const float* w, const void* dres, int dres_every,
+                          long dres_stride, void* dx, int g_dtype, void* dx_bf16, long dx_stride, int rows, int D,
+                          hipStream_t stream);
 long vl_colreduce_ws_floats(int rows, int cols, int planes);
 int vl_layernorm_bwd_params(const void* dy, int dy_dtype, long dy_stride, const void* x, int x_dtype, long x_stride,
                             const float* mean, const float* rstd, float* dw, float* db, int rows, int D,
@@ -143,6 +147,11 @@
 int vl_attn_bwd_fused_bf16(const void* q, const void* k, const void* v, const void* dO, const void* o, const long* strides,
                            const float* lse, void* dq, void* dk, void* dv, long ld_dq, long ld_dkv, int B, int H, int L, int dh,
                            float qscale, float scale, hipStream_t stream);
+int vl_attn_fwd_q1(const void* q, const void* k, const void* v, const long* strides, void* out, long ld_out, float* lse,
+                   int B, int H, int L, int dh, int qrow, float qscale, hipStream_t stream);
+int vl_attn_bwd_q1(const void* q, const void* k, const void* v, const long* strides, const void* dO, long ld_do,
+                   const void* o, long ld_o, const float* lse, void* dq, void* dk, void* dv, long ld_dq, long ld_dkv,
+                   int B, int H, int L, int dh, int qrow, float qscale, float scale, hipStream_t stream);
 int vl_kaldi_fbank(const float* wave, long wave_stride, int batch, long n_samples, const float* window, const float* banks,
                    float* out, int target_len, int win, int shift, int nfft, int nmel, float preemph, float mean, float std,
                    hipStream_t stream);
diff --git a/vit-lens_amd/csrc/vl_attn_pool.hip b/vit-lens_amd/csrc/vl_attn_pool.hip
--- /dev/null
+++ b/vit-lens_amd/csrc/vl_attn_pool.hip
@@ -0,0 +1,238 @@
+#include <stdio.h>
+#include "vl_attn_common.h"
+#include "vitlens_hip.h"
+
+namespace {
+using namespace vlattn;
+
+constexpr int Q1_MAXL = 1024;
+constexpr float Q1_LOG2E = 1.4426950408889634f, Q1_LN2 = 0.6931471805599453f;
+
+struct Q1FwdP {
+  TV q, k, v;
+  bf16_t* o; long ld_o;
+  float* lse;
+  int B, H, L, qrow;
+  float qscale;
+};
+
+struct Q1BwdP {
+  TV q, k, v;
+  const bf16_t* dO; long ld_do;
+  const bf16_t* o; long ld_o;
+  const float* lse;
+  bf16_t *dq, *dk, *dv;
+  long ld_dq, ld_dkv;
+  int B, H, L, qrow;
+  float qscale, scale;
+};
+
+__device__ __forceinline__ void q1_unpack8(u32x4 w, float (&f)[8]) {
+#pragma unroll
+  for (int e = 0; e < 4; ++e) { f[2 * e] = bf2f((bf16_t)(w[e] & 0xffffu)); f[2 * e + 1] = bf2f((bf16_t)(w[e] >> 16)); }
+}
+__device__ __forceinline__ u32x4 q1_pack8(const float (&f)[8]) {
+  u32x4 w;
+#pragma unroll
+  for (int e = 0; e < 4; ++e) w[e] = pack2bf(f[2 * e], f[2 * e + 1]);
+  return w;
+}
+__device__ __forceinline__ float q1_dot8(const float (&a)[8], const float (&b)[8]) {
+  float s = 0.f;
+#pragma unroll
+  for (int e = 0; e < 8; ++e) s = fmaf(a[e], b[e], s);
+  return s;
+}
+__device__ __forceinline__ float q1_sum_c(float v) {
+  v += __shfl_xor(v, 1, 64); v += __shfl_xor(v, 2, 64); v += __shfl_xor(v, 4, 64);
+  return v;
+}
+__device__ __forceinline__ float q1_sum_r(float v) {
+  v += __shfl_xor(v, 8, 64); v += __shfl_xor(v, 16, 64); v += __shfl_xor(v, 32, 64);
+  return v;
+}
+__device__ __forceinline__ void q1_load_q(const TV& q, int b, int h, int qrow, int c, float qscale, float (&q2)[8]) {
+  const bf16_t* Qb = q.p + (long)b * q.sb + (long)h * q.sh + (long)qrow * q.sr;
+  float f[8];
+  q1_unpack8(*(const u32x4*)(Qb + c * 8), f);
+#pragma unroll
+  for (int e = 0; e < 8; ++e) q2[e] = bf2f(f2bf(f[e] * qscale));
+}
+
+__global__ void __launch_bounds__(64) attn_fwd_q1_kernel(const Q1FwdP p) {
+  __shared__ float sS[Q1_MAXL];
+  const int bh = blockIdx.x, b = bh / p.H, h = bh - b * p.H;
+  const int lane = threadIdx.x, r = lane >> 3, c = lane & 7;
+  const int L = p.L;
+  const bf16_t* Kb = p.k.p + (long)b * p.k.sb + (long)h * p.k.sh + c * 8;
+  const bf16_t* Vb = p.v.p + (long)b * p.v.sb + (long)h * p.v.sh + c * 8;
+  float q2[8];
+  q1_load_q(p.q, b, h, p.qrow, c, p.qscale, q2);
+  float mx = -INFINITY;
+  for (int j0 = 0; j0 < L; j0 += 32) {
+    u32x4 kr[4];
+#pragma unroll
+    for (int u = 0; u < 4; ++u) {
+      const int row = j0 + u * 8 + r;
+      kr[u] = *(const u32x4*)(Kb + (long)(row < L ? row : L - 1) * p.k.sr);
+    }
+#pragma unroll
+    for (int u = 0; u < 4; ++u) {
+      const int row = j0 + u * 8 + r;
+      float kf[8];
+      q1_unpack8(kr[u], kf);
+      const float s = q1_sum_c(q1_dot8(q2, kf));
+      if (row < L) {
+        mx = fmaxf(mx, s);
+        if (c == 0) sS[row] = s;
+      }
+    }
+  }
+  mx = wave_max(mx);
+  __syncthreads();
+  float l = 0.f;
+  for (int j = lane; j < L; j += 64) {
+    const float pj = __builtin_amdgcn_exp2f(sS[j] - mx);
+    sS[j] = pj;
+    l += pj;
+  }
+  l = wave_sum(l);
+  __syncthreads();
+  float acc[8];
+#pragma unroll
+  for (int e = 0; e < 8; ++e) acc[e] = 0.f;
+  for (int j0 = 0; j0 < L; j0 += 32) {
+    u32x4 vr[4];
+#pragma unroll
+    for (int u = 0; u < 4; ++u) {
+      const int row = j0 + u * 8 + r;
+      vr[u] = *(const u32x4*)(Vb + (long)(row < L ? row : L - 1) * p.v.sr);
+    }
+#pragma unroll
+    for (int u = 0; u < 4; ++u) {
+      const int row = j0 + u * 8 + r;
+      const float pj = row < L ? sS[row] : 0.f;
+      float vf[8];
+      q1_unpack8(vr[u], vf);
+#pragma unroll
+      for (int e = 0; e < 8; ++e) acc[e] = fmaf(pj, vf[e], acc[e]);
+    }
+  }
+  const float inv = 1.0f / l;
+#pragma unroll
+  for (int e = 0; e < 8; ++e) acc[e] = q1_sum_r(acc[e]) * inv;
+  if (r == 0) *(u32x4*)(p.o + (long)b * p.ld_o + h * 64 + c * 8) = q1_pack8(acc);
+  if (p.lse && lane == 0) p.lse[bh] = (mx + __log2f(l)) * Q1_LN2;
+}
+
+__global__ void __launch_bounds__(64) attn_bwd_q1_kernel(const Q1BwdP p) {
+  const int bh = blockIdx.x, b = bh / p.H, h = bh - b * p.H;
+  const int lane = threadIdx.x, r = lane >> 3, c = lane & 7;
+  const int L = p.L;
+  const bf16_t* Kb = p.k.p + (long)b * p.k.sb + (long)h * p.k.sh + c * 8;
+  const bf16_t* Vb = p.v.p + (long)b * p.v.sb + (long)h * p.v.sh + c * 8;
+  float q2[8], g[8], of[8];
+  q1_load_q(p.q, b, h, p.qrow, c, p.qscale, q2);
+  q1_unpack8(*(const u32x4*)(p.dO + (long)b * p.ld_do + h * 64 + c * 8), g);
+  q1_unpack8(*(const u32x4*)(p.o + (long)b * p.ld_o + h * 64 + c * 8), of);
+  const float delta = q1_sum_c(q1_dot8(g, of));
+  const float nl = -p.lse[bh] * Q1_LOG2E;
+  const long row0 = (long)b * L;
+  bf16_t* dQ = p.dq + h * 64 + c * 8;
+  bf16_t* dK = p.dk + h * 64 + c * 8;
+  bf16_t* dV = p.dv + h * 64 + c * 8;
+  float aq[8];
+#pragma unroll
+  for (int e = 0; e < 8; ++e) aq[e] = 0.f;
+  const u32x4 zero = {0u, 0u, 0u, 0u};
+  for (int j0 = 0; j0 < L; j0 += 32) {
+    u32x4 kr[4], vr[4];
+#pragma unroll
+    for (int u = 0; u < 4; ++u) {
+      const int row = j0 + u * 8 + r;
+      const long rc = row < L ? row : L - 1;
+      kr[u] = *(const u32x4*)(Kb + rc * p.k.sr);
+      vr[u] = *(const u32x4*)(Vb + rc * p.v.sr);
+    }
+#pragma unroll
+    for (int u = 0; u < 4; ++u) {
+      const int row = j0 + u * 8 + r;
+      float kf[8], vf[8];
+      q1_unpack8(kr[u], kf); q1_unpack8(vr[u], vf);
+      const float s = q1_sum_c(q1_dot8(q2, kf));
+      const float dp = q1_sum_c(q1_dot8(g, vf));
+      const float pj = __builtin_amdgcn_exp2f(s + nl);
+      const float ds = pj * (dp - delta);
+      if (row < L) {
+        float dk[8], dv[8];
+        const float dsl = ds * Q1_LN2;
+#pragma unroll
+        for (int e = 0; e < 8; ++e) { dk[e] = dsl * q2[e]; dv[e] = pj * g[e]; aq[e] = fmaf(ds, kf[e], aq[e]); }
+        *(u32x4*)(dK + (row0 + row) * p.ld_dkv) = q1_pack8(dk);
+        *(u32x4*)(dV + (row0 + row) * p.ld_dkv) = q1_pack8(dv);
+        if (row != p.qrow) *(u32x4*)(dQ + (row0 + row) * p.ld_dq) = zero;
+      }
+    }
+  }
+#pragma unroll
+  for (int e = 0; e < 8; ++e) aq[e] = q1_sum_r(aq[e]) * p.scale;
+  if (r == 0) *(u32x4*)(dQ + (row0 + p.qrow) * p.ld_dq) = q1_pack8(aq);
+}
+
+}
+
+extern "C" int vl_set_error(const char* msg);
+
+static const char* q1_check(const long* strides, int nstr, int B, int H, int L, int dh, int qrow) {
+  if (B <= 0 || H <= 0) return "empty problem";
+  if (dh != 64) return "head dim 64 only (the dense kernels take the others)";
+  if (L < 1 || L > Q1_MAXL) return "1 <= L <= 1024 required";
+  if (qrow < 0 || qrow >= L) return "query row index outside [0, L)";
+  if ((long)B * H > 0x7fffffffL) return "too many (batch, head) pairs";
+  if (!strides) return "strides are required";
+  for (int i = 0; i < nstr; ++i)
+    if (strides[i] & 7) return "operand strides must be multiples of 8 elements (16-byte rows)";
+  return nullptr;
+}
+
+extern "C" int vl_attn_fwd_q1(const void* q, const void* k, const void* v, const long* strides, void* out, long ld_out,
+                              float* lse, int B, int H, int L, int dh, int qrow, float qscale, hipStream_t stream) {
+  char msg[160];
+  if (const char* why = q1_check(strides, 9, B, H, L, dh, qrow)) {
+    snprintf(msg, sizeof(msg), "vl_attn_fwd_q1: %s", why);
+    return vl_set_error(msg);
+  }
+  if (!q || !k || !v || !out) return vl_set_error("vl_attn_fwd_q1: null operand");
+  if (((((uintptr_t)q) | ((uintptr_t)k) | ((uintptr_t)v) | ((uintptr_t)out)) & 15) || (ld_out & 7) || ld_out < (long)H * 64)
+    return vl_set_error("vl_attn_fwd_q1: operands must be 16-byte aligned, ld_out a multiple of 8 and >= H * 64");
+  const long* s = strides;
+  Q1FwdP p{TV{(const bf16_t*)q, s[0], s[1], s[2]}, TV{(const bf16_t*)k, s[3], s[4], s[5]}, TV{(const bf16_t*)v, s[6], s[7], s[8]},
+           (bf16_t*)out, ld_out, lse, B, H, L, qrow, qscale};
+  hipLaunchKernelGGL(attn_fwd_q1_kernel, dim3((unsigned)(B * H)), dim3(64), 0, stream, p);
+  const hipError_t e = hipGetLastError();
+  return e == hipSuccess ? 0 : vl_set_error(hipGetErrorString(e));
+}
+
+extern "C" int vl_attn_bwd_q1(const void* q, const void* k, const void* v, const long* strides, const void* dO, long ld_do,
+                              const void* o, long ld_o, const float* lse, void* dq, void* dk, void* dv, long ld_dq, long ld_dkv,
+                              int B, int H, int L, int dh, int qrow, float qscale, float scale, hipStream_t stream) {
+  char msg[160];
+  if (const char* why = q1_check(strides, 9, B, H, L, dh, qrow)) {
+    snprintf(msg, sizeof(msg), "vl_attn_bwd_q1: %s", why);
+    return vl_set_error(msg);
+  }
+  if (!q || !k || !v || !dO || !o || !lse || !dq || !dk || !dv) return vl_set_error("vl_attn_bwd_q1: null operand");
+  if ((((uintptr_t)q) | ((uintptr_t)k) | ((uintptr_t)v) | ((uintptr_t)dO) | ((uintptr_t)o) | ((uintptr_t)dq) | ((uintptr_t)dk) |
+       ((uintptr_t)dv)) & 15)
+    return vl_set_error("vl_attn_bwd_q1: operands and gradient destinations must be 16-byte aligned");
+  if ((ld_do & 7) || (ld_o & 7) || (ld_dq & 7) || (ld_dkv & 7) || ld_do < (long)H * 64 || ld_o < (long)H * 64 ||
+      ld_dq < (long)H * 64 || ld_dkv < (long)H * 64)
+    return vl_set_error("vl_attn_bwd_q1: row strides must be multiples of 8 and >= H * 64");
+  const long* s = strides;
+  Q1BwdP p{TV{(const bf16_t*)q, s[0], s[1], s[2]}, TV{(const bf16_t*)k, s[3], s[4], s[5]}, TV{(const bf16_t*)v, s[6], s[7], s[8]},
+           (const bf16_t*)dO, ld_do, (const bf16_t*)o, ld_o, lse, (bf16_t*)dq, (bf16_t*)dk, (bf16_t*)dv, ld_dq, ld_dkv,
+           B, H, L, qrow, qscale, scale};
+  hipLaunchKernelGGL(attn_bwd_q1_kernel, dim3((unsigned)(B * H)), dim3(64), 0, stream, p);
+  const hipError_t e = hipGetLastError();
+  return e == hipSuccess ? 0 : vl_set_error(hipGetErrorString(e));
+}
diff --git a/vit-lens_amd/csrc/vl_bwd.hip b/vit-lens_amd/csrc/vl_bwd.hip
--- a/vit-lens_amd/csrc/vl_bwd.hip
+++ b/vit-lens_amd/csrc/vl_bwd.hip
@@ -25,6 +25,7 @@
   void* dx; bf16_t* dxb;
   long dys, xs, dxs;
   int rows, D;
+  int dres_every; long dres_s;
 };
 
 template <int NCH, typename TDY, typename TX, typename TG>
@@ -34,7 +35,11 @@
   if (row >= p.rows) return;
   const TDY* dy = (const TDY*)p.dy + (long)row * p.dys;
   const TX* x = (const TX*)p.x + (long)row * p.xs;
-  const TG* dres = p.dres ? (const TG*)p.dres + (long)row * p.dxs : nullptr;
+  const TG* dres = nullptr;
+  if (p.dres) {
+    if (p.dres_every <= 1) dres = (const TG*)p.dres + (long)row * p.dxs;
+    else if (row % p.dres_every == 0) dres = (const TG*)p.dres + (long)(row / p.dres_every) * p.dres_s;
+  }
   TG* dx = p.dx ? (TG*)p.dx + (long)row * p.dxs : nullptr;
   bf16_t* dxb = p.dxb ? p.dxb + (long)row * p.dxs : nullptr;
   const float mu = p.mean[row], rs = p.rstd[row];
@@ -486,11 +491,11 @@
   else hipLaunchKernelGGL((ln_bwd_kernel<0, TDY, TX, TG>), g, b, 0, stream, p);
 }
 
-extern "C" int vl_layernorm_bwd_g(const void* dy, int dy_dtype, long dy_stride, const void* x, int x_dtype, long x_stride,
-                                  const float* mean, const float* rstd, const float* w, const void* dres, void* dx, int g_dtype,
-                                  void* dx_bf16, long dx_stride, int rows, int D, hipStream_t stream) {
+static int ln_bwd_run(const void* dy, int dy_dtype, long dy_stride, const void* x, int x_dtype, long x_stride,
+                      const float* mean, const float* rstd, const float* w, const void* dres, int dres_every, long dres_stride,
+                      void* dx, int g_dtype, void* dx_bf16, long dx_stride, int rows, int D, hipStream_t stream) {
   if (rows <= 0 || D <= 0) return vl_set_error("vl_layernorm_bwd: empty problem");
-  LnBwdP p{dy, x, mean, rstd, w, dres, dx, (bf16_t*)dx_bf16, dy_stride, x_stride, dx_stride, rows, D};
+  LnBwdP p{dy, x, mean, rstd, w, dres, dx, (bf16_t*)dx_bf16, dy_stride, x_stride, dx_stride, rows, D, dres_every, dres_stride};
   const int key = (dy_dtype == VL_BF16 ? 4 : 0) | (x_dtype == VL_BF16 ? 2 : 0) | (g_dtype == VL_BF16 ? 1 : 0);
   switch (key) {
     case 0: ln_bwd_launch<float, float, float>(p, stream); break;
@@ -504,6 +509,23 @@
   }
   VL_HIP_OK(hipGetLastError());
   return 0;
+}
+
+extern "C" int vl_layernorm_bwd_g(const void* dy, int dy_dtype, long dy_stride, const void* x, int x_dtype, long x_stride,
+                                  const float* mean, const float* rstd, const float* w, const void* dres, void* dx, int g_dtype,
+                                  void* dx_bf16, long dx_stride, int rows, int D, hipStream_t stream) {
+  return ln_bwd_run(dy, dy_dtype, dy_stride, x, x_dtype, x_stride, mean, rstd, w, dres, 1, dx_stride, dx, g_dtype, dx_bf16, dx_stride,
+                    rows, D, stream);
+}
+
+extern "C" int vl_layernorm_bwd_sres(const void* dy, int dy_dtype, long dy_stride, const void* x, int x_dtype, long x_stride,
+                                     const float* mean, const float* rstd, const float* w, const void* dres, int dres_every,
+                                     long dres_stride, void* dx, int g_dtype, void* dx_bf16, long dx_stride, int rows, int D,
+                                     hipStream_t stream) {
+  if (!dres || !dx || dres_every < 1) return vl_set_error("vl_layernorm_bwd_sres: dres, dx and dres_every >= 1 are required");
+  if (dres == dx) return vl_set_error("vl_layernorm_bwd_sres: dres must not alias dx");
+  return ln_bwd_run(dy, dy_dtype, dy_stride, x, x_dtype, x_stride, mean, rstd, w, dres, dres_every, dres_stride, dx, g_dtype, dx_bf16,
+                    dx_stride, rows, D, stream);
 }
 
 extern "C" int vl_layernorm_bwd(const void* dy, int dy_dtype, long dy_stride, const void* x, int x_dtype, long x_stride,
diff --git a/vit-lens_amd/vitlens_hip/_lib.py b/vit-lens_amd/vitlens_hip/_lib.py
--- a/vit-lens_amd/vitlens_hip/_lib.py
+++ b/vit-lens_amd/vitlens_hip/_lib.py
@@ -15,7 +15,7 @@
 
 P, I, L, F = C.c_void_p, C.c_int, C.c_long, C.c_float
 
-ABI_VERSION = 606
+ABI_VERSION = 607
 
 SIGNATURES = {
     "vl_version": [],
@@ -80,6 +80,7 @@
     "vl_group_sum": [P, L, P, L, L, I, I, P],
     "vl_layernorm_bwd": [P, I, L, P, I, L, P, P, P, P, P, P, L, I, I, P],
     "vl_layernorm_bwd_g": [P, I, L, P, I, L, P, P, P, P, P, I, P, L, I, I, P],
+    "vl_layernorm_bwd_sres": [P, I, L, P, I, L, P, P, P, P, I, L, P, I, P, L, I, I, P],
     "vl_colreduce_ws_floats": [I, I, I],
     "vl_layernorm_bwd_params": [P, I, L, P, I, L, P, P, P, P, I, I, P, P],
     "vl_colsum": [P, I, L, P, I, I, F, P, P],
@@ -88,6 +89,8 @@
     "vl_attn_bwd_bf16": [P, P, P, P, P, P, P, P, P, P, P, L, L, I, I, I, I, I, F, I, F, P],
     "vl_attn_bwd_fused_supported": [I, I, I, I],
     "vl_attn_bwd_fused_bf16": [P, P, P, P, P, P, P, P, P, P, L, L, I, I, I, I, F, F, P],
+    "vl_attn_fwd_q1": [P, P, P, P, P, L, P, I, I, I, I, I, F, P],
+    "vl_attn_bwd_q1": [P, P, P, P, P, L, P, L, P, P, P, P, L, L, I, I, I, I, I, F, F, P],
     "vl_adamw_step": [P, P, P, P, L, F, F, F, F, F, I, F, P],
     "vl_sumsq_ws_floats": [],
     "vl_sumsq_f32": [P, L, P, P, P],
diff --git a/vit-lens_amd/vitlens_hip/engine.py b/vit-lens_amd/vitlens_hip/engine.py
--- a/vit-lens_amd/vitlens_hip/engine.py
+++ b/vit-lens_amd/vitlens_hip/engine.py
@@ -97,13 +97,40 @@
         self.mean = torch.empty(B * L, device=device, dtype=torch.float32)
         self.rstd = torch.empty(B * L, device=device, dtype=torch.float32)
         self.part = torch.empty(B * L * (D // 64) * 2, device=device, dtype=torch.float32) if D % 64 == 0 else None
+        self.a1 = torch.empty(B, D, device=device, dtype=bf)
+        self.h1 = torch.empty(B, D, device=device, dtype=bf)
+        self.hid1 = torch.empty(B, hidden, device=device, dtype=bf)
 
 
 LN_FOLD = True
 
 
-def run_blocks(blocks, ws: _Workspace, B, L, D, H, causal=False, cfg=-1, fold=None, quick_gelu=False):
+PRUNE_LAST_BLOCK = True
+PRUNE_MAX_L = 1024
+
+
+def prune_last_ok(D, H, res_dtype, L, pooled_only=True, causal=False):
+    return bool(PRUNE_LAST_BLOCK and pooled_only and not causal and res_dtype == torch.bfloat16 and H > 0 and D == 64 * H
+                and 1 <= L <= PRUNE_MAX_L)
+
+
+def cls_rows(x2d, B, L):
+    D = x2d.shape[1]
+    return x2d.as_strided((B, D), (L * D, 1), x2d.storage_offset())
+
+
+def _pooled_block_tail(w, ws, B, L, D, H, act, cfg):
+    xc = cls_rows(ws.x, B, L)
+    ops.attn_fwd_q1(ws.q, ws.k, ws.v, ws.a1, qrow=0, qscale=(D // H) ** -0.5 * ops.LOG2E)
+    ops.gemm(ws.a1, w["out_w"], w["out_b"], out=xc, res=xc, epi=ops.EPI_RES_BF16, cfg=cfg)
+    ops.layernorm(xc, w["ln2_w"], w["ln2_b"], ws.h1, B, D, x_row_stride=L * D)
+    ops.gemm(ws.h1, w["fc_w"], w["fc_b"], out=ws.hid1, epi=ops.EPI_BF16, act=act, cfg=cfg)
+    ops.gemm(ws.hid1, w["proj_w"], w["proj_b"], out=xc, res=xc, epi=ops.EPI_RES_BF16, cfg=cfg)
+
+
+def run_blocks(blocks, ws: _Workspace, B, L, D, H, causal=False, cfg=-1, fold=None, quick_gelu=False, pooled_only=False):
     dh = D // H
+    prune = prune_last_ok(D, H, ws.x.dtype, L, pooled_only, causal)
     act = ops.mlp_act(quick_gelu)
     res_epi = ops.EPI_RES_F32 if ws.x.dtype == torch.float32 else ops.EPI_RES_BF16
     if fold is None:
@@ -116,11 +143,15 @@
         r_in, r_fc = ops.fold_rows(ws.x, ws.qkv, 3 * D), ops.fold_rows(ws.x, ws.hid, ws.hid.shape[1])
     for i, w in enumerate(blocks):
         nxt = i + 1 < len(blocks) and folded[i + 1]
+        pruned = prune and i + 1 == len(blocks)
         if folded[i]:
             k_in = dict(ln_w=w["ln1_w"], ln_b=w["ln1_b"], h_left=ws.h, h_row0=r_in) if mm <= r_in else {}
             ops.ln_row_stats(ws.part, ws.x, mm, ws.mean, ws.rstd, **k_in)
             ops.gemm_lnfold(ws.x, w["in_f"], ws.mean, ws.rstd, ws.qkv, w["in_w"], w["in_b"], w["ln1_w"], w["ln1_b"], ws.h, cfg=cfg,
                             h_ready=bool(k_in))
+            if pruned:
+                _pooled_block_tail(w, ws, B, L, D, H, act, cfg)
+                break
             ops.attn_fwd(ws.q, ws.k, ws.v, ws.a, causal=causal, qscale=dh ** -0.5 * ops.LOG2E)
             mm = ops.gemm_res_rowstats(ws.a, w["out_w"], w["out_b"], ws.x, ws.x, ws.part, cfg=cfg)
             k_fc = dict(ln_w=w["ln2_w"], ln_b=w["ln2_b"], h_left=ws.h, h_row0=r_fc) if mm <= r_fc else {}
@@ -130,6 +161,9 @@
         else:
             ops.layernorm(ws.x, w["ln1_w"], w["ln1_b"], ws.h, B * L, D)
             ops.gemm(ws.h, w["in_w"], w["in_b"], out=ws.qkv, epi=ops.EPI_BF16, cfg=cfg)
+            if pruned:
+                _pooled_block_tail(w, ws, B, L, D, H, act, cfg)
+                break
             ops.attn_fwd(ws.q, ws.k, ws.v, ws.a, causal=causal, qscale=dh ** -0.5 * ops.LOG2E)
             ops.gemm(ws.a, w["out_w"], w["out_b"], out=ws.x, res=ws.x, epi=res_epi, cfg=cfg)
             ops.layernorm(ws.x, w["ln2_w"], w["ln2_b"], ws.h, B * L, D)
@@ -231,7 +265,7 @@
         ws = self.workspace(B, L)
         pos = self.pos if use_orig_pos else torch.zeros_like(self.pos)
         ops.assemble_ln_pre(tokens, self.cls, pos, pos2, self.ln_pre[0], self.ln_pre[1], ws.x, B, T, D)
-        run_blocks(self.blocks, ws, B, L, D, cfg.heads, causal=False, cfg=self.gemm_cfg, quick_gelu=cfg.quick_gelu)
+        run_blocks(self.blocks, ws, B, L, D, cfg.heads, causal=False, cfg=self.gemm_cfg, quick_gelu=cfg.quick_gelu, pooled_only=True)
         pooled = torch.empty(B, D, device=self.device, dtype=torch.bfloat16)
         if self.projT is None:
             pooled = torch.empty(B, D, device=self.device, dtype=torch.float32)
diff --git a/vit-lens_amd/vitlens_hip/ops.py b/vit-lens_amd/vitlens_hip/ops.py
--- a/vit-lens_amd/vitlens_hip/ops.py
+++ b/vit-lens_amd/vitlens_hip/ops.py
@@ -374,6 +374,23 @@
     return out
 
 
+def _q1_rows(t, H, name):
+    if t.dim() != 2 or t.stride(1) != 1 or t.dtype != torch.bfloat16 or t.shape[1] != H * 64:
+        raise ValueError(f"{name}: need a bf16 [B, H*64] matrix with unit column stride, got {tuple(t.shape)} {t.dtype}")
+
+
+def attn_fwd_q1(q, k, v, out, lse=None, qrow=0, qscale=1.0):
+    B, H, L, dh = q.shape
+    if k.shape != q.shape or v.shape != q.shape or q.dtype != torch.bfloat16:
+        raise ValueError("attn_fwd_q1: q, k, v must be bf16 views of one [B,H,L,dh] shape (self-attention)")
+    _q1_rows(out, H, "attn_fwd_q1: out")
+    if out.shape[0] != B or (lse is not None and (lse.dtype != torch.float32 or not lse.is_contiguous() or lse.numel() != B * H)):
+        raise ValueError("attn_fwd_q1: out must have B rows, lse must be a contiguous f32 [B, H]")
+    check(_lib.vl_attn_fwd_q1(_p(q), _p(k), _p(v), _bhld_strides(q, k, v), _p(out), out.stride(0), _p(lse), B, H, L, dh,
+                              int(qrow), float(qscale), _stream()))
+    return out
+
+
 def layernorm(x, w, b, out, rows, D, x_row_stride=None, row_index=None, row_mul=0, mean=None, rstd=None,
               eps=1e-5):
     xs = D if x_row_stride is None else x_row_stride
@@ -551,6 +568,13 @@
                                   _p(dx), gdt, _p(dx_bf16), D if dx_row_stride is None else dx_row_stride, rows, D, _stream()))
 
 
+def layernorm_bwd_sparse_res(dy, x, mean, rstd, w, rows, D, dres, dres_every, dx):
+    if dres.dtype != dx.dtype or dres.dim() != 2 or dres.stride(1) != 1 or dres.shape[0] * dres_every < rows - dres_every + 1:
+        raise ValueError("layernorm_bwd_sparse_res: dres must be a row-major matrix of dx's dtype with one row per dres_every rows")
+    check(_lib.vl_layernorm_bwd_sres(_p(dy), _dt(dy), D, _p(x), _dt(x), D, _p(mean), _p(rstd), _p(w), _p(dres), int(dres_every),
+                                     dres.stride(0), _p(dx), _dt(dx), None, D, rows, D, _stream()))
+
+
 _colreduce_ws = {}
 
 
@@ -605,6 +629,22 @@
                                 ld_dq, ld_dkv, B, H, Lq, Lk, dh, float(qs), 1 if causal else 0, float(scale), _stream()))
 
 
+def attn_bwd_q1(q, k, v, dO, o, lse, dq, dk, dv, ld_dq, ld_dkv, qrow=0, softmax_scale=None):
+    B, H, L, dh = q.shape
+    if k.shape != q.shape or v.shape != q.shape or q.dtype != torch.bfloat16:
+        raise ValueError("attn_bwd_q1: q, k, v must be bf16 views of one [B,H,L,dh] shape (self-attention)")
+    _q1_rows(dO, H, "attn_bwd_q1: dO"); _q1_rows(o, H, "attn_bwd_q1: o")
+    if dO.shape[0] != B or o.shape[0] != B or lse.dtype != torch.float32 or not lse.is_contiguous() or lse.numel() != B * H:
+        raise ValueError("attn_bwd_q1: dO and o must have B rows, lse must be a contiguous f32 [B, H]")
+    for t in (dq, dk, dv):
+        if t.dtype != torch.bfloat16 or t.dim() != 2 or t.shape[0] < B * L or t.shape[1] < H * 64:
+            raise ValueError("attn_bwd_q1: dq / dk / dv must be bf16 [>= B*L, >= H*64] token-major destinations")
+    scale = dh ** -0.5 if softmax_scale is None else softmax_scale
+    check(_lib.vl_attn_bwd_q1(_p(q), _p(k), _p(v), _bhld_strides(q, k, v), _p(dO), dO.stride(0), _p(o), o.stride(0), _p(lse),
+                              _p(dq), _p(dk), _p(dv), ld_dq, ld_dkv, B, H, L, dh, int(qrow), float(scale * LOG2E), float(scale),
+                              _stream()))
+
+
 def adamw_step(p, g, m, v, lr, beta1, beta2, eps, weight_decay, step, grad_scale=1.0):
     for t in (p, g, m, v):
         if t.dtype != torch.float32 or not t.is_contiguous():
diff --git a/vit-lens_amd/vitlens_hip/train.py b/vit-lens_amd/vitlens_hip/train.py
--- a/vit-lens_amd/vitlens_hip/train.py
+++ b/vit-lens_amd/vitlens_hip/train.py
@@ -30,7 +30,9 @@
         for l in range(layers):
             self.X[2 * l] = xres(T, D); self.X[2 * l + 1] = mids[l]
         self.X[2 * layers] = xres(T, D)
-        self.stats = per_layer(lambda: [f32(T) for _ in range(4)])
+        ident = lambda: [torch.zeros(T, device=device), torch.ones(T, device=device), torch.zeros(T, device=device),
+                         torch.ones(T, device=device)]
+        self.stats = per_layer(ident)
         self.qkv = per_layer(lambda: bf(T, 3 * D))
         hv = lambda m, i=0: ops.heads_view(m, B, L, H, dh, i * D)
         self.q = [hv(m, 0) for m in self.qkv]; self.k = [hv(m, 1) for m in self.qkv]; self.v = [hv(m, 2) for m in self.qkv]
@@ -54,6 +56,14 @@
         self.du = bf(T, hidden); self.dh = bf(T, D)
         self.dOm = bf(T, D); self.dO = hv(self.dOm)
         self.delta = f32(B, H, L); self.dqkv = bf(T, 3 * D)
+        self.a1 = bf(B, D); self.lse1 = f32(B, H); self.h2c = bf(B, D); self.stats2c = [f32(B), f32(B)]
+        self.hid1 = bf(B, hidden); self.u1 = bf(B, hidden)
+        self.dxc = bf(B, D); self.du1 = bf(B, hidden); self.dhc = bf(B, D); self.dO1 = bf(B, D)
+
+
+def prunes_last_block(layers, train_blocks, checkpoint, causal, res_dtype, D, H, L) -> bool:
+    return bool(layers > 0 and (layers - 1) not in set(train_blocks) and not checkpoint
+                and _engine.prune_last_ok(D, H, res_dtype, L, True, causal))
 
 
 class TowerTrainer:
@@ -74,6 +84,7 @@
         self._saved = {}
         self.grads: Dict[str, torch.Tensor] = {}
         self.ctx = None
+        self._pruned = False
 
     def refresh_derived(self, blocks=(), proj=False):
         for l in blocks:
@@ -110,8 +121,9 @@
         res_epi = ops.EPI_RES_F32 if e.res_dtype == torch.float32 else ops.EPI_RES_BF16
         ops.assemble_ln_pre(tokens, e.cls, e.pos, pos2, e.ln_pre[0], e.ln_pre[1], S.X[0], B, T, D,
                             xpre=S.xpre, mean=S.pre_stats[0], rstd=S.pre_stats[1])
+        self._pruned = prunes_last_block(self.layers, self.train_blocks, self.checkpoint, self.causal, e.res_dtype, D, H, L)
         for l in range(self.layers):
-            self._block_forward(S, l, B, L)
+            self._block_forward(S, l, B, L, cls_only=self._pruned and l == self.layers - 1)
         xl = S.X[2 * self.layers]
         ops.layernorm(xl, e.ln_post[0], e.ln_post[1], S.pooled, B, D, x_row_stride=L * D,
                       mean=S.post_stats[0], rstd=S.post_stats[1])
@@ -122,7 +134,18 @@
         self.ctx = (B, L, tokens, pos2 is not None)
         return feat
 
-    def _block_forward(self, S, l, B, L, write_out=True):
+    def _cls_tail_forward(self, S, l, B, L):
+        e, D = self.eng, self.D
+        w, cfg = e.blocks[l], e.gemm_cfg
+        x0c, x1c, x2c = (_engine.cls_rows(S.X[i], B, L) for i in (2 * l, 2 * l + 1, 2 * l + 2))
+        ops.attn_fwd_q1(S.q[l], S.k[l], S.v[l], S.a1, lse=S.lse1, qrow=0, qscale=(D // self.H) ** -0.5 * ops.LOG2E)
+        ops.gemm(S.a1, w["out_w"], w["out_b"], out=x1c, res=x0c, epi=ops.EPI_RES_BF16, cfg=cfg)
+        ops.layernorm(x1c, w["ln2_w"], w["ln2_b"], S.h2c, B, D, x_row_stride=L * D, mean=S.stats2c[0], rstd=S.stats2c[1])
+        ops.gemm(S.h2c, w["fc_w"], w["fc_b"], out=S.hid1, epi=ops.EPI_BF16, act=self.act_dsave, cfg=cfg, out2=S.u1)
+        ops.gemm(S.hid1, w["proj_w"], w["proj_b"], out=x2c, res=x1c, epi=ops.EPI_RES_BF16, cfg=cfg)
+        S.part_of, S.part_rows = None, 0
+
+    def _block_forward(self, S, l, B, L, write_out=True, cls_only=False):
         e, D, H = self.eng, self.D, self.H
         dh = D // H
         cfg = e.gemm_cfg
@@ -142,6 +165,8 @@
             ops.ln_row_stats(S.part, x0, mm0, m1, r1, **k_in)
             ops.gemm_lnfold(x0, w["in_f"], m1, r1, S.qkv[l], w["in_w"], w["in_b"], w["ln1_w"], w["ln1_b"], S.h, cfg=cfg,
                             h_ready=bool(k_in))
+            if cls_only:
+                return self._cls_tail_forward(S, l, B, L)
             ops.attn_fwd(S.q[l], S.k[l], S.v[l], S.a[l], lse=S.lse[l], causal=self.causal, qscale=dh ** -0.5 * ops.LOG2E)
             mm = ops.gemm_res_rowstats(S.a[l], w["out_w"], w["out_b"], x1, x0, S.part, cfg=cfg)
             k_fc = dict(ln_w=w["ln2_w"], ln_b=w["ln2_b"], h_left=S.h, h_row0=r_fc) if mm <= r_fc else {}
@@ -151,6 +176,8 @@
         else:
             ops.layernorm(S.X[2 * l], w["ln1_w"], w["ln1_b"], h1, B * L, D, mean=m1, rstd=r1)
             ops.gemm(h1, w["in_w"], w["in_b"], out=S.qkv[l], epi=ops.EPI_BF16, cfg=cfg)
+            if cls_only:
+                return self._cls_tail_forward(S, l, B, L)
             ops.attn_fwd(S.q[l], S.k[l], S.v[l], S.a[l], lse=S.lse[l], causal=self.causal, qscale=dh ** -0.5 * ops.LOG2E)
             ops.gemm(S.a[l], w["out_w"], w["out_b"], out=S.X[2 * l + 1], res=S.X[2 * l], epi=res_epi, cfg=cfg)
             ops.layernorm(S.X[2 * l + 1], w["ln2_w"], w["ln2_b"], h2, B * L, D, mean=m2, rstd=r2)
@@ -194,10 +221,14 @@
             ops.layernorm_bwd_params(dpooled, S.X[2 * self.layers], S.post_stats[0], S.post_stats[1],
                                      self.grad_buffer(P + "ln_post.weight", e.ln_post[0]),
                                      self.grad_buffer(P + "ln_post.bias", e.ln_post[1]), B, D, x_row_stride=L * D)
-        S.dx.zero_()
-        ops.layernorm_bwd(dpooled, S.X[2 * self.layers], S.post_stats[0], S.post_stats[1], e.ln_post[0], B, D,
-                          dx=S.dx, x_row_stride=L * D, dx_row_stride=L * D)
-        self._blocks_backward(S, B, L, on_block_done)
+        if self._pruned:
+            ops.layernorm_bwd(dpooled, S.X[2 * self.layers], S.post_stats[0], S.post_stats[1], e.ln_post[0], B, D,
+                              dx=S.dxc, x_row_stride=L * D)
+        else:
+            S.dx.zero_()
+            ops.layernorm_bwd(dpooled, S.X[2 * self.layers], S.post_stats[0], S.post_stats[1], e.ln_post[0], B, D,
+                              dx=S.dx, x_row_stride=L * D, dx_row_stride=L * D)
+        self._blocks_backward(S, B, L, on_block_done, cls_only=self._pruned)
         dxpre = torch.empty(S.dx.shape, device=S.dx.device, dtype=torch.float32)
         if self.train_ln_pre:
             ops.layernorm_bwd_params(S.dx, S.xpre, S.pre_stats[0], S.pre_stats[1], self.grad_buffer(P + "ln_pre.weight", e.ln_pre[0]),
@@ -210,7 +241,20 @@
         self.dxpre = dxpre
         return dxpre.view(B, L, D)[:, 1:, :].reshape(B * T, D)
 
-    def _blocks_backward(self, S, B, L, on_block_done=None):
+    def _cls_block_backward(self, S, l, B, L):
+        e, D = self.eng, self.D
+        w, wT, cfg = e.blocks[l], self.wT[l], e.gemm_cfg
+        m1, r1 = S.stats[l][0], S.stats[l][1]
+        x1c = _engine.cls_rows(S.X[2 * l + 1], B, L)
+        ops.gemm(S.dxc, wT["proj_w"], None, out=S.du1, res=S.u1, epi=ops.EPI_DGELU, act=self.act_dsave, cfg=cfg)
+        ops.gemm(S.du1, wT["fc_w"], None, out=S.dhc, epi=ops.EPI_BF16, cfg=cfg)
+        ops.layernorm_bwd(S.dhc, x1c, S.stats2c[0], S.stats2c[1], w["ln2_w"], B, D, dres=S.dxc, dx=S.dxc, x_row_stride=L * D)
+        ops.gemm(S.dxc, wT["out_w"], None, out=S.dO1, epi=ops.EPI_BF16, cfg=cfg)
+        ops.attn_bwd_q1(S.q[l], S.k[l], S.v[l], S.dO1, S.a1, S.lse1, S.dqkv, S.dqkv[:, D:], S.dqkv[:, 2 * D:], 3 * D, 3 * D, qrow=0)
+        ops.gemm(S.dqkv, wT["in_w"], None, out=S.dh, epi=ops.EPI_BF16, cfg=cfg)
+        ops.layernorm_bwd_sparse_res(S.dh, S.X[2 * l], m1, r1, w["ln1_w"], B * L, D, dres=S.dxc, dres_every=L, dx=S.dx)
+
+    def _blocks_backward(self, S, B, L, on_block_done=None, cls_only=False):
         e, D, H = self.eng, self.D, self.H
         rows = B * L
         cfg = e.gemm_cfg
@@ -220,6 +264,9 @@
         if f32_stream:
             ops.cast_bf16(S.dx, out=S.dxb)
         for l in reversed(range(self.layers)):
+            if cls_only and l == self.layers - 1:
+                self._cls_block_backward(S, l, B, L)
+                continue
             if self.checkpoint:
                 self._block_forward(S, l, B, L, write_out=False)
             w, wT = e.blocks[l], self.wT[l]
```
